# jinseikenai/glomeruli_segmentation

Hardware: AMD Instinct MI355X
Metric: patches/sec (1024x512 RGB) ESPNet p=2 q=8 5 classes, HBM-resident, two batches in flight (higher is better)
Workload: dtype f32; 1 GPU; ESPNet p=2 q=8 encoder+decoder, batch=32 synthetic 1024x512 uint8 BGR tiles per GPU, normalise+forward+argmax+counts, inputs resident in HBM, steps rotate through 4 distinct batches, 2 batch(es) in flight (engine lanes, one HIP stream each) for `value`; global_batch=32, weights=espnet_fold1 (tests/golden), parallelism=tile-range per rank x1

## Files before the change

glomeruli_segmentation_amd/_lib.py:

```python
import ctypes
import os

_PKG = os.path.dirname(os.path.abspath(__file__))
LIB_PATH = os.path.join(_PKG, "libglomseg.so")
if os.environ.get("GLOMSEG_LIB") and os.environ.get("GLOMSEG_EXPERIMENT") == "1":
    LIB_PATH = os.environ["GLOMSEG_LIB"]

GS_OK = 0
GS_IN_U8_BGR_NHWC = 0
GS_IN_F32_NCHW = 1
ABI_VERSION = 10
GS_BUILD_DIAG = 1
GS_FORM_NONE = -1
GS_MAX_ENSEMBLE_C = 8
MAX_CROPS_PER_CALL = 64

STATUS_NAMES = {0: "GS_OK", 1: "GS_ERR_INVALID", 2: "GS_ERR_HIP", 3: "GS_ERR_NOMEM", 4: "GS_ERR_UNSUPPORTED",
                5: "GS_ERR_NODEVICE", 6: "GS_ERR_DEVICE_FAULT"}


class GlomsegError(RuntimeError):
    def __init__(self, status, message):
        super().__init__("%s: %s" % (STATUS_NAMES.get(status, status), message))
        self.status = status


class LayerDesc(ctypes.Structure):
    _fields_ = [("name", ctypes.c_char * 96), ("offset", ctypes.c_int64), ("ndim", ctypes.c_int32),
                ("shape", ctypes.c_int32 * 4)]


class CropDesc(ctypes.Structure):
    _fields_ = [("in_off", ctypes.c_int64), ("out_off", ctypes.c_int64), ("h", ctypes.c_int32), ("w", ctypes.c_int32),
                ("x1", ctypes.c_int32), ("y1", ctypes.c_int32)]


class PasteTarget(ctypes.Structure):
    _fields_ = [("slide_map", ctypes.c_void_p), ("map_h", ctypes.c_int32), ("map_w", ctypes.c_int32), ("ds", ctypes.c_int32),
                ("sx_lut", ctypes.c_void_p), ("sy_lut", ctypes.c_void_p)]


class CropOverlay(ctypes.Structure):
    _fields_ = [("palette_rgb", ctypes.c_void_p), ("n_colours", ctypes.c_int32), ("wa", ctypes.c_float), ("wb", ctypes.c_float),
                ("out_bgr", ctypes.POINTER(ctypes.c_void_p))]


class CropScoring(ctypes.Structure):
    _fields_ = [("labels", ctypes.POINTER(ctypes.c_void_p)), ("conf", ctypes.c_void_p), ("seen", ctypes.c_void_p),
                ("gt_overlay_bgr", ctypes.POINTER(ctypes.c_void_p)), ("gt_clamp", ctypes.c_int32)]


class EvalBox(ctypes.Structure):
    _fields_ = [("x0", ctypes.c_int32), ("y0", ctypes.c_int32), ("x1", ctypes.c_int32), ("y1", ctypes.c_int32),
                ("raster_w", ctypes.c_int32), ("raster_h", ctypes.c_int32), ("offset", ctypes.c_int64)]


class EvalSet(ctypes.Structure):
    _fields_ = [("rasters", ctypes.c_void_p), ("raster_bytes", ctypes.c_int64), ("boxes", ctypes.c_void_p),
                ("n_boxes", ctypes.c_int32), ("win_ptr", ctypes.c_void_p), ("win_idx", ctypes.c_void_p), ("n_idx", ctypes.c_int32),
                ("small_map", ctypes.c_void_p)]


class DetectorLayerPlan(ctypes.Structure):
    _fields_ = [("images", ctypes.c_int64), ("in_h", ctypes.c_int32), ("in_w", ctypes.c_int32), ("out_h", ctypes.c_int32),
                ("out_w", ctypes.c_int32), ("form", ctypes.c_int32)]


class DetectorPlan(ctypes.Structure):
    _fields_ = [("hf", ctypes.c_int32), ("wf", ctypes.c_int32), ("workspace_bytes", ctypes.c_int64), ("n_layers", ctypes.c_int32),
                ("layers", DetectorLayerPlan * 16)]


class WeightPiece(ctypes.Structure):
    _fields_ = [("name", ctypes.c_char * 32), ("offset", ctypes.c_longlong), ("floats", ctypes.c_longlong)]


class KernelTime(ctypes.Structure):
    _fields_ = [("name", ctypes.c_char * 64), ("total_ms", ctypes.c_double), ("launches", ctypes.c_int64),
                ("flops_per_tile", ctypes.c_double)]


_P = ctypes.c_void_p
_FP = ctypes.POINTER(ctypes.c_float)
_I = ctypes.c_int

PROTOTYPES = {
    "gs_last_error": (ctypes.c_char_p, []),
    "gs_abi_version": (_I, []),
    "gs_build_flags": (_I, []),
    "gs_device_fault_check": (_I, []),
    "gs_espnet_create": (_I, [_P, ctypes.POINTER(LayerDesc), _I, _I, _I, _I, _I, ctypes.POINTER(_P)]),
    "gs_espnet_destroy": (None, [_P]),
    "gs_espnet_reserve": (_I, [_P, _I, _I, _I]),
    "gs_espnet_forward": (_I, [_P, _P, _I, _I, _I, _I, _FP, _FP, _P, _P, _P, _P]),
    "gs_espnet_set_lanes": (_I, [_P, _I]),
    "gs_espnet_lanes": (_I, [_P]),
    "gs_espnet_forward_lane": (_I, [_P, _I, _P, _I, _I, _I, _I, _FP, _FP, _P, _P, _P, _P]),
    "gs_espnet_segment_host": (_I, [_P, _P, _I, _I, _I, _FP, _FP, _I, _P, _P]),
    "gs_espnet_segment_crops": (_I, [_P, _I, _P, ctypes.POINTER(CropDesc), _I, _FP, _FP, _I, _I, _P, _P, _P,
                                ctypes.POINTER(PasteTarget), _P]),
    "gs_espnet_ensemble_segment_crops": (_I, [ctypes.POINTER(_P), _I, _P, ctypes.POINTER(CropDesc), _I, _FP, _FP, _I, _I, _P, _P, _P,
                                         ctypes.POINTER(PasteTarget), _P]),
    "gs_espnet_segment_crops_host": (_I, [ctypes.POINTER(_P), _I, ctypes.POINTER(_P), ctypes.POINTER(_I), ctypes.POINTER(_I), _I, _FP, _FP,
                                     _I, _I, _I, ctypes.POINTER(_P), _P, _P, ctypes.POINTER(PasteTarget), ctypes.POINTER(_I),
                                     ctypes.POINTER(_I), ctypes.POINTER(CropOverlay)]),
    "gs_crops_from_masks": (_I, [_P, ctypes.POINTER(CropDesc), _I, _I, _I, _I, _P, _P, ctypes.POINTER(PasteTarget), _P, _P, _I,
                            ctypes.c_float, ctypes.c_float, _I, _P, _P]),
    "gs_plan_crop_batches": (_I, [ctypes.POINTER(_I), ctypes.POINTER(_I), _I, _I, ctypes.POINTER(_I), _I, ctypes.POINTER(_I)]),
    "gs_host_block_is_pinned": (_I, [_P, ctypes.c_size_t]),
    "gs_espnet_ensemble_forward": (_I, [ctypes.POINTER(_P), _I, _P, _I, _I, _I, _FP, _FP, _P, _P, _P]),
    "gs_espnet_read_stage": (_I, [_P, ctypes.c_char_p, _I, _P, ctypes.c_size_t, ctypes.POINTER(_I * 3)]),
    "gs_espnet_block_forward": (_I, [_P, _I, _I, _I, _P, _I, _I, _P]),
    "gs_espnet_plan_forward": (_I, [_I, _I, _I, _I, _I, _I, _I, ctypes.POINTER(_I), _I, ctypes.POINTER(_I)]),
    "gs_espnet_form_info": (_I, [_I, _I, ctypes.POINTER(ctypes.c_char_p), ctypes.POINTER(_I)]),
    "gs_espnet_profile_enable": (_I, [_P, _I]),
    "gs_espnet_profile_read": (_I, [_P, ctypes.POINTER(KernelTime), _I, ctypes.POINTER(_I)]),
    "gs_crop_preprocess": (_I, [_P, _I, _I, _FP, _FP, _I, _I, _P, _P]),
    "gs_mask_resize_nearest": (_I, [_P, _I, _I, _I, _I, _P, _P]),
    "gs_find_contours": (_I, [_P, _I, _I, _I, _P, _I, _P, _I, ctypes.POINTER(_I), ctypes.POINTER(_I)]),
    "gs_arc_length_closed": (ctypes.c_double, [_P, _I]),
    "gs_approx_poly_closed": (_I, [_P, _I, ctypes.c_double, _P]),
    "gs_wsi_paste_max": (_I, [_P, _I, _I, _I, _P, _I, _I, _I, _I, _P]),
    "gs_wsi_paste_max_lut": (_I, [_P, _I, _I, _I, _P, _P, _P, _I, _I, _I, _I, _P]),
    "gs_overlay_classmap": (_I, [_P, _P, _I, _I, _P, _I, ctypes.c_float, ctypes.c_float, _P, _P]),
    "gs_confusion_u8": (_I, [_P, _P, ctypes.c_longlong, _I, _P, _P]),
    "gs_wsi_eval_windows": (_I, [_I, _I, _I, _I, ctypes.POINTER(EvalSet), ctypes.POINTER(EvalSet), _P, _P, _I, _I, _P, _P, _P]),
    "gs_conv2d_nhwc": (_I, [_P, _I, _I, _I, _I, _P, _I, _I, _I, _P, _I, _I, _I, _P, _P]),
    "gs_conv2d_nhwc_form": (_I, [_I] * 10 + [ctypes.POINTER(ctypes.c_char_p)]),
    "gs_roialign": (_I, [_P, _I, _I, _I, _I, _P, _P, _I, _I, _P, _P]),
    "gs_nms": (_I, [_P, _P, _I, ctypes.c_float, ctypes.c_float, _I, _P, _P, _P]),
    "gs_detector_create": (_I, [_P, ctypes.POINTER(LayerDesc), _I, ctypes.POINTER(_P)]),
    "gs_detector_destroy": (None, [_P]),
    "gs_detector_max_detections": (_I, []),
    "gs_detector_num_proposals": (_I, []),
    "gs_detector_layer_info": (_I, [_I, ctypes.POINTER(ctypes.c_char_p)] + [ctypes.POINTER(_I)] * 6),
    "gs_detector_plan": (_I, [_I, _I, _I, ctypes.POINTER(DetectorPlan)]),
    "gs_detector_set_thresholds": (_I, [_P, ctypes.c_float, ctypes.c_float, ctypes.c_float]),
    "gs_detector_forward": (_I, [_P, _P, _I, _I, _I, _P, _P, _P, _P, _P, _P, _P, _P, _P]),
    "gs_detector_detect_host": (_I, [_P, ctypes.POINTER(_P), _I, _I, _I, _I, _P, _P, _P, _P]),
}

SCORING_PROTOTYPES = {
    "gs_espnet_score_crops": (_I, [_P, _P, ctypes.POINTER(CropDesc), _I, _I, _I, _I, _P, _P, _P]),
    "gs_espnet_segment_crops_host_scored": (_I, PROTOTYPES["gs_espnet_segment_crops_host"][1] + [ctypes.POINTER(CropScoring)]),
}

PLAN_PROTOTYPES = {
    "gs_espnet_plan_flags": (_I, [_I, _I, _I, _I, _I, _I, _I, _I, ctypes.POINTER(_I)]),
    "gs_espnet_pack_weights": (_I, [_P, ctypes.POINTER(LayerDesc), _I, _I, _I, _I, _I, _P, ctypes.c_size_t, ctypes.POINTER(ctypes.c_size_t),
                                ctypes.POINTER(WeightPiece), _I, ctypes.POINTER(_I)]),
    "gs_espnet_workspace_plan": (_I, [_I] * 7 + [ctypes.POINTER(ctypes.c_size_t)]),
}
GS_PLAN_LAZY_B2, GS_PLAN_L3C_IN_REDUCE, GS_PLAN_CLS_IN_L3 = 1, 2, 4

INSTANCE_PROTOTYPES = {
    "gs_instances_plan": (_I, [_I, _I, _I, _I, ctypes.POINTER(ctypes.c_size_t)]),
    "gs_slide_instances": (_I, [_P, _I, _I, _I, _I, _P, ctypes.c_size_t, _I, _P, _P, _P, _P, _P]),
}

MATCH_PROTOTYPES = {
    "gs_instance_match_plan": (_I, [_I, _I, _I, ctypes.POINTER(ctypes.c_size_t)]),
    "gs_instance_overlaps": (_I, [_P, _P, _P, _P, _I, _I, _P, ctypes.c_size_t, _I, _P, _P, _P, _P]),
    "gs_instance_match": (_I, [_P, _P, _P, _I, _P, _I, _P, _I, _I, _I, _I, _P, _P, _P]),
}

BOUNDARY_PROTOTYPES = {
    "gs_boundary_dist_plan": (_I, [_I, _I, ctypes.POINTER(ctypes.c_size_t)]),
    "gs_instance_boundary_dist": (_I, [_P, _P, _P, _I, _P, _I, _I, _I, _P, ctypes.c_size_t, _P, _P, _P, _P]),
}

_lib = None


def load():
    global _lib
    if _lib is not None:
        return _lib
    if not os.path.exists(LIB_PATH):
        raise ImportError(
            "%s is missing: build it with `python -m glomeruli_segmentation_amd.build` "
            "(hipcc --offload-arch=gfx950).  There is no CPU fallback." % LIB_PATH)
    lib = ctypes.CDLL(LIB_PATH, mode=ctypes.RTLD_GLOBAL)
    for name, (res, args) in list(PROTOTYPES.items()) + list(SCORING_PROTOTYPES.items()) + list(PLAN_PROTOTYPES.items()) + \
            list(INSTANCE_PROTOTYPES.items()) + list(MATCH_PROTOTYPES.items()) + list(BOUNDARY_PROTOTYPES.items()):
        if name in PLAN_PROTOTYPES and not hasattr(lib, name):
            continue
        fn = getattr(lib, name)
        fn.restype = res
        fn.argtypes = args
    if lib.gs_abi_version() != ABI_VERSION:
        raise ImportError("libglomseg.so ABI %d != binding ABI %d: rebuild" % (lib.gs_abi_version(), ABI_VERSION))
    if (lib.gs_build_flags() & GS_BUILD_DIAG) and os.environ.get("GLOMSEG_ALLOW_DIAG") != "1":
        raise ImportError("%s is a -DGS_DIAG experiment build (its timing variants return wrong results by construction); "
                          "set GLOMSEG_ALLOW_DIAG=1 to load it for an A/B measurement" % LIB_PATH)
    _lib = lib
    return lib


def check(status):
    if status != GS_OK:
        raise GlomsegError(status, load().gs_last_error().decode("utf-8", "replace"))


def fptr3(values):
    arr = (ctypes.c_float * len(values))(*[float(v) for v in values])
    return arr
```

glomeruli_segmentation_amd/build.py:

```python
import os
import subprocess
import sys
import tempfile

PKG = os.path.dirname(os.path.abspath(__file__))
CSRC = os.path.join(PKG, "csrc")
LIB = os.path.join(PKG, "libglomseg.so")
SOURCES = ["espnet.hip", "dec_tail.hip", "crops.hip", "detect_ops.hip", "detector.hip", "wsi_eval.hip", "instances.hip", "instance_match.hip", "boundary_dist.hip", "contours.cpp"]
HEADERS = ["gs_internal.h", "conv_mfma.h", "dec_tail.h", "dec_tail_args.h", "espnet_kernels.h", "espnet_facts.h", "espnet_weights.h", "workspace_plan.h", "crop_sample.h", "crop_plan.h", "wave_block.h", "slide_map_plan.h", "instance_plan.h", "instance_match_plan.h", "boundary_dist_plan.h", "detect_math.h", "detect_plan.h", "host_copy.h", "host_jobs.h", "host_pipe.h",
           os.path.join("..", "..", "include", "glomseg.h"), os.path.join("..", "..", "include", "glomseg_scoring.h"),
           os.path.join("..", "..", "include", "glomseg_plan.h"), os.path.join("..", "..", "include", "glomseg_instances.h"),
           os.path.join("..", "..", "include", "glomseg_instance_match.h"),
           os.path.join("..", "..", "include", "glomseg_boundary_dist.h")]
FLAGS = ["-O3", "--offload-arch=gfx950", "-std=c++17", "-fPIC", "-Wall", "-Wno-unused-result",
         "-Wno-unused-value"]


def _sources():
    return [s for s in SOURCES if os.path.exists(os.path.join(CSRC, s))]


def _stale(lib):
    if not os.path.exists(lib):
        return True
    t = os.path.getmtime(lib)
    deps = [os.path.join(CSRC, s) for s in _sources() + HEADERS] + [os.path.abspath(__file__)]
    deps += [os.path.join(CSRC, f) for f in os.listdir(CSRC) if f.endswith(".h") or f.endswith(".inc")]
    return any(os.path.getmtime(d) > t for d in deps)


def build_lib(force=False, verbose=False, out=None, extra_flags=()):
    lib = os.path.abspath(out) if out else LIB
    if not (force or _stale(lib)):
        return lib
    hipcc = os.environ.get("HIPCC", "/opt/rocm/bin/hipcc")
    os.makedirs(os.path.dirname(lib), exist_ok=True)
    objdir = CSRC if out is None else tempfile.mkdtemp(prefix="glomseg_obj_")
    objs = []
    procs = []
    for s in _sources():
        o = os.path.join(objdir, s.replace(".hip", ".o").replace(".cpp", ".o"))
        objs.append(o)
        cmd = [hipcc] + FLAGS + list(extra_flags) + (["-x", "hip"] if s.endswith(".cpp") else []) + ["-c", os.path.join(CSRC, s), "-o", o]
        if verbose:
            print(" ".join(cmd))
        procs.append((cmd, subprocess.Popen(cmd)))
    for cmd, p in procs:
        if p.wait() != 0:
            raise RuntimeError("hipcc failed: " + " ".join(cmd))
    cmd = [hipcc, "--offload-arch=gfx950", "-shared", "-fPIC", "-o", lib] + objs + ["-Wl,-rpath,/opt/rocm/lib"]
    if verbose:
        print(" ".join(cmd))
    subprocess.check_call(cmd)
    return lib


if __name__ == "__main__":
    argv = sys.argv[1:]
    extra = []
    if "--" in argv:
        extra = argv[argv.index("--") + 1:]
        argv = argv[:argv.index("--")]
    out = argv[argv.index("--out") + 1] if "--out" in argv else None
    print(build_lib(force="--force" in argv or out is not None, verbose=True, out=out, extra_flags=extra))
```

glomeruli_segmentation_amd/csrc/conv_mfma.h:

```cpp
#pragma once
#include <map>
#include <mutex>
#include <type_traits>

#include "gs_internal.h"

namespace gs {

#ifdef GS_DIAG
constexpr bool kDiag = true;
#else
constexpr bool kDiag = false;
#endif

template <int N, typename F>
__device__ __forceinline__ void static_for(F &&f)
{
    if constexpr (N > 0) {
        static_for<N - 1>(f);
        f(std::integral_constant<int, N - 1>{});
    }
}

typedef float f32x16 __attribute__((ext_vector_type(16)));
typedef float f32x4 __attribute__((ext_vector_type(4)));

template <int MT>
struct Mfma;
template <>
struct Mfma<32> {
    static constexpr int KL = 2, NACC = 16;
    using acc_t = f32x16;
    static __device__ __forceinline__ acc_t run(float a, float b, acc_t c)
    {
        return __builtin_amdgcn_mfma_f32_32x32x2f32(a, b, c, 0, 0, 0);
    }
    static __device__ __forceinline__ int row(int r, int kq) { return (r & 3) + 8 * (r >> 2) + 4 * kq; }
};
template <>
struct Mfma<16> {
    static constexpr int KL = 4, NACC = 4;
    using acc_t = f32x4;
    static __device__ __forceinline__ acc_t run(float a, float b, acc_t c)
    {
        return __builtin_amdgcn_mfma_f32_16x16x4f32(a, b, c, 0, 0, 0);
    }
    static __device__ __forceinline__ int row(int r, int kq) { return kq * 4 + r; }
};

struct ConvArgs {
    const float *in;
    long long in_sn;
    int in_sc, in_pitch, in_off;
    unsigned in_img_bytes;
    const float *wpack;
    int wfloats;
    float *out;
    long long out_sn;
    int out_sc, out_pitch, out_off;
    unsigned out_img_bytes, res_img_bytes;
    const float *res;
    long long res_sn;
    int res_sc, res_pitch, res_off;
    float *out2;
    long long out2_sn;
    int out2_sc, out2_pitch, out2_off, out2_coff;
    unsigned out2_img_bytes;
    float *out3;
    long long out3_sn;
    int out3_sc, out3_pitch, out3_off, nout3;
    unsigned out3_img_bytes;
    int bnl_s0, bnl_s1;
    float *side;
    long long side_sn;
    int side_sc, side_pitch, side_off;
    unsigned side_img_bytes;
    const float *crec;
    float *cls;
    long long cls_sn;
    int cls_sc, cls_pitch;
    unsigned cls_img_bytes;
    int stagger;
    int prio_mode;
    unsigned long long *stamp;
    int N, H, W;
    int strips;
    int total_tasks;
    int wu;
};

typedef unsigned u32x3_t __attribute__((ext_vector_type(3)));
typedef unsigned u32x2_t __attribute__((ext_vector_type(2)));
typedef unsigned u32x4_t __attribute__((ext_vector_type(4)));

template <int N, int AUX = 0>
__device__ __forceinline__ void buf_load_vec(const __amdgpu_buffer_rsrc_t &rs, int voff, int soff, float *dst)
{
    if constexpr (N == 1) {
        dst[0] = __builtin_bit_cast(float, __builtin_amdgcn_raw_buffer_load_b32(rs, voff, soff, AUX));
    } else if constexpr (N == 2) {
        const u32x2_t v = __builtin_amdgcn_raw_buffer_load_b64(rs, voff, soff, AUX);
        const unsigned e0 = v[0], e1 = v[1];
        dst[0] = __builtin_bit_cast(float, e0);
        dst[1] = __builtin_bit_cast(float, e1);
    } else {
        static_assert(N == 4 || N == 8, "vector width");
#pragma unroll
        for (int h = 0; h < N / 4; ++h) {
            const u32x4_t v = __builtin_amdgcn_raw_buffer_load_b128(rs, voff + 16 * h, soff, AUX);
            const unsigned e0 = v[0], e1 = v[1], e2 = v[2], e3 = v[3];
            dst[4 * h + 0] = __builtin_bit_cast(float, e0);
            dst[4 * h + 1] = __builtin_bit_cast(float, e1);
            dst[4 * h + 2] = __builtin_bit_cast(float, e2);
            dst[4 * h + 3] = __builtin_bit_cast(float, e3);
        }
    }
}
template <int N, int AUX = 0>
__device__ __forceinline__ void buf_store_vec(const __amdgpu_buffer_rsrc_t &rs, int voff, const float *src)
{
    if constexpr (N == 1) {
        __builtin_amdgcn_raw_buffer_store_b32(__builtin_bit_cast(unsigned, src[0]), rs, voff, 0, AUX);
    } else if constexpr (N == 2) {
        u32x2_t v;
        v[0] = __builtin_bit_cast(unsigned, src[0]);
        v[1] = __builtin_bit_cast(unsigned, src[1]);
        __builtin_amdgcn_raw_buffer_store_b64(v, rs, voff, 0, AUX);
    } else {
#pragma unroll
        for (int h = 0; h < N / 4; ++h) {
            u32x4_t v;
#pragma unroll
            for (int j = 0; j < 4; ++j)
                v[j] = __builtin_bit_cast(unsigned, src[4 * h + j]);
            __builtin_amdgcn_raw_buffer_store_b128(v, rs, voff + 16 * h, 0, AUX);
        }
    }
}

__device__ __forceinline__ float prelu_pin(float alpha)
{
    return alpha <= 1.0f ? __builtin_inff() : -__builtin_inff();
}
__device__ __forceinline__ float prelu_med3(float v, float alpha, float pin)
{
    return __builtin_amdgcn_fmed3f(v, alpha * v, pin);
}

typedef float f32x2 __attribute__((ext_vector_type(2)));
__device__ __forceinline__ float cls_fma(float a, float b, float c) { return fmaf(a, b, c); }
__device__ __forceinline__ f32x2 cls_fma(float a, f32x2 b, f32x2 c) { return __builtin_elementwise_fma((f32x2)(a), b, c); }
__device__ __forceinline__ float cls_prelu(float v, float alpha, float pin) { return prelu_med3(v, alpha, pin); }
__device__ __forceinline__ f32x2 cls_prelu(f32x2 v, float alpha, float pin)
{
    const f32x2 av = v * alpha;
    f32x2 o;
    o[0] = __builtin_amdgcn_fmed3f(v[0], av[0], pin);
    o[1] = __builtin_amdgcn_fmed3f(v[1], av[1], pin);
    return o;
}

constexpr int F_BNACT = 1;
constexpr int F_RES = 2;
constexpr int F_NOSTORE = 4;
constexpr int F_DUAL = 8;
constexpr int F_S2PAIR = 512;
constexpr int F_VEC = 1024;
constexpr int F_RES_NT = 8192;
constexpr int F_ST_NT = 16384;
constexpr int F_ST2_NT = 32768;
constexpr int F_IN_NT = 65536;
constexpr int F_A_GLOBAL = 131072;
constexpr int F_FUSE1X1 = 262144;
constexpr int F_S2_FLIP = 1048576;
constexpr int F_SKIP_PAD = 4194304;
constexpr int F_BNLOAD = 8388608;
constexpr int F_SIDE_SHIFT = 27;
constexpr int F_SIDE1X1(int classes) { return classes << F_SIDE_SHIFT; }
constexpr int F_CLS1X1 = 256;
constexpr int CLS_N = 5, CLS_REC = 8;
constexpr int F_X_NOLOAD = 16;
constexpr int F_X_NOLDS = 32;
constexpr int F_X_NOEPI = 64;
constexpr int F_X_STAMP2 = 4096;
constexpr int STAMP2_SLOTS = 128;
constexpr int F_X_STAMP = 128;
constexpr int F_X_NOEPIMEM = 2097152;
constexpr int F_X_RESL2 = 33554432;
constexpr int F_X_STL2 = 67108864;
constexpr int F_X_ALL = F_X_NOLOAD | F_X_NOLDS | F_X_NOEPI | F_X_STAMP | F_X_STAMP2 | F_X_NOEPIMEM | F_X_RESL2 | F_X_STL2;

constexpr int conv_cls_lds_offset(int image_lds_floats) { return (image_lds_floats + 255) / 256 * 256; }

#ifndef CFG_STAGE_ROT
#define CFG_STAGE_ROT 17
#endif
#ifndef CFG_L3_RING
#define CFG_L3_RING 13
#endif
#ifndef CFG_L2_RING
#define CFG_L2_RING 27
#endif
constexpr int conv_ring_depth(int MT, int TAPS, int NDIL, int P, int G)
{
    return (MT == 32 && TAPS == 9 && NDIL == 5 && (P == 1 || P == 2) && G == 13) ? CFG_L3_RING
           : (MT == 16 && TAPS == 9 && NDIL == 5 && P == 4 && G == 9) ? CFG_L2_RING
                                                                    : G * (TAPS == 9 ? 3 : 1);
}

#define M_KL_OF(MT_) (Mfma<MT_>::KL)
template <int MT, int WAVES, int CINP, int TAPS, int STRIDE, int NDIL, int NOUT1, int NOUT, int P, int G, int FLAGS>
__global__ void __launch_bounds__(WAVES * 64, WAVES >= 8 ? WAVES / 8 : 2) conv_mfma_kernel(const ConvArgs a)
{
    constexpr bool BNACT = FLAGS & F_BNACT, RES = FLAGS & F_RES, STORE1 = !(FLAGS & F_NOSTORE), DUAL = FLAGS & F_DUAL;
    constexpr bool S2P = FLAGS & F_S2PAIR;
    constexpr bool VEC = FLAGS & F_VEC;
    constexpr bool AGL = FLAGS & F_A_GLOBAL, FUSE = FLAGS & F_FUSE1X1;
    constexpr bool S2FLIP = FLAGS & F_S2_FLIP;
    constexpr bool SKIP = FLAGS & F_SKIP_PAD;
    constexpr bool BNL = FLAGS & F_BNLOAD;
    constexpr int SCLS = (FLAGS >> F_SIDE_SHIFT) & 15;
    constexpr bool SIDE = SCLS > 0;
    constexpr bool CLSF = FLAGS & F_CLS1X1;
    static_assert(!CLSF || (MT == 32 && NDIL == 5 && TAPS == 9 && (FLAGS & F_BNACT) && !(FLAGS & (F_DUAL | F_NOSTORE | F_BNLOAD | F_X_ALL)) &&
                            !SIDE && ((NOUT1 + (NDIL - 1) * NOUT) * CLS_REC) % 256 == 0 && (NOUT1 + (NDIL - 1) * NOUT) * CLS_REC / 256 <= WAVES),
                  "F_CLS1X1 is for the level-3 branch launches: 32-row accumulators, five slots, the records in whole DMA pieces");
    static_assert(!SIDE || ((FLAGS & F_S2PAIR) && TAPS == 9 && STRIDE == 2 && MT == 32 && NDIL == 1 && SCLS <= SIDE_REC &&
                            (CINP / M_KL_OF(MT)) % G == 0 && G * M_KL_OF(MT) <= SIDE_ZROWS && !(FLAGS & (F_A_GLOBAL | F_VEC | F_X_ALL))),
                  "F_SIDE1X1 is for the stride-2 3x3 reduce on 32-pixel runs, a tap row in whole chunks");
    static_assert(!BNL || ((FLAGS & F_S2PAIR) && !(FLAGS & (F_BNACT | F_A_GLOBAL | F_VEC))), "F_BNLOAD is for the plain stride-2 reduce");
    static_assert(!SKIP || (TAPS == 9 && STRIDE == 1 && !(FLAGS & F_S2PAIR) && G * M_KL_OF(MT) == CINP),
                  "F_SKIP_PAD: unit-stride 3x3 with one tap row per chunk");
    static_assert(!S2FLIP || (STRIDE == 2 && TAPS == 9 && NDIL == 1), "F_S2_FLIP is for the stride-2 3x3 reduce");
    static_assert(kDiag || !(FLAGS & F_X_ALL), "timing / stamp variants exist in -DGS_DIAG builds only");
    constexpr int IAUX = (FLAGS & F_IN_NT) ? 2 : 0;
    constexpr int RAUX = (FLAGS & F_RES_NT) ? 2 : 0, SAUX = (FLAGS & F_ST_NT) ? 2 : 0, SAUX2 = (FLAGS & F_ST2_NT) ? 2 : 0;
    static_assert(!VEC || (STRIDE == 1 && (P == 2 || P == 4 || P == 8)), "F_VEC needs unit stride and P in {2,4,8}");
    static_assert(!S2P || (STRIDE == 2 && TAPS == 9 && NDIL == 1), "F_S2PAIR is for the stride-2 3x3 reduce");
    using M = Mfma<MT>;
    constexpr int KL = M::KL;
    constexpr int NSTEP = CINP / KL;
    constexpr int NROW = NOUT1 > NOUT ? NOUT1 : NOUT;
    constexpr int COUT = NOUT1 + (NDIL - 1) * NOUT;
    constexpr int TYN = TAPS == 1 ? 1 : 3;
    constexpr int TXN = TAPS == 9 ? 3 : 1;
    constexpr int XSTEP = P * MT;
    constexpr int RGN = TYN * NSTEP;
    constexpr int D = G * TXN;
    constexpr int R = conv_ring_depth(MT, TAPS, NDIL, P, G);
    constexpr int RA = R;
    static_assert(D % R == 0 && (R == D || !(FLAGS & (F_S2PAIR | F_BNLOAD))), "the ring divides the chunk");
    constexpr int CPD = RGN / G;
    constexpr int NCHUNK = NDIL * CPD;
    static_assert(CINP % KL == 0, "k-steps must tile");
    static_assert(TAPS == 1 || TAPS == 9, "1x1 or 3x3");
    static_assert(RGN % G == 0, "chunk must divide the row groups of one dilation");
    static_assert(NROW <= MT, "one MFMA row block");
    constexpr int KSTR = 4;

    extern __shared__ __attribute__((aligned(16))) float lds[];
    const int tid = threadIdx.x;
    unsigned long long tstamp0 = 0;
    if (FLAGS & (F_X_STAMP | F_X_STAMP2))
        tstamp0 = __builtin_amdgcn_s_memrealtime();
    constexpr int WFL = NDIL * TAPS * CINP * NROW;
    constexpr int LDS_SRC0 = AGL ? WFL : 0;
    static_assert(!AGL || WFL % 4 == 0, "LDS-DMA source must stay 16-byte aligned");
    static_assert(!FUSE || (TAPS == 9 && BNACT), "the fused 1x1 follows a branch kernel's epilogue");
    const float *bnp = lds + (WFL - LDS_SRC0);
    constexpr int BNFL = (BNACT ? 3 * COUT : 0) + (DUAL ? 3 * COUT : 0);
    const float *tab = bnp + BNFL;
    constexpr int BNL_C = CINP + M::KL;
    const float *bnl = lds + (conv_image(CINP, TAPS, NDIL, NOUT1, NOUT, BNACT, DUAL, FUSE ? M::NACC : 0).total - LDS_SRC0);
    const float *sidew = lds + side_table_offset(conv_image(CINP, TAPS, NDIL, NOUT1, NOUT, BNACT, DUAL, FUSE ? M::NACC : 0).total, CINP, M::KL);
    constexpr int CREC_OFF = conv_cls_lds_offset(conv_image(CINP, TAPS, NDIL, NOUT1, NOUT, BNACT, DUAL, FUSE ? M::NACC : 0).total - LDS_SRC0);
    const float *crecl = lds + CREC_OFF;
    const __amdgpu_buffer_rsrc_t rsrc_w =
        __builtin_amdgcn_make_buffer_rsrc(const_cast<float *>(a.wpack), 0, AGL ? WFL * 4 : 0, 0x00020000);

    const int lane = tid & 63;
    const int wid = __builtin_amdgcn_readfirstlane(tid >> 6);
    const int px = lane % MT, kq = lane / MT;
    const int xl = VEC ? px * P : px;
    const int voff = (kq * a.in_sc + xl * STRIDE) * 4;
    const int lbase = kq * NROW + (px < NROW ? px : NROW - 1);
    const int vout = (kq * KSTR * a.out_sc + xl) * 4;
    const int vres = RES ? (kq * KSTR * a.res_sc + xl) * 4 : 0;
    const int vout2 = DUAL ? (kq * KSTR * a.out2_sc + xl) * 4 : 0;
    const int vout3 = FUSE ? (kq * KSTR * a.out3_sc + xl) * 4 : 0;
    const int vcls = CLSF ? (kq * CLS_N * a.cls_sc + xl) * 4 : 0;
    const int prio_mode = kDiag ? a.prio_mode : 1;
    const bool second_of_simd = WAVES >= 8 ? wid >= WAVES / 2 : blockIdx.x >= gridDim.x / 2;

    const int NB = gridDim.x;
    const int wu = a.wu;
    int t0, t1, tstride;
    if ((NB & 7) == 0) {
        const int xcd = blockIdx.x & 7, per = NB >> 3;
        const int c0 = (int)((long long)a.total_tasks * xcd / 8), c1 = (int)((long long)a.total_tasks * (xcd + 1) / 8);
        t0 = c0 + (blockIdx.x >> 3) * wu + wid;
        t1 = c1;
        tstride = per * wu;
    } else {
        t0 = blockIdx.x * wu + wid;
        t1 = a.total_tasks;
        tstride = NB * wu;
    }
    if (wid >= wu)
        t0 = t1;
    const long long wg = (long long)blockIdx.x * WAVES + wid;
    const int tasks_per_img = a.H * a.strips;
    bool staged = false;

    float aq[RA], bq[S2P ? 1 : R][P];
    float bl[S2P ? G : 1][P][3];

    for (int task = t0; task < t1 || !staged; task += tstride) {
        const bool idle = task >= t1;
        const int tk = idle ? (a.total_tasks - 1) : task;
        const int n = tk / tasks_per_img;
        const int rem = tk - n * tasks_per_img;
        const int img_stride = tstride / tasks_per_img > 0 ? tstride / tasks_per_img : 1;
        const int yrot = SKIP ? a.H / 2 : 0;
        const int y0r = rem / a.strips;
        const int y = SKIP && ((n / img_stride) & 1) ? (y0r + yrot >= a.H ? y0r + yrot - a.H : y0r + yrot) : y0r;
        const int x0 = (rem - y0r * a.strips) * XSTEP;

        const __amdgpu_buffer_rsrc_t rsrc = __builtin_amdgcn_make_buffer_rsrc(
            const_cast<float *>(a.in + (long long)n * a.in_sn), 0, a.in_img_bytes, 0x00020000);
        const int sbase = (a.in_off + y * STRIDE * a.in_pitch + x0 * STRIDE) * 4;
        const int tn = task + tstride < t1 ? task + tstride : tk;
        const int n_n = tn / tasks_per_img;
        const int rem_n = tn - n_n * tasks_per_img;
        const int y0r_n = rem_n / a.strips;
        const int y_n = SKIP && ((n_n / img_stride) & 1) ? (y0r_n + yrot >= a.H ? y0r_n + yrot - a.H : y0r_n + yrot) : y0r_n;
        const __amdgpu_buffer_rsrc_t rsrc_n = __builtin_amdgcn_make_buffer_rsrc(
            const_cast<float *>(a.in + (long long)n_n * a.in_sn), 0, a.in_img_bytes, 0x00020000);
        const int sbase_n = (a.in_off + y_n * STRIDE * a.in_pitch + (rem_n - y0r_n * a.strips) * XSTEP * STRIDE) * 4;
        const bool flip = S2FLIP && (y & 1), flip_n = S2FLIP && (y_n & 1);
        const __amdgpu_buffer_rsrc_t rout =
            __builtin_amdgcn_make_buffer_rsrc(a.out + (long long)n * a.out_sn, 0, a.out_img_bytes, 0x00020000);
        const int sout = (a.out_off + y * a.out_pitch + x0) * 4;
        const __amdgpu_buffer_rsrc_t rres = __builtin_amdgcn_make_buffer_rsrc(
            const_cast<float *>(RES ? a.res + (long long)n * a.res_sn : a.in), 0, RES ? a.res_img_bytes : 0u, 0x00020000);
        const int sres = RES ? (a.res_off + y * a.res_pitch + x0) * 4 : 0;
        const __amdgpu_buffer_rsrc_t rout2 = __builtin_amdgcn_make_buffer_rsrc(
            DUAL ? a.out2 + (long long)n * a.out2_sn : a.out, 0, DUAL ? a.out2_img_bytes : 0u, 0x00020000);
        const int sout2 = DUAL ? (a.out2_off + y * a.out2_pitch + x0) * 4 : 0;
        const __amdgpu_buffer_rsrc_t rout3 = __builtin_amdgcn_make_buffer_rsrc(
            FUSE ? a.out3 + (long long)n * a.out3_sn : a.out, 0, FUSE ? a.out3_img_bytes : 0u, 0x00020000);
        const int sout3 = FUSE ? (a.out3_off + y * a.out3_pitch + x0) * 4 : 0;
        const __amdgpu_buffer_rsrc_t rcls = __builtin_amdgcn_make_buffer_rsrc(
            CLSF ? a.cls + (long long)n * a.cls_sn : a.out, 0, CLSF ? a.cls_img_bytes : 0u, 0x00020000);
        const int scls = CLSF ? (y * a.cls_pitch + x0) * 4 : 0;

        typename M::acc_t acc[P];
        typename M::acc_t acc2[FUSE ? P : 1];
        auto chunk_live = [&](int yy, int c) {
            const int di = c / CPD, ty = c - di * CPD;
            return ty == 1 || (ty == 0 ? yy >= (1 << di) : yy + (1 << di) < a.H);
        };
        const int c_first = SKIP && !chunk_live(y, 0) ? 1 : 0;
        const int c_first_n = SKIP && !chunk_live(y_n, 0) ? 1 : 0;

        constexpr int OOB = 0x7ffffff0;
        int vo[P], vr[P], vo2[P], vo3[P], vc[P];
#pragma unroll
        for (int p = 0; p < P; ++p) {
            const bool xok = x0 + (VEC ? xl : p * MT + px) < a.W;
            vo[p] = xok ? vout + (VEC ? 0 : p * MT * 4) : OOB;
            vr[p] = xok ? vres + (VEC ? 0 : p * MT * 4) : OOB;
            vo2[p] = xok ? vout2 + (VEC ? 0 : p * MT * 4) : OOB;
            vo3[p] = xok ? vout3 + (VEC ? 0 : p * MT * 4) : OOB;
            vc[p] = xok ? vcls + (VEC ? 0 : p * MT * 4) + scls : OOB;
        }
        constexpr int RR = RES ? M::NACC : 1;
        float resv[RR][P];
        auto load_res = [&](int di, int r) {
            if (!RES)
                return;
            if (FLAGS & F_X_NOEPIMEM) {
#pragma unroll
                for (int p = 0; p < P; ++p)
                    resv[r % RR][p] = __builtin_bit_cast(float, di + r + p);
                return;
            }
            const int nout = di == 0 ? NOUT1 : NOUT;
            const int cb = di == 0 ? 0 : NOUT1 + (di - 1) * NOUT;
            const int ch0 = M::row(r, 0);
            const bool live = ch0 + kq * KSTR < nout;
            const int sr = (cb + ch0) * a.res_sc * 4 + sres;
            if (VEC) {
                if (FLAGS & F_X_RESL2)
                    buf_load_vec<P, RAUX>(rres, live ? ((int)(wg & 255) * 8192 + ((vr[0] + sr) & 0x1ff0)) : OOB, 0, resv[r % RR]);
                else
                    buf_load_vec<P, RAUX>(rres, live ? vr[0] : OOB, sr, resv[r % RR]);
                return;
            }
#pragma unroll
            for (int p = 0; p < P; ++p)
                resv[r % RR][p] = __builtin_bit_cast(
                    float, __builtin_amdgcn_raw_buffer_load_b32(rres, live ? vr[p] : OOB, sr, RAUX));
        };
        auto prefetch_res = [&](int di) {
#pragma unroll
            for (int r = 0; r < RR; ++r)
                load_res(di, r);
        };

        auto decode_rg = [&](int cw, int g, int &ty0, int &sidx) {
            if constexpr (G % NSTEP == 0) {
                ty0 = cw * (G / NSTEP) + g / NSTEP;
                sidx = g % NSTEP;
            } else if constexpr (NSTEP % G == 0) {
                constexpr int CPR = NSTEP / G;
                ty0 = cw / CPR;
                sidx = (cw - ty0 * CPR) * G + g;
            } else {
                const int rg = cw * G + g;
                ty0 = rg / NSTEP;
                sidx = rg - ty0 * NSTEP;
            }
        };
        auto fetch_b = [&](const __amdgpu_buffer_rsrc_t &rs, int sb, int c, int g, int tx, bool fl) {
            const int di = c / CPD;
            int ty0, sidx;
            decode_rg(c - di * CPD, g, ty0, sidx);
            const int ty = S2FLIP && fl ? TYN - 1 - ty0 : ty0;
            const int toff = TAPS == 9 ? ((ty - 1) * a.in_pitch + (tx - 1)) << di : 0;
            const int soff = sb + (toff + sidx * KL * a.in_sc) * 4;
            if ((FLAGS & F_X_NOLOAD) && staged)
                return;
            if (VEC) {
                buf_load_vec<P, IAUX>(rs, voff, soff, bq[S2P ? 0 : (g * TXN + tx) % R]);
                return;
            }
#pragma unroll
            for (int p = 0; p < P; ++p)
                bq[(g * TXN + tx) % R][p] = __builtin_bit_cast(
                    float, __builtin_amdgcn_raw_buffer_load_b32(rs, voff + p * MT * STRIDE * 4, soff, IAUX));
        };
        auto fetch_pair = [&](const __amdgpu_buffer_rsrc_t &rs, int sb, int c, int g, bool fl) {
            if ((FLAGS & F_X_NOLOAD) && staged)
                return;
            int ty0, sidx;
            decode_rg(c, g, ty0, sidx);
            const int ty = S2FLIP && fl ? TYN - 1 - ty0 : ty0;
            const int soff = sb + ((ty - 1) * a.in_pitch - 1 + sidx * KL * a.in_sc) * 4;
#pragma unroll
            for (int p = 0; p < P; ++p) {
                const u32x3_t v = __builtin_amdgcn_raw_buffer_load_b96(rs, voff + p * MT * STRIDE * 4, soff, IAUX);
                const unsigned e0 = v[0], e1 = v[1], e2 = v[2];
                bl[g][p][0] = __builtin_bit_cast(float, e0);
                bl[g][p][1] = __builtin_bit_cast(float, e1);
                bl[g][p][2] = __builtin_bit_cast(float, e2);
            }
        };
        auto fetch_a = [&](int c, int g, int tx, bool fl) {
            const int di = c / CPD;
            int ty0, sidx;
            decode_rg(c - di * CPD, g, ty0, sidx);
            const int ty = S2FLIP && fl ? TYN - 1 - ty0 : ty0;
            const int tap = TAPS == 9 ? ty * 3 + tx : 0;
            if ((FLAGS & F_X_NOLDS) && staged)
                return;
            if (AGL)
                aq[(g * TXN + tx) % R] = __builtin_bit_cast(
                    float, __builtin_amdgcn_raw_buffer_load_b32(rsrc_w, lbase * 4, (((di * TAPS + tap) * CINP + sidx * KL) * NROW) * 4, 0));
            else
                aq[(g * TXN + tx) % R] = lds[((di * TAPS + tap) * CINP + sidx * KL) * NROW + lbase];
        };

        auto bnl_fetch = [&](int cc, int gg, int yy, bool ff, float &sc2, float &sh2, float &al2, bool &raw) {
            int ty0c, sidxc;
            decode_rg(cc, gg, ty0c, sidxc);
            const int tyc = S2FLIP && ff ? TYN - 1 - ty0c : ty0c;
            raw = sidxc >= a.bnl_s0 && sidxc < a.bnl_s1;
            const bool padrow = yy * STRIDE + tyc - 1 < 0 && raw;
            const int ch = (padrow ? NSTEP : sidxc) * KL + kq;
            sc2 = bnl[ch];
            sh2 = bnl[BNL_C + ch];
            al2 = bnl[2 * BNL_C + ch];
        };
        float tsc = 1.0f, tsh = 0.0f, tal = 1.0f, tpin = 0.0f;
        float nsc = 1.0f, nsh = 0.0f, nal = 1.0f;
        bool traw = false, nraw = false;
        float bt[BNL ? 2 : 1][P][3];
        static_assert(!BNL || G % 2 == 0, "F_BNLOAD: the two-group operand buffer alternates by row-group parity");
        auto bnl_apply = [&](float &dst, float v, float sc2, float sh2, float al2, float pin2, bool zero) {
            v = v * sc2 + sh2;
            v = prelu_med3(v, al2, pin2);
            dst = zero ? 0.0f : v;
        };

        float side[SIDE ? P : 1][SIDE ? SCLS : 1][2], sw[SIDE ? SCLS : 1];
        const __amdgpu_buffer_rsrc_t rside = __builtin_amdgcn_make_buffer_rsrc(
            SIDE ? a.side + (long long)n * a.side_sn : a.out, 0, SIDE ? a.side_img_bytes : 0u, 0x00020000);

        if (task == t0) {
#pragma unroll
            for (int g = 0; g < G; ++g) {
                if (S2P) {
                    fetch_pair(rsrc, sbase, 0, g, flip);
                    continue;
                }
#pragma unroll
                for (int tx = 0; tx < TXN; ++tx)
                    if (g * TXN + tx < R)
                        fetch_b(rsrc, sbase, c_first, g, tx, flip);
            }
        }
        if (!staged) {
            const int pieces = (a.wfloats - LDS_SRC0 + 255) / 256;
            if ((FLAGS & F_X_STAMP2) && lane == 0)
                a.stamp[wg * STAMP2_SLOTS + STAMP2_SLOTS - 2] = __builtin_amdgcn_s_memrealtime();
            const int rot = (int)((blockIdx.x * (unsigned)CFG_STAGE_ROT) % (unsigned)(pieces > 0 ? pieces : 1));
            for (int j0 = wid; j0 < pieces; j0 += WAVES) {
                const int j = j0 + rot < pieces ? j0 + rot : j0 + rot - pieces;
                __builtin_amdgcn_global_load_lds(
                    (const __attribute__((address_space(1))) void *)(a.wpack + LDS_SRC0 + j * 256 + lane * 4),
                    (__attribute__((address_space(3))) void *)(lds + j * 256), 16, 0, 0);
            }
            if (CLSF) {
                if (wid < COUT * CLS_REC / 256)
                    __builtin_amdgcn_global_load_lds(
                        (const __attribute__((address_space(1))) void *)(a.crec + wid * 256 + lane * 4),
                        (__attribute__((address_space(3))) void *)(lds + CREC_OFF + wid * 256), 16, 0, 0);
                if (tid < CLS_REC)
                    lds[CREC_OFF + COUT * CLS_REC + tid] = 0.0f;
// ... 421 lines not shown
```

glomeruli_segmentation_amd/csrc/espnet.hip:

```cpp
#include <chrono>
#include <cmath>
#include <cstdio>
#include <cstdlib>
#include <functional>
#include <map>
#include <memory>
#include <string>
#include <thread>
#include <vector>

#include "../../include/glomseg_plan.h"
#include "conv_mfma.h"
#include "dec_tail_args.h"
#include "enc_head.h"
#include "enc_head_ens.h"
#include "espnet_config.h"
#include "forward_plan.h"
#include "espnet_kernels.h"
#include "espnet_weights.h"
#include "host_copy.h"
#include "host_pipe.h"
#include "workspace_plan.h"

namespace gs {

static thread_local std::string g_err;
void set_error(const char *fmt, ...)
{
    char buf[1024];
    va_list ap;
    va_start(ap, fmt);
    vsnprintf(buf, sizeof buf, fmt, ap);
    va_end(ap);
    g_err = buf;
}

#ifdef GS_DIAG
static bool getenv_flag(const char *name)
{
    const char *e = std::getenv(name);
    return e && std::atoi(e) != 0;
}
static bool no_vec() { return getenv_flag("GS_NO_VEC"); }
#else
static constexpr bool no_vec() { return false; }
#endif

enum KernelId {
    K_STEM, K_POOL, K_L2_C1S, K_L2_DOWN, K_L2_C1, K_L2_ESP, K_CAT_B2, K_L3_C1S, K_L3_DOWN, K_L3_C1, K_L3_ESP,
    K_DEC1, K_DEC2, K_DEC3, K_DEC_CONV, K_DEC4, K_DEC_TAIL, K_ENC_HEAD, K_ENC_HEAD_ENS, K_COUNT
};
static const char *kKernelNames[K_COUNT] = {
    "stem_kernel", "pool_kernel", "conv_l2_reduce_s2", "conv_l2_down_branches", "conv_l2_reduce_1x1",
    "conv_l2_esp_branches", "cat_b2_kernel", "conv_l3_reduce_s2", "conv_l3_down_branches", "conv_l3_reduce_1x1",
    "conv_l3_esp_branches", "dec1_kernel", "dec2_kernel", "dec3_kernel", "conv_dec_cbr", "dec4_kernel", "dec_tail_kernel",
    "enc_head_kernel", "enc_head_ens_kernel"};

struct Model : Workspace {
    int classes = 0, p = 0, q = 0;
    int cp = 0;
    bool encoder_only = false;
    int device = 0, num_cus = 256;
#ifdef GS_DIAG
    int variant = 0;
#else
    static constexpr int variant = 0;
#endif
    float *dblob = nullptr;
    EspnetOffsets w;

    void *ws = nullptr;
    size_t ws_bytes = 0;
    int ws_n = 0, ws_h = 0, ws_w = 0;
    float *prob = nullptr;
    size_t prob_bytes = 0;
    std::map<std::string, std::pair<Act, int>> stages;
    void set_stage(const std::string &name, const Act &act, int C)
    {
        for (auto it = stages.begin(); it != stages.end();)
            it = it->second.first.base == act.base ? stages.erase(it) : std::next(it);
        stages[name] = {act, C};
    }
    int last_n = 0;
    bool b2_lazy = false;

    bool profile = false;
    struct Ev { hipEvent_t a, b; int k; };
    std::vector<Ev> events;
    double prof_ms[K_COUNT] = {0};
    long long prof_launches[K_COUNT] = {0};
    double prof_flops[K_COUNT] = {0};
};

static gs_status layout_workspace(Model *m, int n, int H, int W)
{
    if (m->ws && n <= m->ws_n && H == m->ws_h && W == m->ws_w)
        return GS_OK;
    if (m->ws) {
        GS_HIP(hipDeviceSynchronize());
        GS_HIP(hipFree(m->ws));
        m->ws = nullptr;
    }
    WorkspacePlan plan;
    const gs_status st = plan_workspace(n, H, W, m->cp, m->p, m->encoder_only, plan);
    if (st != GS_OK)
        return st;
    void *ws = nullptr;
    if (hipMalloc(&ws, plan.bytes) != hipSuccess) {
        set_error("workspace allocation of %zu bytes failed (n=%d, %dx%d)", plan.bytes, n, H, W);
        return GS_ERR_NOMEM;
    }
    GS_HIP(hipMemset(ws, 0, plan.bytes));
    GS_HIP(hipDeviceSynchronize());
    static_cast<Workspace &>(*m) = plan.acts;
    int i = 0;
    for (Act *a : acts_of(*m))
        a->base = reinterpret_cast<float *>(static_cast<char *>(ws) + plan.at[i++]);
    m->ws = ws;
    m->ws_bytes = plan.bytes;
    m->ws_n = n;
    m->ws_h = H;
    m->ws_w = W;
    return GS_OK;
}

struct Launcher {
    Model *m;
    hipStream_t s;
    gs_status st = GS_OK;
    int n;
    template <typename F>
    void run(int kid, double flops_per_tile, F &&f)
    {
        if (st != GS_OK)
            return;
        Model::Ev ev{nullptr, nullptr, kid};
        if (m->profile) {
            if (hipEventCreate(&ev.a) != hipSuccess || hipEventCreate(&ev.b) != hipSuccess ||
                hipEventRecord(ev.a, s) != hipSuccess) {
                set_error("profiling event setup failed");
                st = GS_ERR_HIP;
                return;
            }
        }
        st = f();
        if (st == GS_OK && hipGetLastError() != hipSuccess) {
            set_error("launch of %s failed", kKernelNames[kid]);
            st = GS_ERR_HIP;
        }
        if (m->profile && st == GS_OK) {
            hipEventRecord(ev.b, s);
            m->events.push_back(ev);
            m->prof_flops[kid] += flops_per_tile;
        }
    }
};

static ConvArgs conv_args(const Act &in, const float *wpack, const Act &out, const Act *res, int n)
{
    ConvArgs a{};
    a.in = in.base;
    a.in_sn = in.sn;
    a.in_sc = in.sc;
    a.in_pitch = in.pitch;
    a.in_off = in.off;
    a.in_img_bytes = (unsigned)(in.sn * sizeof(float));
    a.wpack = wpack;
    a.out = out.base;
    a.out_sn = out.sn;
    a.out_sc = out.sc;
    a.out_pitch = out.pitch;
    a.out_off = out.off;
    a.out_img_bytes = (unsigned)(out.sn * sizeof(float));
    if (res) {
        a.res = res->base;
        a.res_sn = res->sn;
        a.res_sc = res->sc;
        a.res_pitch = res->pitch;
        a.res_off = res->off;
        a.res_img_bytes = (unsigned)(res->sn * sizeof(float));
    }
    a.N = n;
    a.H = out.H;
    a.W = out.W;
    return a;
}

static inline unsigned blocks_for(long long items) { return (unsigned)((items + 255) / 256); }

#ifdef GS_DIAG
#include "espnet_diag.inc"
#define GS_DIAG_TRY(call)     \
    do {                      \
        gs_status dst_;       \
        if (call) return dst_; \
    } while (0)
#else
#define GS_DIAG_TRY(call) \
    do {                  \
    } while (0)
#define GS_DIAG_STAMPED(var, tag, ca, ...)
#endif

static gs_status not_planned(const char *launch_class)
{
    set_error("internal: the forward plan has no form for launch class %s", launch_class);
    return GS_ERR_INVALID;
}

template <int FLAGS, int... C>
static gs_status launch_vec(const ConvArgs &ca, int num_cus, hipStream_t s, bool vec)
{
    return vec ? launch_conv_mfma<C..., FLAGS | F_VEC>(ca, num_cus, s) : launch_conv_mfma<C..., FLAGS>(ca, num_cus, s);
}

static gs_status launch_l2_reduce(const Model *m, const ConvArgs &ca, hipStream_t s) { return launch_conv_mfma<CFG_L2_C1S, F_S2PAIR | POL_L2_C1S | S2FLIP_L2>(ca, m->num_cus, s); }
static gs_status launch_l2_c1(const Model *m, const ConvArgs &ca, hipStream_t s) { return launch_conv_mfma<CFG_L2_C1, POL_L2_C1>(ca, m->num_cus, s); }
static gs_status launch_l3_c1(const Model *m, const ConvArgs &ca, hipStream_t s) { return launch_conv_mfma<CFG_L3_C1, POL_L3_C1>(ca, m->num_cus, s); }

static gs_status launch_l2_down(const Model *m, form::l2_down f, const ConvArgs &ca, hipStream_t s)
{
    switch (f) {
    case form::l2_down::P2S_VEC: return launch_vec<F_BNACT | (POL_L2_DOWN & F_ST_NT) | FUSE_L2, CFG_L2_BR_P2S>(ca, m->num_cus, s, true);
    case form::l2_down::P4S_VEC_SKIP:
        GS_DIAG_STAMPED(162, "l2down", ca, F_BNACT | (POL_L2_DOWN & F_ST_NT) | FUSE_L2 | F_VEC, CFG_L2_BR_P4)
        return launch_conv_mfma<CFG_L2_BR_P4S, F_BNACT | (POL_L2_DOWN & F_ST_NT) | FUSE_L2 | F_VEC | F_SKIP_PAD>(ca, m->num_cus, s);
    case form::l2_down::P4_VEC:
        GS_DIAG_STAMPED(162, "l2down", ca, F_BNACT | (POL_L2_DOWN & F_ST_NT) | FUSE_L2 | F_VEC, CFG_L2_BR_P4)
        return launch_vec<F_BNACT | (POL_L2_DOWN & F_ST_NT) | FUSE_L2, CFG_L2_BR_P4>(ca, m->num_cus, s, true);
    case form::l2_down::P4: return launch_vec<F_BNACT | (POL_L2_DOWN & F_ST_NT) | FUSE_L2, CFG_L2_BR_P4>(ca, m->num_cus, s, false);
    case form::l2_down::UNFUSED_P4_VEC: return launch_vec<F_BNACT | (POL_L2_DOWN & F_ST_NT), CFG_L2_BR_P4>(ca, m->num_cus, s, true);
    case form::l2_down::UNFUSED_P4: return launch_vec<F_BNACT | (POL_L2_DOWN & F_ST_NT), CFG_L2_BR_P4>(ca, m->num_cus, s, false);
    case form::l2_down::none: break;
    }
    return not_planned("l2_down");
}

static gs_status launch_l2_esp_fused(const Model *m, form::l2_esp_fused f, const ConvArgs &ca, hipStream_t s)
{
    switch (f) {
    case form::l2_esp_fused::P2S_VEC: return launch_vec<F_BNACT | F_RES | POL_L2_ESP | FUSE_L2, CFG_L2_BR_P2S>(ca, m->num_cus, s, true);
    case form::l2_esp_fused::P4_VEC:
        GS_DIAG_STAMPED(161, "l2esp", ca, F_BNACT | F_RES | POL_L2_ESP | FUSE_L2 | F_VEC, CFG_L2_BR_P4)
        return launch_vec<F_BNACT | F_RES | POL_L2_ESP | FUSE_L2, CFG_L2_BR_P4>(ca, m->num_cus, s, true);
    case form::l2_esp_fused::P4: return launch_vec<F_BNACT | F_RES | POL_L2_ESP | FUSE_L2, CFG_L2_BR_P4>(ca, m->num_cus, s, false);
    case form::l2_esp_fused::UNFUSED_P4_VEC: return launch_vec<F_BNACT | F_RES | POL_L2_ESP, CFG_L2_BR_P4>(ca, m->num_cus, s, true);
    case form::l2_esp_fused::UNFUSED_P4: return launch_vec<F_BNACT | F_RES | POL_L2_ESP, CFG_L2_BR_P4>(ca, m->num_cus, s, false);
    case form::l2_esp_fused::none: break;
    }
    return not_planned("l2_esp_fused");
}

static gs_status launch_l2_esp_last(const Model *m, form::l2_esp_last f, const ConvArgs &ca, hipStream_t s)
{
    switch (f) {
    case form::l2_esp_last::P2S_VEC: return launch_vec<F_BNACT | F_RES | F_NOSTORE | F_DUAL | POL_L2_LAST, CFG_L2_BR_P2S>(ca, m->num_cus, s, true);
    case form::l2_esp_last::P4_VEC:
        GS_DIAG_STAMPED(163, "l2last", ca, F_BNACT | F_RES | F_NOSTORE | F_DUAL | POL_L2_LAST | F_VEC, CFG_L2_BR_P4)
        return launch_vec<F_BNACT | F_RES | F_NOSTORE | F_DUAL | POL_L2_LAST, CFG_L2_BR_P4>(ca, m->num_cus, s, true);
    case form::l2_esp_last::P4: return launch_vec<F_BNACT | F_RES | F_NOSTORE | F_DUAL | POL_L2_LAST, CFG_L2_BR_P4>(ca, m->num_cus, s, false);
    case form::l2_esp_last::none: break;
    }
    return not_planned("l2_esp_last");
}

static gs_status launch_l3_reduce(const Model *m, form::l3_reduce f, bool side5, const ConvArgs &ca, hipStream_t s)
{
    constexpr int SIDE5 = F_SIDE1X1(5);
    if (side5)
        switch (f) {
        case form::l3_reduce::BNL_P1: return launch_conv_mfma<CFG_L3_C1S_BNL_P1, F_S2PAIR | POL_L3_C1S | S2FLIP_L3 | F_BNLOAD | SIDE5>(ca, m->num_cus, s);
        case form::l3_reduce::BNL: return launch_conv_mfma<CFG_L3_C1S_BNL, F_S2PAIR | POL_L3_C1S | S2FLIP_L3 | F_BNLOAD | SIDE5>(ca, m->num_cus, s);
        case form::l3_reduce::C1S: return launch_conv_mfma<CFG_L3_C1S, F_S2PAIR | POL_L3_C1S | S2FLIP_L3 | SIDE5>(ca, m->num_cus, s);
        case form::l3_reduce::none: return not_planned("l3_reduce");
        }
    switch (f) {
    case form::l3_reduce::BNL_P1: return launch_conv_mfma<CFG_L3_C1S_BNL_P1, F_S2PAIR | POL_L3_C1S | S2FLIP_L3 | F_BNLOAD>(ca, m->num_cus, s);
    case form::l3_reduce::BNL:
        GS_DIAG_STAMPED(165, "l3c1s", ca, F_S2PAIR | POL_L3_C1S | S2FLIP_L3 | F_BNLOAD, CFG_L3_C1S_BNL)
        return launch_conv_mfma<CFG_L3_C1S_BNL, F_S2PAIR | POL_L3_C1S | S2FLIP_L3 | F_BNLOAD>(ca, m->num_cus, s);
    case form::l3_reduce::C1S: return launch_conv_mfma<CFG_L3_C1S, F_S2PAIR | POL_L3_C1S | S2FLIP_L3>(ca, m->num_cus, s);
    case form::l3_reduce::none: break;
    }
    return not_planned("l3_reduce");
}

static gs_status launch_l3_down(const Model *m, form::l3_down f, bool cls5, const ConvArgs &ca, hipStream_t s)
{
    if (cls5)
        switch (f) {
        case form::l3_down::P1R: return launch_conv_mfma<CFG_L3_BR_P1R, F_BNACT | POL_L3_DOWN | FUSE_L3 | SKIP_L3 | (CFG_SMALL_AGL ? F_A_GLOBAL : 0) | F_CLS1X1>(ca, m->num_cus, s);
        case form::l3_down::P2R_VEC: return launch_conv_mfma<CFG_L3_BR_P2R, F_BNACT | POL_L3_DOWN | FUSE_L3 | F_VEC | SKIP_L3 | F_CLS1X1>(ca, m->num_cus, s);
        case form::l3_down::P2F: return launch_conv_mfma<CFG_L3_BR_P2F, F_BNACT | POL_L3_DOWN | FUSE_L3 | F_CLS1X1>(ca, m->num_cus, s);
        default: return not_planned("l3_down with the classifier's side sums");
        }
    switch (f) {
    case form::l3_down::P1R: return launch_conv_mfma<CFG_L3_BR_P1R, F_BNACT | POL_L3_DOWN | FUSE_L3 | SKIP_L3 | (CFG_SMALL_AGL ? F_A_GLOBAL : 0)>(ca, m->num_cus, s);
    case form::l3_down::P2R_VEC:
        GS_DIAG_STAMPED(164, "l3down", ca, F_BNACT | POL_L3_DOWN | FUSE_L3 | F_VEC | SKIP_L3, CFG_L3_BR_P2R)
        return launch_conv_mfma<CFG_L3_BR_P2R, F_BNACT | POL_L3_DOWN | FUSE_L3 | F_VEC | SKIP_L3>(ca, m->num_cus, s);
    case form::l3_down::BR_VEC: return launch_conv_mfma<CFG_L3_BR, F_BNACT | POL_L3_DOWN | FUSE_L3 | F_VEC>(ca, m->num_cus, s);
    case form::l3_down::P2F: return launch_conv_mfma<CFG_L3_BR_P2F, F_BNACT | POL_L3_DOWN | FUSE_L3>(ca, m->num_cus, s);
    case form::l3_down::UNFUSED_BR_VEC: return launch_vec<F_BNACT | POL_L3_DOWN, CFG_L3_BR>(ca, m->num_cus, s, true);
    case form::l3_down::UNFUSED_BR: return launch_vec<F_BNACT | POL_L3_DOWN, CFG_L3_BR>(ca, m->num_cus, s, false);
    case form::l3_down::none: break;
    }
    return not_planned("l3_down");
}

static gs_status launch_l3_esp_fused(const Model *m, form::l3_esp_fused f, const ConvArgs &ca, int block, hipStream_t s)
{
    switch (f) {
    case form::l3_esp_fused::P1R: return launch_conv_mfma<CFG_L3_BR_P1R, F_BNACT | F_RES | POL_L3_ESP | FUSE_L3 | SKIP_L3 | (CFG_SMALL_AGL ? F_A_GLOBAL : 0)>(ca, m->num_cus, s);
    case form::l3_esp_fused::P2R_VEC:
        if (block == 1) {
            GS_DIAG_STAMPED(160, "l3esp", ca, F_BNACT | F_RES | F_VEC | POL_L3_ESP | FUSE_L3 | SKIP_L3, CFG_L3_BR_P2R)
        }
        return launch_conv_mfma<CFG_L3_BR_P2R, F_BNACT | F_RES | F_VEC | POL_L3_ESP | FUSE_L3 | SKIP_L3>(ca, m->num_cus, s);
    case form::l3_esp_fused::P2F: return launch_conv_mfma<CFG_L3_BR_P2F, F_BNACT | F_RES | FUSE_L3>(ca, m->num_cus, s);
    case form::l3_esp_fused::none: break;
    }
    return not_planned("l3_esp_fused");
}

static gs_status launch_l3_esp_last(const Model *m, form::l3_esp_last f, bool cls5, const ConvArgs &ca, hipStream_t s)
{
    if (cls5)
        switch (f) {
        case form::l3_esp_last::P1R: return launch_conv_mfma<CFG_L3_BR_P1R, F_BNACT | F_RES | POL_L3_ESP | SKIP_L3 | (CFG_SMALL_AGL ? F_A_GLOBAL : 0) | F_CLS1X1>(ca, m->num_cus, s);
        case form::l3_esp_last::P2R_VEC: return launch_conv_mfma<CFG_L3_BR_P2R, F_BNACT | F_RES | F_VEC | POL_L3_ESP | SKIP_L3 | F_CLS1X1>(ca, m->num_cus, s);
        case form::l3_esp_last::BR_VEC: return launch_conv_mfma<CFG_L3_BR, F_BNACT | F_RES | F_VEC | POL_L3_ESP | F_CLS1X1>(ca, m->num_cus, s);
        case form::l3_esp_last::P2: return launch_conv_mfma<CFG_L3_BR_P2, F_BNACT | F_RES | F_CLS1X1>(ca, m->num_cus, s);
        case form::l3_esp_last::none: return not_planned("l3_esp_last");
        }
    switch (f) {
    case form::l3_esp_last::P1R: return launch_conv_mfma<CFG_L3_BR_P1R, F_BNACT | F_RES | POL_L3_ESP | SKIP_L3 | (CFG_SMALL_AGL ? F_A_GLOBAL : 0)>(ca, m->num_cus, s);
    case form::l3_esp_last::P2R_VEC: return launch_conv_mfma<CFG_L3_BR_P2R, F_BNACT | F_RES | F_VEC | POL_L3_ESP | SKIP_L3>(ca, m->num_cus, s);
    case form::l3_esp_last::BR_VEC: return launch_conv_mfma<CFG_L3_BR, F_BNACT | F_RES | F_VEC | POL_L3_ESP>(ca, m->num_cus, s);
    case form::l3_esp_last::P2: return launch_conv_mfma<CFG_L3_BR_P2, F_BNACT | F_RES>(ca, m->num_cus, s);
    case form::l3_esp_last::none: break;
    }
    return not_planned("l3_esp_last");
}

template <int CLS>
static gs_status launch_dec3(const Model *m, form::dec3 f, const ConvArgs &ca, hipStream_t s)
{
    switch (f) {
    case form::dec3::MT16:
    case form::dec3::MT32: return launch_vec<F_BNACT, dec_mt(CLS), 8, 2 * CLS, 9, 1, 1, CLS, CLS, dec_pixels(CLS), 3>(ca, m->num_cus, s, false);
    case form::dec3::MT16_VEC:
    case form::dec3::MT32_VEC: return launch_vec<F_BNACT, dec_mt(CLS), 8, 2 * CLS, 9, 1, 1, CLS, CLS, dec_pixels(CLS), 3>(ca, m->num_cus, s, true);
    case form::dec3::KERNEL:
    case form::dec3::none: break;
    }
    return not_planned("dec3");
}

template <int CLS>
static gs_status launch_dec_conv(const Model *m, form::dec_conv f, const ConvArgs &ca, hipStream_t s)
{
    constexpr int CINP = (19 + CLS + 3) / 4 * 4;
    switch (f) {
    case form::dec_conv::MT16:
    case form::dec_conv::MT32: return launch_vec<F_BNACT | POL_DEC_CONV, dec_mt(CLS), 8, CINP, 9, 1, 1, CLS, CLS, dec_pixels(CLS), 3>(ca, m->num_cus, s, false);
    case form::dec_conv::MT16_VEC:
    case form::dec_conv::MT32_VEC: return launch_vec<F_BNACT | POL_DEC_CONV, dec_mt(CLS), 8, CINP, 9, 1, 1, CLS, CLS, dec_pixels(CLS), 3>(ca, m->num_cus, s, true);
    case form::dec_conv::TAIL:
    case form::dec_conv::none: break;
    }
    return not_planned("dec_conv");
}

struct Encoded { int last; bool lazy_b2; };
static Encoded encode(Model *m, Launcher &L, const ForwardPlan &plan, const ForwardReq &r)
{
    const float *wb = m->dblob;
    const hipStream_t s = r.s;
    const int n = r.n, H = r.H, W = r.W, H1 = H / 2, W1 = W / 2, H2 = H / 4, W2 = W / 4, H3 = H / 8, W3 = W / 8;
    const double px1 = (double)H1 * W1, px2 = (double)H2 * W2, px3 = (double)H3 * W3;
    m->stages.clear();
    m->last_n = n;
    L.run(K_STEM, px1 * (27 * 16 * 2), [&] {
        StemArgs a{};
        a.in = r.in;
        for (int i = 0; i < 3; ++i) {
            a.mean[i] = r.mean ? r.mean[i] : 0.0f;
            a.std[i] = r.stdv ? r.stdv[i] : 1.0f;
        }
        std::memcpy(a.w1, m->w.stem_params, sizeof(float) * 432);
        std::memcpy(a.bn1, m->w.stem_params + 432, sizeof(float) * 48);
        std::memcpy(a.b1, m->w.stem_params + 480, sizeof(float) * 57);
        a.a0 = view(m->a0);
        a.inp1 = view(m->inp1);
        a.N = n;
        a.H = H;
        a.W = W;
        if (r.hist && ens_finishes((int)r.role)) {
            a.hist_zero = r.hist;
            a.hist_count = n * m->classes;
        }
        hipLaunchKernelGGL(r.in_format == GS_IN_U8_BGR_NHWC ? stem_kernel<true> : stem_kernel<false>,
                           dim3(blocks_for((long long)n * H1 * ((W1 + STEM_PX - 1) / STEM_PX))), dim3(256), 0, s, a);
        return GS_OK;
    });
    L.run(K_POOL, 0, [&] {
        hipLaunchKernelGGL(pool_kernel, dim3(blocks_for((long long)n * 3 * H2 * W2)), dim3(256), 0, s, view(m->inp1),
                           view(m->inp2), n, 3, m->p > 0 ? wb + m->w.b2 : nullptr, view(m->a1), 128, 131);
        return GS_OK;
    });
    m->set_stage("b1", m->a0, 19);
    m->set_stage("sample2", m->inp2, 3);

    L.run(K_L2_C1S, px2 * (19 * 9 * 12 * 2), [&] {
        GS_DIAG_TRY(diag_reduce_s2(m, 2, conv_args(m->a0, wb + m->w.l2_0.c1, m->r2[0], nullptr, n), s, dst_));
        return launch_l2_reduce(m, conv_args(m->a0, wb + m->w.l2_0.c1, m->r2[0], nullptr, n), s);
    });
    auto with_dual = [&](ConvArgs a, int coff) {
        a.out2 = m->a1.base;
        a.out2_sn = m->a1.sn;
        a.out2_sc = m->a1.sc;
        a.out2_pitch = m->a1.pitch;
        a.out2_off = m->a1.off;
        a.out2_coff = coff;
        a.out2_img_bytes = (unsigned)(m->a1.sn * sizeof(float));
        return a;
    };
    auto with_fused = [&](ConvArgs a, const Act &r, int nout3) {
        a.out3 = r.base;
        a.out3_sn = r.sn;
        a.out3_sc = r.sc;
        a.out3_pitch = r.pitch;
        a.out3_off = r.off;
        a.out3_img_bytes = (unsigned)(r.sn * sizeof(float));
        a.nout3 = nout3;
        return a;
    };
    auto with_cls = [&](ConvArgs a, int producer) {
        a.crec = wb + m->w.b3 + (long long)producer * 128 * CLS_REC;
        a.cls_sc = H3 * W3;
        a.cls_pitch = W3;
        a.cls = m->tt.base + (long long)producer * 2 * CLS_N * a.cls_sc;
        a.cls_sn = m->tt.sn;
        a.cls_img_bytes = (unsigned)((size_t)2 * CLS_N * a.cls_sc * sizeof(float));
        return a;
    };
    const bool lazy_b2 = plan.lazy_b2;
    m->b2_lazy = lazy_b2;
    int rd2 = 0;
    L.run(K_L2_DOWN, px2 * (12 * 9 * 64 * 2) + (m->w.l2_0.fused_next ? px2 * (64 * 12 * 2) : 0), [&] {
        const ConvArgs ca = conv_args(m->r2[rd2], wb + m->w.l2_0.br, m->bb[0], nullptr, n);
        return launch_l2_down(m, plan.l2_down, m->w.l2_0.fused_next ? with_fused(ca, m->r2[rd2 ^ 1], 12) : ca, s);
    });
    bool have_r2 = m->w.l2_0.fused_next;
    rd2 ^= have_r2 ? 1 : 0;
    m->set_stage("level2_0", m->bb[0], 64);
    int cur2 = 0;
    for (int i = 0; i < m->p; ++i) {
        const int nxt = cur2 == 1 ? 2 : 1;
        const bool last = i == m->p - 1;
        const bool fuse_next = m->w.l2[i].fused_next;
        if (!have_r2)
            L.run(K_L2_C1, px2 * (64 * 12 * 2), [&] {
                return launch_l2_c1(m, conv_args(m->bb[cur2], wb + m->w.l2[i].c1, m->r2[rd2], nullptr, n), s);
            });
        L.run(K_L2_ESP, px2 * (12 * 9 * 64 * 2) + (fuse_next ? px2 * (64 * 12 * 2) : 0), [&] {
            const ConvArgs ca = conv_args(m->r2[rd2], wb + m->w.l2[i].br, m->bb[nxt], &m->bb[cur2], n);
            if (last)
                return launch_l2_esp_last(m, plan.l2_esp_last, with_dual(ca, 0), s);
            return launch_l2_esp_fused(m, plan.l2_esp_fused, fuse_next ? with_fused(ca, m->r2[rd2 ^ 1], 12) : ca, s);
        });
        have_r2 = fuse_next;
        rd2 ^= have_r2 ? 1 : 0;
        cur2 = nxt;
        if (!last)
            m->set_stage("level2." + std::to_string(i), m->bb[cur2], 64);
    }
    if (plan.cat_b2 == form::cat_b2::KERNEL) {
        L.run(K_CAT_B2, 0, [&] {
            hipLaunchKernelGGL(cat_b2_kernel, dim3(blocks_for((long long)n * 131 * H2 * W2)), dim3(256), 0, s, view(m->bb[cur2]),
                               view(m->bb[0]), view(m->inp2), wb + m->w.b2, view(m->a1), n);
            return GS_OK;
        });
    }
    m->set_stage("b2", m->a1, 131);

    int rd3 = 0;
    L.run(K_L3_C1S, px3 * (131 * 9 * 25 * 2) + (plan.l3c_in_reduce ? px2 * (131 * m->classes * 2) : 0), [&] {
        GS_DIAG_TRY(diag_reduce_s2(m, 3, conv_args(m->a1, wb + m->w.l3_0.c1, m->r3[0], nullptr, n), s, dst_));
        ConvArgs ca = conv_args(m->a1, wb + m->w.l3_0.c1, m->r3[0], nullptr, n);
        if (lazy_b2) {
            ca.bnl_s0 = 64 / 2;
            ca.bnl_s1 = 128 / 2;
        }
        if (plan.l3c_in_reduce) {
            ca.side = m->l3c.base;
            ca.side_sn = m->l3c.sn;
            ca.side_sc = m->l3c.sc;
            ca.side_pitch = m->l3c.pitch;
            ca.side_off = m->l3c.off;
            ca.side_img_bytes = (unsigned)(m->l3c.sn * sizeof(float));
        }
        return launch_l3_reduce(m, plan.l3_reduce, plan.l3c_in_reduce, ca, s);
    });
    if (plan.l3c_in_reduce)
        m->set_stage("level3_C", m->l3c, m->classes);
    const double cls_flops = plan.cls_in_l3 ? px3 * (128 * m->classes * 2) : 0;
    L.run(K_L3_DOWN, px3 * (25 * 9 * 128 * 2) + (m->w.l3_0.fused_next ? px3 * (128 * 25 * 2) : 0) + cls_flops, [&] {
        ConvArgs ca = conv_args(m->r3[rd3], wb + m->w.l3_0.br, m->cc[0], nullptr, n);
        if (plan.cls_in_l3) {
            if ((long long)CLS_PART_PLANES * H3 * W3 > m->tt.sn) {
                set_error("internal: the classifier's partial planes do not fit the workspace's tt");
                return GS_ERR_INVALID;
            }
            ca = with_cls(ca, 0);
        }
        return launch_l3_down(m, plan.l3_down, plan.cls_in_l3, m->w.l3_0.fused_next ? with_fused(ca, m->r3[rd3 ^ 1], 25) : ca, s);
    });
    bool have_r3 = m->w.l3_0.fused_next;
    m->set_stage("level3_reduce", m->r3[rd3], 25);
    rd3 ^= have_r3 ? 1 : 0;
    m->set_stage("level3_0", m->cc[0], 128);
    int cur3 = 0;
    for (int i = 0; i < m->q; ++i) {
        const int nxt = cur3 == 1 ? 2 : 1;
        const bool fuse_next = m->w.l3[i].fused_next;
        if (!have_r3)
            L.run(K_L3_C1, px3 * (128 * 25 * 2), [&] {
                return launch_l3_c1(m, conv_args(m->cc[cur3], wb + m->w.l3[i].c1, m->r3[rd3], nullptr, n), s);
            });
        L.run(K_L3_ESP, px3 * (25 * 9 * 128 * 2) + (fuse_next ? px3 * (128 * 25 * 2) : 0) + (i == m->q - 1 ? cls_flops : 0), [&] {
            const ConvArgs ca = conv_args(m->r3[rd3], wb + m->w.l3[i].br, m->cc[nxt], &m->cc[cur3], n);
            GS_DIAG_TRY(diag_l3_esp(m, ca, i, s, dst_));
            if (fuse_next)
                return launch_l3_esp_fused(m, plan.l3_esp_fused, with_fused(ca, m->r3[rd3 ^ 1], 25), i, s);
            const bool cls5 = plan.cls_in_l3 && i == m->q - 1;
            return launch_l3_esp_last(m, plan.l3_esp_last, cls5, cls5 ? with_cls(ca, 1) : ca, s);
        });
        have_r3 = fuse_next;
        rd3 ^= have_r3 ? 1 : 0;
        cur3 = nxt;
        m->set_stage("level3." + std::to_string(i), m->cc[cur3], 128);
    }
    return {cur3, lazy_b2};
}

template <int CLS>
static gs_status decode(Model *m, Launcher &L, const ForwardPlan &plan, const ForwardReq &r, const Encoded &enc)
{
    const float *wb = m->dblob;
    const hipStream_t s = r.s;
    const int n = r.n, H = r.H, W = r.W, H1 = H / 2, W1 = W / 2, H2 = H / 4, W2 = W / 4, H3 = H / 8, W3 = W / 8;
    const double px1 = (double)H1 * W1, px2 = (double)H2 * W2, px3 = (double)H3 * W3;
    const int ncls = m->classes;
    float *enc_logits = !m->encoder_only ? nullptr : r.logits ? r.logits : m->o2c.base;
    L.run(K_DEC1, (plan.cls_in_l3 ? 0 : px3 * (256 * ncls * 2)) + px3 * (ncls * ncls * 4 * 2), [&] {
        if constexpr (CLS == CLS_N) {
            if (plan.cls_in_l3) {
                Dec1SumsArgs a{};
                a.part = m->tt.base;
                a.psn = m->tt.sn;
                a.psc = H3 * W3;
                a.br = wb + m->w.br;
                a.wup = wb + m->w.wup3;
                a.out = view(m->o2c);
                a.N = n;
                a.H3 = H3;
                a.W3 = W3;
                a.classes = ncls;
                hipLaunchKernelGGL(dec1_sums_kernel<CLS>, dim3(blocks_for((long long)n * H3 * W3)), dim3(256), 0, s, a);
                return GS_OK;
            }
        }
        Dec1Args a{};
        a.c0 = view(m->cc[0]);
        a.clast = view(m->cc[enc.last]);
        a.b3w = wb + m->w.b3;
        a.br = m->encoder_only ? nullptr : wb + m->w.br;
        a.wup = m->encoder_only ? nullptr : wb + m->w.wup3;
        a.out = view(m->o2c);
        a.enc_logits = enc_logits;
        a.N = n;
        a.classes = ncls;
        constexpr int CB = CLS <= 5 ? 16 : CLS <= 8 ? 8 : 4;
        hipLaunchKernelGGL((dec1_kernel<CLS, CB>), dim3((unsigned)(((long long)n * H3 * W3 + 63) / 64)), dim3(256), 0, s, a);
        return GS_OK;
    });
    if (m->encoder_only) {
        if (r.mask)
            L.run(K_ENC_HEAD, (double)H * W * (ncls * 6), [&] {
                EncHeadArgs a{};
                a.logits = enc_logits;
                a.mask = r.mask;
                a.hist = r.hist;
                a.classes = ncls;
                a.H3 = H3;
                a.W3 = W3;
                launch_enc_head(a, n, s);
                return GS_OK;
            });
        return L.st;
    }
    m->set_stage("up_l3", m->o2c, ncls);

    L.run(K_DEC2, plan.l3c_in_reduce ? 0 : px2 * (131 * ncls * 2), [&] {
        Dec2Args a{};
        a.o2c = view(m->o2c);
        a.br = wb + m->w.cbr0;
        a.t = view(m->tt);
        a.N = n;
        a.classes = ncls;
        if constexpr (l3c_side_sums(CLS)) {
            if (plan.l3c_in_reduce) {
                a.a1 = view(m->l3c);
                hipLaunchKernelGGL(dec2_br_kernel<CLS>, dim3(blocks_for((long long)n * H2 * W2)), dim3(256), 0, s, a);
                return GS_OK;
            }
        }
        a.a1 = view(m->a1);
        a.raw = view(m->bb[0]);
        a.b2 = wb + m->w.b2;
        a.raw_c0 = 64;
        a.raw_cn = enc.lazy_b2 ? 64 : 0;
        a.w3c = wb + m->w.w3c;
        hipLaunchKernelGGL(dec2_kernel<CLS>, dim3((unsigned)(((long long)n * H2 * W2 + 63) / 64)), dim3(256), 0, s, a);
        return GS_OK;
    });
    if (ncls == CLS)
        m->set_stage("combine_t", m->tt, 2 * CLS);
    if constexpr (dec3_on_mfma(CLS)) {
        L.run(K_DEC3, px2 * (2 * ncls * 9 * ncls * 2), [&] {
            return launch_dec3<CLS>(m, plan.dec3, conv_args(m->tt, wb + m->w.wcc_mfma, m->t3, nullptr, n), s);
        });
        L.run(K_DEC3, px2 * (ncls * ncls * 4 * 2), [&] {
            Dec3Args a{};
            a.t = view(m->t3);
            a.wup = wb + m->w.wup2;
            a.bnu = wb + m->w.bnu2;
            a.e = view(m->ee);
            a.N = n;
            a.classes = ncls;
            hipLaunchKernelGGL(dec3b_kernel<CLS>, dim3(blocks_for((long long)n * H2 * W2)), dim3(256), 0, s, a);
            return GS_OK;
        });
    } else {
        L.run(K_DEC3, px2 * (2 * ncls * 9 * ncls * 2) + px2 * (ncls * ncls * 4 * 2), [&] {
            Dec3Args a{};
            a.t = view(m->tt);
            a.wc = wb + m->w.wcc;
            a.bnc = wb + m->w.bncc;
            a.wup = wb + m->w.wup2;
            a.bnu = wb + m->w.bnu2;
            a.e = view(m->ee);
            a.N = n;
            a.classes = ncls;
            hipLaunchKernelGGL(dec3_kernel<CLS>, dim3(blocks_for((long long)n * H2 * W2)), dim3(256), 0, s, a);
            return GS_OK;
        });
    }
    m->set_stage("up_l2", m->ee, ncls);
    if constexpr (dec_tail_fused(CLS)) {
        L.run(K_DEC_TAIL, px1 * ((19 + CLS) * 9 * CLS * 2) + px1 * (CLS * CLS * 4 * 2), [&] {
            DecTailArgs a{};
            a.in = m->a0c.base;
            a.in_sn = m->a0c.sn;
            a.in_sc = m->a0c.sc;
            a.in_pitch = m->a0c.pitch;
            a.in_off = m->a0c.off;
            a.in_img_bytes = (unsigned)(m->a0c.sn * sizeof(float));
            a.wpack = wb + m->w.wtail;
            a.logits = r.logits;
            a.mask = r.mask;
            a.hist = ens_finishes((int)r.role) ? r.hist : nullptr;
            a.prob = r.prob;
            a.ens_mode = (int)r.role;
            a.ens_w = r.ens_w;
            if (r.logits) {
                a.ff = m->ff.base;
                a.ff_sn = m->ff.sn;
                a.ff_sc = m->ff.sc;
                a.ff_pitch = m->ff.pitch;
                a.ff_off = m->ff.off;
            }
            a.N = n;
            a.H1 = H1;
            a.W1 = W1;
            return launch_dec_tail(a, m->num_cus, s);
        });
        if (r.logits)
            m->set_stage("conv", m->ff, CLS);
    } else {
        L.run(K_DEC_CONV, px1 * ((19 + ncls) * 9 * ncls * 2), [&] {
            return launch_dec_conv<CLS>(m, plan.dec_conv, conv_args(m->a0c, wb + m->w.wconv, m->ff, nullptr, n), s);
        });
        m->set_stage("conv", m->ff, ncls);
        L.run(K_DEC4, px1 * (ncls * ncls * 4 * 2), [&] {
            Dec4Args a{};
            a.f = view(m->ff);
            a.wcl = wb + m->w.wclassifier;
            a.logits = r.logits;
            a.mask = r.mask;
            a.hist = r.hist;
            a.prob = r.prob;
            a.ens_mode = (int)r.role;
            a.ens_w = r.ens_w;
            a.N = n;
            a.classes = ncls;
            const dim3 grid(blocks_for(((long long)H1 * W1 + dec4_px<CLS>() - 1) / dec4_px<CLS>()), n);
            hipLaunchKernelGGL((r.role != EnsRole::NONE ? dec4_kernel<CLS, true> : dec4_kernel<CLS, false>), grid, dim3(256), 0, s, a);
            return GS_OK;
        });
    }
    return L.st;
}

static gs_status forward_any(Model *m, const ForwardReq &r)
{
    Launcher L{m, r.s, GS_OK, r.n};
    const ForwardPlan plan = plan_forward(r.n, r.H, r.W, m->p, m->q, m->cp, m->num_cus, no_vec(), m->encoder_only);
    const Encoded e = encode(m, L, plan, r);
    switch (m->cp) {
    case 5: return decode<5>(m, L, plan, r, e);
    case 4: return decode<4>(m, L, plan, r, e);
    case 8: return decode<8>(m, L, plan, r, e);
    case 12: return decode<12>(m, L, plan, r, e);
    case 16: return decode<16>(m, L, plan, r, e);
    case 20: return decode<20>(m, L, plan, r, e);
    }
    set_error("internal: no decoder instantiation for %d padded classes", m->cp);
    return GS_ERR_UNSUPPORTED;
}

struct TileSlot : PipeSlot {
    Staging<uint8_t> in, out;
    Staging<unsigned long long> hist;
    void free_staging() { in.free(), out.free(), hist.free(); }
};

}

using namespace gs;

extern "C" {

const char *gs_last_error(void) { return g_err.c_str(); }
int gs_abi_version(void) { return 10; }
gs_status gs_device_fault_check(void)
{
    GS_HIP(hipDeviceSynchronize());
    int flags = 0;
    gs_status st = dec_tail_fault_flags(&flags);
    if (st != GS_OK) return st;
    if (flags) {
        set_error("device fault word %d: a decoder-tail wave gave up its strip-boundary exchange; the results of the calls since the last check are invalid", flags);
        return GS_ERR_DEVICE_FAULT;
    }
    return GS_OK;
}
int gs_build_flags(void)
{
#ifdef GS_DIAG
    return GS_BUILD_DIAG;
#else
    return 0;
#endif
}

struct gs_espnet {
    Model m;
    std::vector<std::unique_ptr<Model>> lanes;
    HostPipe<TileSlot, 4> tile_pipe;
    gs::CropPipe *crop_pipe = nullptr;
    Model &lane(int k) { return k == 0 ? m : *lanes[k - 1]; }
};

}

namespace gs {
CropPipe *&espnet_crop_pipe(gs_espnet *h) { return h->crop_pipe; }
int espnet_device(gs_espnet *h) { return h->m.device; }
int espnet_is_full_net(gs_espnet *h) { return h->m.encoder_only ? 0 : 1; }
int espnet_lanes(gs_espnet *h) { return 1 + (int)h->lanes.size(); }
int espnet_classes(gs_espnet *h) { return h->m.classes; }
static gs_status ensemble_scratch(gs_espnet *h, int lane, int n, int height, int width, float **prob)
{
    GS_REQUIRE(lane >= 0 && lane <= (int)h->lanes.size(), "lane %d does not exist (gs_espnet_set_lanes)", lane);
    Model &m0 = h->lane(lane);
    const gs_status st = grow(m0.prob, m0.prob_bytes, (size_t)n * m0.classes * height * width * sizeof(float), "ensemble scratch");
    *prob = m0.prob;
    return st;
}
gs_status espnet_forward(gs_espnet *h, int lane, const ForwardReq &r)
{
    GS_REQUIRE(h && r.in, "forward: null handle or input");
    GS_REQUIRE(lane >= 0 && lane <= (int)h->lanes.size(), "lane %d does not exist (gs_espnet_set_lanes)", lane);
    Model &m = h->lane(lane);
    GS_REQUIRE(!m.encoder_only || r.role == EnsRole::NONE, "an ESPNet-C handle cannot be an ensemble member");
    const gs_status st = layout_workspace(&m, r.n, r.H, r.W);
    return st != GS_OK ? st : forward_any(&m, r);
}

gs_status ensemble_kind(gs_espnet *const *models, int n_models, bool *enc_only)
{
    int n_enc = 0;
    for (int k = 0; k < n_models; ++k) {
        GS_REQUIRE(models[k], "ensemble member %d is null", k);
        n_enc += models[k]->m.encoder_only ? 1 : 0;
    }
    *enc_only = n_enc == n_models;
    for (int k = 0; k < n_models; ++k) {
        GS_REQUIRE(*enc_only || !models[k]->m.encoder_only, "ensemble member %d is not a full ESPNet", k);
        GS_REQUIRE(models[k]->m.classes == models[0]->m.classes, "ensemble member %d has %d classes, member 0 has %d", k,
                   models[k]->m.classes, models[0]->m.classes);
        for (int j = 0; *enc_only && j < k; ++j)
            GS_REQUIRE(models[j] != models[k], "ESPNet-C ensemble members %d and %d are the same handle", j, k);
    }
    if (*enc_only && n_models > GS_MAX_ENSEMBLE_C) {
        set_error("an ESPNet-C ensemble has at most %d members (got %d)", GS_MAX_ENSEMBLE_C, n_models);
        return GS_ERR_UNSUPPORTED;
    }
    return GS_OK;
}

static gs_status espnet_c_ensemble_head(gs_espnet *const *models, int n_models, int lane, const ForwardReq &r)
{
    EncHeadEnsArgs a{};
    for (int k = 0; k < n_models; ++k) {
        const Model &mk = models[k]->lane(lane);
        GS_REQUIRE(mk.encoder_only && mk.ws && r.n <= mk.ws_n && r.H == mk.ws_h && r.W == mk.ws_w,
                   "internal: member %d holds no 1/8-scale logits of this batch", k);
        a.logits[k] = mk.o2c.base;
    }
    a.mask = r.mask;
    a.hist = r.hist;
    a.classes = models[0]->m.classes;
    a.members = n_models;
    a.H3 = r.H / 8;
    a.W3 = r.W / 8;
    a.inv_members = 1.0f / (float)n_models;
    Model &m0 = models[0]->lane(lane);
    Launcher L{&m0, r.s, GS_OK, r.n};
    L.run(K_ENC_HEAD_ENS, (double)r.H * r.W * (a.classes * n_models * 20), [&] {
        launch_ens_head(a, r.n, r.s);
        return GS_OK;
    });
    return L.st;
}

gs_status run_ensemble(gs_espnet *const *models, int n_models, int lane, const ForwardReq &shared, const float *means,
                       const float *stds, const std::function<gs_status(int)> &prepare)
{
    const bool enc_only = models[0]->m.encoder_only;
    ForwardReq r = shared;
    r.ens_w = 1.0f / (float)n_models;
    gs_status st = GS_OK;
    if (!enc_only && (st = ensemble_scratch(models[0], lane, r.n, r.H, r.W, &r.prob)) != GS_OK) return st;
    for (int k = 0; k < n_models; ++k) {
        if (prepare && (st = prepare(k)) != GS_OK) return st;
        r.mean = means ? means + 3 * k : nullptr, r.stdv = stds ? stds + 3 * k : nullptr;
        if (enc_only)
            r.mask = nullptr, r.hist = k == 0 ? shared.hist : nullptr;
        else
            r.role = ens_role(k, n_models);
        st = espnet_forward(models[k], lane, r);
        if (st != GS_OK) return st;
    }
    return enc_only ? espnet_c_ensemble_head(models, n_models, lane, shared) : GS_OK;
}
}

extern "C" {

static gs_status check_model_args(const char *fn, const float *blob, const gs_layer_desc *table, int n_layers, int classes, int p, int q)
{
    GS_REQUIRE(blob && table && n_layers > 0, "%s: null argument", fn);
    GS_REQUIRE(p >= 0 && q >= 0, "%s: p and q must be non-negative", fn);
    if (classes < 2 || classes > 20) {
        set_error("%s: classes must be 2..20 (got %d)", fn, classes);
        return GS_ERR_UNSUPPORTED;
    }
    return GS_OK;
}

gs_status gs_espnet_create(const float *blob, const gs_layer_desc *table, int n_layers, int classes, int p, int q,
                           int encoder_only, gs_espnet **out)
{
    GS_REQUIRE(out, "gs_espnet_create: null argument");
    gs_status st = check_model_args("gs_espnet_create", blob, table, n_layers, classes, p, q);
    if (st != GS_OK) return st;
    int ndev = 0;
    if (hipGetDeviceCount(&ndev) != hipSuccess || ndev == 0) {
        set_error("gs_espnet_create: no HIP device visible");
        return GS_ERR_NODEVICE;
    }
    std::unique_ptr<gs_espnet> h(new gs_espnet());
    Model &m = h->m;
    m.classes = classes;
    m.cp = padded_classes(classes);
    m.p = p;
    m.q = q;
    m.encoder_only = encoder_only != 0;
    GS_HIP(hipGetDevice(&m.device));
    hipDeviceProp_t prop;
    GS_HIP(hipGetDeviceProperties(&prop, m.device));
    if (std::strncmp(prop.gcnArchName, "gfx950", 6) != 0) {
        set_error("gs_espnet_create: device %d is %s; this library is built for gfx950 only", m.device, prop.gcnArchName);
        return GS_ERR_NODEVICE;
    }
    m.num_cus = prop.multiProcessorCount;
#ifdef GS_DIAG
    if (const char *v = std::getenv("GS_VARIANT"))
        m.variant = std::atoi(v);
#endif
    EspnetWeights packed;
    st = pack_espnet_weights(blob, table, n_layers, classes, p, q, m.encoder_only, packed);
    if (st != GS_OK) return st;
    m.w = packed;
    GS_HIP(hipMalloc(reinterpret_cast<void **>(&m.dblob), packed.blob.size() * sizeof(float)));
    GS_HIP(hipMemcpy(m.dblob, packed.blob.data(), packed.blob.size() * sizeof(float), hipMemcpyHostToDevice));
    *out = h.release();
    return GS_OK;
}

gs_status gs_espnet_pack_weights(const float *blob, const gs_layer_desc *table, int n_layers, int classes, int p, int q,
                                 int encoder_only, float *out, size_t cap, size_t *n_floats, gs_weight_piece *pieces, int piece_cap,
                                 int *n_pieces)
{
    GS_REQUIRE(n_floats, "gs_espnet_pack_weights: null argument");
    gs_status st = check_model_args("gs_espnet_pack_weights", blob, table, n_layers, classes, p, q);
    if (st != GS_OK) return st;
    EspnetWeights packed;
    st = pack_espnet_weights(blob, table, n_layers, classes, p, q, encoder_only != 0, packed);
    if (st != GS_OK) return st;
    *n_floats = packed.blob.size();
    if (n_pieces) *n_pieces = (int)packed.pieces.size();
    if (out) {
        GS_REQUIRE(cap >= packed.blob.size(), "gs_espnet_pack_weights: %zu floats needed, room for %zu", packed.blob.size(), cap);
        std::memcpy(out, packed.blob.data(), packed.blob.size() * sizeof(float));
    }
    if (pieces) {
        GS_REQUIRE(piece_cap >= (int)packed.pieces.size(), "gs_espnet_pack_weights: %zu pieces, room for %d", packed.pieces.size(), piece_cap);
        std::memcpy(pieces, packed.pieces.data(), packed.pieces.size() * sizeof(gs_weight_piece));
    }
    return GS_OK;
}

static void free_lane(Model &l)
{
    for (auto &ev : l.events) {
        hipEventDestroy(ev.a);
        hipEventDestroy(ev.b);
    }
    if (l.ws) hipFree(l.ws);
    if (l.prob) hipFree(l.prob);
}

void gs_espnet_destroy(gs_espnet *h)
{
    if (!h)
        return;
    hipDeviceSynchronize();
    h->tile_pipe.destroy();
    crop_pipe_destroy(h->crop_pipe);
    for (int k = 0; k <= (int)h->lanes.size(); ++k)
        free_lane(h->lane(k));
    if (h->m.dblob) hipFree(h->m.dblob);
    delete h;
}

static gs_status check_shape(int n, int height, int width)
{
    GS_REQUIRE(n > 0, "batch size must be positive (got %d)", n);
    GS_REQUIRE(height >= 8 && width >= 8 && height % 8 == 0 && width % 8 == 0,
               "tile size must be a positive multiple of 8 in both dimensions (got %dx%d)", height, width);
    return GS_OK;
}

gs_status gs_espnet_reserve(gs_espnet *h, int n, int height, int width)
{
    GS_REQUIRE(h, "null handle");
    gs_status st = check_shape(n, height, width);
    if (st != GS_OK) return st;
    for (int k = 0; k <= (int)h->lanes.size(); ++k) {
        st = layout_workspace(&h->lane(k), n, height, width);
        if (st != GS_OK) return st;
    }
    return GS_OK;
}

gs_status gs_espnet_workspace_plan(int n, int height, int width, int p, int q, int classes, int encoder_only, size_t *bytes)
{
    GS_REQUIRE(bytes, "gs_espnet_workspace_plan: null argument");
    gs_status st = check_shape(n, height, width);
    if (st != GS_OK) return st;
    GS_REQUIRE(p >= 0 && q >= 0, "gs_espnet_workspace_plan: p and q must be non-negative");
    if (classes < 2 || classes > 20) {
        set_error("gs_espnet_workspace_plan: classes must be 2..20 (got %d)", classes);
        return GS_ERR_UNSUPPORTED;
    }
    WorkspacePlan plan;
    st = plan_workspace(n, height, width, padded_classes(classes), p, encoder_only != 0, plan);
    *bytes = plan.bytes;
    return st;
}

gs_status gs_espnet_set_lanes(gs_espnet *h, int n_lanes)
{
    GS_REQUIRE(h, "null handle");
    GS_REQUIRE(n_lanes >= 1 && n_lanes <= 4, "gs_espnet_set_lanes: 1 to 4 lanes (got %d)", n_lanes);
    GS_HIP(hipDeviceSynchronize());
    while ((int)h->lanes.size() > n_lanes - 1) {
        free_lane(*h->lanes.back());
        h->lanes.pop_back();
    }
    while ((int)h->lanes.size() < n_lanes - 1) {
        std::unique_ptr<Model> l(new Model(h->m));
        l->ws = nullptr;
        l->ws_bytes = 0;
        l->ws_n = l->ws_h = l->ws_w = 0;
        l->prob = nullptr;
        l->prob_bytes = 0;
        l->stages.clear();
        l->events.clear();
        l->profile = false;
        h->lanes.push_back(std::move(l));
    }
    return GS_OK;
}

int gs_espnet_lanes(gs_espnet *h) { return h ? 1 + (int)h->lanes.size() : 0; }

gs_status gs_espnet_forward(gs_espnet *h, const void *in, int in_format, int n, int height, int width,
                            const float mean[3], const float std[3], float *logits, uint8_t *mask,
                            unsigned long long *hist, void *hip_stream)
{
    return gs_espnet_forward_lane(h, 0, in, in_format, n, height, width, mean, std, logits, mask, hist, hip_stream);
}

gs_status gs_espnet_forward_lane(gs_espnet *h, int lane, const void *in, int in_format, int n, int height, int width,
                                 const float mean[3], const float std[3], float *logits, uint8_t *mask,
                                 unsigned long long *hist, void *hip_stream)
{
    GS_REQUIRE(h && in, "gs_espnet_forward: null handle or input");
    GS_REQUIRE(lane >= 0 && lane <= (int)h->lanes.size(), "lane %d does not exist (gs_espnet_set_lanes)", lane);
    gs_status st = check_shape(n, height, width);
    if (st != GS_OK) return st;
    GS_REQUIRE(in_format == GS_IN_U8_BGR_NHWC || in_format == GS_IN_F32_NCHW, "unknown input format %d", in_format);
    GS_REQUIRE(in_format != GS_IN_U8_BGR_NHWC || (mean && std), "uint8 input needs mean and std");
    GS_REQUIRE(logits || mask, "nothing to compute: logits and mask are both NULL");
    GS_REQUIRE(!hist || mask, "hist requires the mask output");
    if (in_format == GS_IN_U8_BGR_NHWC)
        for (int i = 0; i < 3; ++i)
            GS_REQUIRE(std[i] != 0.0f, "std[%d] is zero", i);
    ForwardReq r;
    r.in = in, r.in_format = in_format, r.n = n, r.H = height, r.W = width;
    r.mean = mean, r.stdv = std, r.logits = logits, r.mask = mask, r.hist = hist, r.s = static_cast<hipStream_t>(hip_stream);
    return espnet_forward(h, lane, r);
}

gs_status gs_espnet_read_stage(gs_espnet *h, const char *stage, int image, float *dst, size_t cap, int dims[3])
{
    GS_REQUIRE(h && stage && dims, "gs_espnet_read_stage: null argument");
    Model &m = h->m;
    auto it = m.stages.find(stage);
    GS_REQUIRE(it != m.stages.end(), "stage '%s' was not produced by the last forward", stage);
    GS_REQUIRE(image >= 0 && image < m.last_n, "image index %d out of range", image);
    const Act &a = it->second.first;
    const int C = it->second.second;
    dims[0] = C;
    dims[1] = a.H;
    dims[2] = a.W;
    const size_t count = (size_t)C * a.H * a.W;
    if (!dst)
        return GS_OK;
    GS_REQUIRE(cap >= count, "destination too small for stage '%s'", stage);
    float *tmp = nullptr;
    GS_HIP(hipMalloc(reinterpret_cast<void **>(&tmp), count * sizeof(float)));
    hipLaunchKernelGGL(unpad_kernel, dim3(blocks_for((long long)count)), dim3(256), 0, 0, view(a), image, C, tmp);
    if (m.b2_lazy && std::string(stage) == "b2")
        hipLaunchKernelGGL(b2_apply_kernel, dim3(blocks_for((long long)64 * a.H * a.W)), dim3(256), 0, 0, tmp, m.dblob + m.w.b2, a.H * a.W, 64, 64);
    hipError_t e = hipMemcpy(dst, tmp, count * sizeof(float), hipMemcpyDeviceToHost);
    hipFree(tmp);
    GS_HIP(e);
    return GS_OK;
}

gs_status gs_espnet_block_forward(gs_espnet *h, int kind, int level, int index, const float *in, int height, int width,
                                  float *out)
{
    GS_REQUIRE(h && in && out, "gs_espnet_block_forward: null argument");
    GS_REQUIRE((kind == 0 || kind == 1) && (level == 2 || level == 3), "kind must be 0/1 and level 2/3");
    GS_REQUIRE(height >= 1 && width >= 1, "empty input");
    Model &m = h->m;
    GS_REQUIRE(kind == 1 || (index >= 0 && index < (level == 2 ? m.p : m.q)), "no ESP block %d at level %d", index, level);
    GS_REQUIRE(kind == 0 || (height % 2 == 0 && width % 2 == 0), "the down-sampler needs an even input size");
    const int up = kind == 0 ? (level == 2 ? 4 : 8) : (level == 2 ? 2 : 4);
    gs_status st = layout_workspace(&m, 1, height * up, width * up);
    if (st != GS_OK) return st;
    const float *wb = m.dblob;
    const Act &src = kind == 0 ? (level == 2 ? m.bb[0] : m.cc[0]) : (level == 2 ? m.a0 : m.a1);
    const Act &dst = level == 2 ? (kind == 0 ? m.bb[1] : m.bb[0]) : (kind == 0 ? m.cc[1] : m.cc[0]);
    const Act &red = level == 2 ? m.r2[0] : m.r3[0];
    const int cin = kind == 0 ? (level == 2 ? 64 : 128) : (level == 2 ? 19 : 131);
    const int cout = level == 2 ? 64 : 128;
    GS_REQUIRE(src.H == height && src.W == width, "internal: workspace level size mismatch");
    const size_t nin = (size_t)cin * height * width, nout = (size_t)cout * dst.H * dst.W;
    float *tmp = nullptr;
    GS_HIP(hipMalloc(reinterpret_cast<void **>(&tmp), (nin > nout ? nin : nout) * sizeof(float)));
    gs_status rc = GS_OK;
    hipStream_t s = nullptr;
    auto body = [&]() -> gs_status {
        GS_HIP(hipMemcpy(tmp, in, nin * sizeof(float), hipMemcpyHostToDevice));
        hipLaunchKernelGGL(pad_kernel, dim3(blocks_for((long long)nin)), dim3(256), 0, s, view(src), 0, cin, tmp);
        const PackedConv &pc = kind == 1 ? (level == 2 ? m.w.l2_0 : m.w.l3_0) : (level == 2 ? m.w.l2[index] : m.w.l3[index]);
        const ConvArgs rca = conv_args(src, wb + pc.c1, red, nullptr, 1);
        const ConvArgs bca = conv_args(red, wb + pc.br, dst, kind == 1 ? nullptr : &src, 1);
        gs_status r;
        if (level == 2) {
            r = kind == 1 ? launch_l2_reduce(&m, rca, s) : launch_l2_c1(&m, rca, s);
            if (r != GS_OK) return r;
            r = kind == 1 ? launch_l2_down(&m, unfused_l2_down(dst.W, no_vec()), bca, s)
                          : launch_l2_esp_fused(&m, unfused_l2_esp(dst.W, no_vec()), bca, s);
        } else {
            r = kind == 1 ? launch_l3_reduce(&m, form::l3_reduce::C1S, false, rca, s) : launch_l3_c1(&m, rca, s);
            if (r != GS_OK) return r;
            r = kind == 1 ? launch_l3_down(&m, unfused_l3_down(dst.W, no_vec()), false, bca, s)
                          : launch_l3_esp_last(&m, whole_row_l3_esp(dst.W, no_vec()), false, bca, s);
        }
        if (r != GS_OK) return r;
        hipLaunchKernelGGL(unpad_kernel, dim3(blocks_for((long long)nout)), dim3(256), 0, s, view(dst), 0, cout, tmp);
        GS_HIP(hipGetLastError());
        GS_HIP(hipMemcpy(out, tmp, nout * sizeof(float), hipMemcpyDeviceToHost));
        return GS_OK;
    };
    rc = body();
    hipFree(tmp);
    m.stages.clear();
    return rc;
}

gs_status gs_espnet_plan_forward(int n, int height, int width, int p, int q, int classes, int num_cus, int *out_forms, int cap,
                                 int *n_out)
{
    GS_REQUIRE(n_out, "gs_espnet_plan_forward: null argument");
    gs_status st = check_shape(n, height, width);
    if (st != GS_OK) return st;
    GS_REQUIRE(p >= 0 && q >= 0 && num_cus > 0, "gs_espnet_plan_forward: p and q must be non-negative, num_cus positive");
    if (classes < 2 || classes > 20) {
        set_error("gs_espnet_plan_forward: classes must be 2..20 (got %d)", classes);
        return GS_ERR_UNSUPPORTED;
    }
    *n_out = kLaunchClassCount;
    if (!out_forms)
        return GS_OK;
    GS_REQUIRE(cap >= kLaunchClassCount, "gs_espnet_plan_forward: %d entries needed, room for %d", kLaunchClassCount, cap);
    plan_forward(n, height, width, p, q, padded_classes(classes), num_cus, no_vec()).codes(out_forms);
    return GS_OK;
}

gs_status gs_espnet_plan_flags(int n, int height, int width, int p, int q, int classes, int encoder_only, int num_cus, int *flags)
{
    GS_REQUIRE(flags, "gs_espnet_plan_flags: null argument");
    int count = 0;
    gs_status st = gs_espnet_plan_forward(n, height, width, p, q, classes, num_cus, nullptr, 0, &count);
    if (st != GS_OK) return st;
    const ForwardPlan pl = plan_forward(n, height, width, p, q, padded_classes(classes), num_cus, no_vec(), encoder_only != 0);
    *flags = (pl.lazy_b2 ? GS_PLAN_LAZY_B2 : 0) | (pl.l3c_in_reduce ? GS_PLAN_L3C_IN_REDUCE : 0) | (pl.cls_in_l3 ? GS_PLAN_CLS_IN_L3 : 0);
    return GS_OK;
}

gs_status gs_espnet_form_info(int launch_class, int form, const char **name, int *pixels_per_lane)
{
    GS_REQUIRE(launch_class >= 0 && launch_class < kLaunchClassCount, "no launch class %d", launch_class);
    const LaunchClassInfo &c = kLaunchClasses[launch_class];
    GS_REQUIRE(form >= GS_FORM_NONE && form < c.n_forms, "launch class %s has no form %d", c.name, form);
    if (name) *name = form == GS_FORM_NONE ? c.name : c.forms[form].name;
    if (pixels_per_lane) *pixels_per_lane = form == GS_FORM_NONE ? 0 : c.forms[form].pixels_per_lane;
    return GS_OK;
}

gs_status gs_espnet_profile_enable(gs_espnet *h, int on)
{
    GS_REQUIRE(h, "null handle");
    h->m.profile = on != 0;
    return GS_OK;
}

gs_status gs_espnet_profile_read(gs_espnet *h, gs_kernel_time *out, int cap, int *n_out)
{
    GS_REQUIRE(h && n_out, "null argument");
    Model &m = h->m;
    for (auto &ev : m.events) {
        GS_HIP(hipEventSynchronize(ev.b));
        float ms = 0.0f;
        GS_HIP(hipEventElapsedTime(&ms, ev.a, ev.b));
        m.prof_ms[ev.k] += ms;
        m.prof_launches[ev.k] += 1;
        hipEventDestroy(ev.a);
        hipEventDestroy(ev.b);
    }
    m.events.clear();
    int k = 0;
    for (int i = 0; i < K_COUNT && out && k < cap; ++i) {
        if (!m.prof_launches[i])
            continue;
        std::snprintf(out[k].name, sizeof out[k].name, "%s", kKernelNames[i]);
        out[k].total_ms = m.prof_ms[i];
        out[k].launches = m.prof_launches[i];
        out[k].flops_per_tile = m.prof_flops[i] / (double)m.prof_launches[i];
        ++k;
    }
    *n_out = k;
    for (int i = 0; i < K_COUNT; ++i) {
        m.prof_ms[i] = 0;
        m.prof_launches[i] = 0;
        m.prof_flops[i] = 0;
    }
    return GS_OK;
}

gs_status gs_espnet_ensemble_forward(gs_espnet *const *models, int n_models, const void *in_u8, int n, int height,
                                     int width, const float *means, const float *stds, uint8_t *mask,
                                     unsigned long long *hist, void *hip_stream)
{
    GS_REQUIRE(models && n_models > 0 && in_u8 && means && stds && mask, "gs_espnet_ensemble_forward: null argument");
    gs_status st = check_shape(n, height, width);
    if (st != GS_OK) return st;
    bool enc_only = false;
    st = ensemble_kind(models, n_models, &enc_only);
    if (st != GS_OK) return st;
    for (int k = 0; k < n_models; ++k)
        for (int i = 0; i < 3; ++i)
            GS_REQUIRE(stds[3 * k + i] != 0.0f, "ensemble member %d: std[%d] is zero", k, i);
    ForwardReq r;
    r.in = in_u8, r.in_format = GS_IN_U8_BGR_NHWC, r.n = n, r.H = height, r.W = width;
    r.mask = mask, r.hist = hist, r.s = static_cast<hipStream_t>(hip_stream);
    return run_ensemble(models, n_models, 0, r, means, stds);
}

gs_status gs_espnet_segment_host(gs_espnet *h, const uint8_t *tiles, int n_tiles, int height, int width,
                                 const float mean[3], const float std[3], int batch, uint8_t *masks,
                                 unsigned long long *hist)
{
    GS_REQUIRE(h && tiles && masks && mean && std, "gs_espnet_segment_host: null argument");
    GS_REQUIRE(n_tiles > 0 && batch > 0, "n_tiles and batch must be positive");
    gs_status st = check_shape(batch, height, width);
    if (st != GS_OK) return st;
    if (batch > n_tiles) batch = n_tiles;
    const size_t in_b = (size_t)height * width * 3, out_b = (size_t)height * width;
    const size_t ncl = (size_t)h->m.classes;
    const int nl = h->lanes.empty() ? 1 : 2;
    const bool in_pinned = host_is_pinned(tiles), out_pinned = host_is_pinned(masks) && (!hist || host_is_pinned(hist));
    auto &pipe = h->tile_pipe;
    HipLatch fail;
    if (!pipe.ensure(2, true, fail, [&](TileSlot &s) {
            s.in.grow(in_b * batch, fail);
            s.out.grow(out_b * batch, fail);
            s.hist.grow(sizeof(unsigned long long) * GS_MAX_CLASSES * batch, fail);
        }))
        return fail.rc;
#ifdef GS_DIAG
    const bool ptrace = std::getenv("GS_PIPE_TRACE") != nullptr;
    const auto pt0 = std::chrono::steady_clock::now();
    auto stamp = [&](int bi, const char *what) {
        if (ptrace && bi < 12)
            std::fprintf(stderr, "pipe %2d %-10s %9.1f us\n", bi, what,
                         std::chrono::duration<double, std::micro>(std::chrono::steady_clock::now() - pt0).count());
    };
    const int pskip = std::getenv("GS_PIPE_SKIP") ? std::atoi(std::getenv("GS_PIPE_SKIP")) : 0;
#else
    auto stamp = [](int, const char *) {};
    constexpr int pskip = 0;
#endif
    const gs_status rc = pipe.run(
        (n_tiles + batch - 1) / batch, nl == 1, fail,
        [&](int bi, TileSlot &s, hipStream_t h2d) {
            s.first = bi * batch;
            s.count = n_tiles - s.first < batch ? n_tiles - s.first : batch;
            const uint8_t *src = tiles + (size_t)s.first * in_b;
            if (!in_pinned) {
                parallel_memcpy(s.in.h, src, in_b * s.count);
                src = s.in.h;
            }
            if (!(pskip & 1) || bi < pipe.NSLOT)
                fail(hipMemcpyAsync(s.in.d, src, in_b * s.count, hipMemcpyHostToDevice, h2d), "H2D copy");
        },
        [&](int bi, TileSlot &s, hipStream_t compute) {
            return gs_espnet_forward_lane(h, bi % nl, s.in.d, GS_IN_U8_BGR_NHWC, s.count, height, width, mean, std, nullptr, s.out.d,
                                          s.hist.d, compute);
        },
        [&](int, TileSlot &s, hipStream_t compute) {
            uint8_t *hdst = out_pinned ? masks + (size_t)s.first * out_b : s.out.h;
            unsigned long long *hhdst = (out_pinned && hist) ? hist + (size_t)s.first * ncl : s.hist.h;
            const size_t hb = sizeof(unsigned long long) * ncl * s.count;
            if (!(pskip & 2))
                fail(hipMemcpy2DAsync(hdst, out_b, s.out.d, out_b, out_b, s.count, hipMemcpyDeviceToHost, compute), "D2H copy");
            if (hist || !out_pinned)
                fail(hipMemcpy2DAsync(hhdst, hb, s.hist.d, hb, hb, 1, hipMemcpyDeviceToHost, compute), "D2H copy");
        },
        [&](TileSlot &s) {
            if (out_pinned)
                return;
            parallel_memcpy(masks + (size_t)s.first * out_b, s.out.h, out_b * s.count);
            if (hist) std::memcpy(hist + (size_t)s.first * ncl, s.hist.h, sizeof(unsigned long long) * ncl * s.count);
        },
        stamp);
    return rc != GS_OK ? rc : gs_device_fault_check();
}

}
```

glomeruli_segmentation_amd/csrc/espnet_kernels.h:

```cpp
#pragma once
#include <type_traits>
#include "gs_internal.h"

namespace gs {

struct ActV {
    float *base;
    long long sn;
    int sc, pitch, off;
    int H, W;
};
static inline ActV view(const Act &a) { return ActV{a.base, a.sn, a.sc, a.pitch, a.off, a.H, a.W}; }

__device__ __forceinline__ float *at(const ActV &t, int n, int c, int y, int x)
{
    return t.base + (long long)n * t.sn + (long long)c * t.sc + t.off + y * t.pitch + x;
}
__device__ __forceinline__ float ldz(const ActV &t, int n, int c, int y, int x)
{
    const bool ok = (unsigned)y < (unsigned)t.H && (unsigned)x < (unsigned)t.W;
    const int yc = min(max(y, 0), t.H - 1), xc = min(max(x, 0), t.W - 1);
    const float v = *at(t, n, c, yc, xc);
    return ok ? v : 0.0f;
}
#ifndef NT_STEM_ST
#define NT_STEM_ST 1
#endif
#ifndef NT_DEC1_LD
#define NT_DEC1_LD 1
#endif
#ifndef NT_DEC2_LD
#define NT_DEC2_LD 1
#endif
#ifndef NT_DEC4_ST
#define NT_DEC4_ST 1
#endif
typedef float f32x2_t __attribute__((ext_vector_type(2)));
template <bool NT>
__device__ __forceinline__ float ld_stream(const float *p)
{
    return NT ? __builtin_nontemporal_load(p) : *p;
}
template <bool NT, typename T>
__device__ __forceinline__ void st_stream(T *p, T v)
{
    if (NT)
        __builtin_nontemporal_store(v, p);
    else
        *p = v;
}

__device__ __forceinline__ float prelu(float v, float alpha)
{
    return __builtin_amdgcn_fmed3f(v, alpha * v, alpha <= 1.0f ? __builtin_inff() : -__builtin_inff());
}
__device__ __forceinline__ float bn_prelu(float v, const float *bnp, int C, int c)
{
    return prelu(v * bnp[c] + bnp[C + c], bnp[2 * C + c]);
}
__device__ __forceinline__ float bn_prelu_sel(float v, const float *bnp, int C, int c)
{
    v = v * bnp[c] + bnp[C + c];
    return v > 0.0f ? v : bnp[2 * C + c] * v;
}

struct StemArgs {
    const void *in;
    float mean[3], std[3];
    float w1[432];
    float bn1[48];
    float b1[57];
    ActV a0;
    ActV inp1;
    unsigned long long *hist_zero;
    int hist_count;
    int N, H, W;
};

template <bool U8>
__device__ __forceinline__ float stem_fetch(const StemArgs &a, const float (*lut)[256], int n, int c, int y, int x)
{
    const bool ok = (unsigned)y < (unsigned)a.H && (unsigned)x < (unsigned)a.W;
    const int yc = min(max(y, 0), a.H - 1), xc = min(max(x, 0), a.W - 1);
    float v;
    if (U8)
        v = lut[c][static_cast<const unsigned char *>(a.in)[(((long long)n * a.H + yc) * a.W + xc) * 3 + c]];
    else
        v = static_cast<const float *>(a.in)[(((long long)n * 3 + c) * a.H + yc) * a.W + xc];
    return ok ? v : 0.0f;
}

constexpr int STEM_PX = 2;
#ifndef STEM_DWORD
#define STEM_DWORD 1
#endif
#ifndef STEM_LUT_COPIES
#define STEM_LUT_COPIES 1
#endif
template <bool U8>
__global__ void __launch_bounds__(256) stem_kernel(const StemArgs a)
{
    constexpr int NC = (U8 && STEM_DWORD) ? STEM_LUT_COPIES : 1;
    __shared__ float lut[3][256 * NC];
    if (U8) {
#pragma unroll
        for (int c = 0; c < 3; ++c) {
            float v = (float)threadIdx.x;
            v = v - a.mean[c];
            v = v / a.std[c];
            v = v / 255.0f;
#pragma unroll
            for (int k = 0; k < NC; ++k)
                lut[c][threadIdx.x * NC + k] = v;
        }
        __syncthreads();
    }
    if (a.hist_zero && blockIdx.x == 0)
        for (int i = threadIdx.x; i < a.hist_count; i += 256)
            a.hist_zero[i] = 0ull;
    const int H1 = a.H / 2, W1 = a.W / 2;
    const int W1p = (W1 + STEM_PX - 1) / STEM_PX;
    const long long idx = (long long)blockIdx.x * 256 + threadIdx.x;
    if (idx >= (long long)a.N * H1 * W1p)
        return;
    const int x = (int)(idx % W1p) * STEM_PX;
    const int y = (int)((idx / W1p) % H1);
    const int n = (int)(idx / ((long long)W1p * H1));
    const bool two = x + 1 < W1;

    float v[3][3][2 * STEM_PX + 1];
    if (U8 && STEM_DWORD) {
        const unsigned char *img = static_cast<const unsigned char *>(a.in) + (long long)n * a.H * a.W * 3;
        const int cp = (threadIdx.x & (NC - 1));
        unsigned d[3][4];
#pragma unroll
        for (int ky = 0; ky < 3; ++ky) {
            const int yy = min(max(2 * y - 1 + ky, 0), a.H - 1);
            const unsigned *row = reinterpret_cast<const unsigned *>(img + (long long)yy * a.W * 3) + (x > 0 ? (6 * x - 4) / 4 : 0);
            d[ky][0] = row[0];
            d[ky][1] = row[1];
            d[ky][2] = row[2];
            d[ky][3] = row[3];
            if (x == 0) {
                d[ky][3] = d[ky][2];
                d[ky][2] = d[ky][1];
                d[ky][1] = d[ky][0];
                d[ky][0] = 0u;
            }
        }
        const bool top = y == 0, left = x == 0;
#pragma unroll
        for (int ky = 0; ky < 3; ++ky)
#pragma unroll
            for (int kx = 0; kx < 2 * STEM_PX + 1; ++kx)
#pragma unroll
                for (int c = 0; c < 3; ++c) {
                    const int pos = 1 + kx * 3 + c;
                    const unsigned b = (d[ky][pos >> 2] >> (8 * (pos & 3))) & 0xffu;
                    float t = lut[c][b * NC + cp];
                    if ((ky == 0 && top) || (kx == 0 && left))
                        t = 0.0f;
                    v[c][ky][kx] = t;
                }
    } else if (!U8 && STEM_DWORD) {
        const float *img = static_cast<const float *>(a.in) + (long long)n * 3 * a.H * a.W;
        const bool top = y == 0, left = x == 0;
#pragma unroll
        for (int c = 0; c < 3; ++c)
#pragma unroll
            for (int ky = 0; ky < 3; ++ky) {
                const int yy = max(2 * y - 1 + ky, 0);
                const float *row = img + ((long long)c * a.H + yy) * a.W + (left ? 0 : 2 * x - 1);
                float r[5];
#pragma unroll
                for (int kx = 0; kx < 5; ++kx)
                    r[kx] = row[kx];
#pragma unroll
                for (int kx = 0; kx < 5; ++kx) {
                    float t = left ? (kx > 0 ? r[kx - 1] : 0.0f) : r[kx];
                    if (ky == 0 && top)
                        t = 0.0f;
                    v[c][ky][kx] = t;
                }
            }
    } else {
#pragma unroll
        for (int c = 0; c < 3; ++c)
#pragma unroll
            for (int ky = 0; ky < 3; ++ky)
#pragma unroll
                for (int kx = 0; kx < 2 * STEM_PX + 1; ++kx)
                    v[c][ky][kx] = stem_fetch<U8>(a, reinterpret_cast<const float(*)[256]>(&lut[0][0]), n, c, 2 * y - 1 + ky, 2 * x - 1 + kx);
    }

    float outv[19][STEM_PX], poolv[3][STEM_PX];
#pragma unroll
    for (int o = 0; o < 16; ++o) {
        float s[STEM_PX];
#pragma unroll
        for (int q = 0; q < STEM_PX; ++q)
            s[q] = 0.0f;
#pragma unroll
        for (int c = 0; c < 3; ++c)
#pragma unroll
            for (int ky = 0; ky < 3; ++ky)
#pragma unroll
                for (int kx = 0; kx < 3; ++kx) {
                    const float wgt = a.w1[((o * 3 + c) * 3 + ky) * 3 + kx];
#pragma unroll
                    for (int q = 0; q < STEM_PX; ++q)
                        s[q] = fmaf(wgt, v[c][ky][2 * q + kx], s[q]);
                }
#pragma unroll
        for (int q = 0; q < STEM_PX; ++q)
            outv[o][q] = bn_prelu_sel(bn_prelu_sel(s[q], a.bn1, 16, o), a.b1, 19, o);
    }
#pragma unroll
    for (int c = 0; c < 3; ++c)
#pragma unroll
        for (int q = 0; q < STEM_PX; ++q) {
            float s = 0.0f;
#pragma unroll
            for (int ky = 0; ky < 3; ++ky)
#pragma unroll
                for (int kx = 0; kx < 3; ++kx)
                    s += v[c][ky][2 * q + kx];
            s = s / 9.0f;
            poolv[c][q] = s;
            outv[16 + c][q] = bn_prelu_sel(s, a.b1, 19, 16 + c);
        }
#pragma unroll
    for (int o = 0; o < 19; ++o) {
        if (two)
            st_stream<NT_STEM_ST>(reinterpret_cast<f32x2_t *>(at(a.a0, n, o, y, x)), f32x2_t{outv[o][0], outv[o][1]});
        else
            st_stream<NT_STEM_ST>(at(a.a0, n, o, y, x), outv[o][0]);
    }
#pragma unroll
    for (int c = 0; c < 3; ++c) {
        if (two)
            st_stream<NT_STEM_ST>(reinterpret_cast<f32x2_t *>(at(a.inp1, n, c, y, x)), f32x2_t{poolv[c][0], poolv[c][1]});
        else
            st_stream<NT_STEM_ST>(at(a.inp1, n, c, y, x), poolv[c][0]);
    }
}

__global__ void __launch_bounds__(256)
pool_kernel(const ActV in, const ActV out, int N, int C, const float *bnp2, const ActV out2, int coff2, int C2)
{
    const long long idx = (long long)blockIdx.x * 256 + threadIdx.x;
    if (idx >= (long long)N * C * out.H * out.W)
        return;
    const int x = (int)(idx % out.W);
    const int y = (int)((idx / out.W) % out.H);
    const int c = (int)((idx / ((long long)out.W * out.H)) % C);
    const int n = (int)(idx / ((long long)out.W * out.H * C));
    float s = 0.0f;
#pragma unroll
    for (int ky = 0; ky < 3; ++ky)
#pragma unroll
        for (int kx = 0; kx < 3; ++kx)
            s += ldz(in, n, c, 2 * y - 1 + ky, 2 * x - 1 + kx);
    s = s / 9.0f;
    *at(out, n, c, y, x) = s;
    if (bnp2)
        *at(out2, n, coff2 + c, y, x) = bn_prelu(s, bnp2, C2, coff2 + c);
}

__global__ void __launch_bounds__(256)
cat_b2_kernel(const ActV o1, const ActV o10, const ActV inp2, const float *bnp, const ActV out, int N)
{
    const long long idx = (long long)blockIdx.x * 256 + threadIdx.x;
    if (idx >= (long long)N * 131 * out.H * out.W)
        return;
    const int x = (int)(idx % out.W);
    const int y = (int)((idx / out.W) % out.H);
    const int c = (int)((idx / ((long long)out.W * out.H)) % 131);
    const int n = (int)(idx / ((long long)out.W * out.H * 131));
    const float v = c < 64 ? *at(o1, n, c, y, x) : c < 128 ? *at(o10, n, c - 64, y, x) : *at(inp2, n, c - 128, y, x);
    *at(out, n, c, y, x) = bn_prelu(v, bnp, 131, c);
}

template <int CLS>
__device__ __forceinline__ int real_classes(int classes)
{
    return CLS == 5 ? 5 : classes;
}
template <int CLS>
__device__ __forceinline__ void zero_padding_lanes(float *s, int ncls)
{
    if constexpr (CLS != 5) {
#pragma unroll
        for (int k = 0; k < CLS; ++k)
            s[k] = k < ncls ? s[k] : 0.0f;
    }
}
template <int CLS>
constexpr int dec1_record() { return (3 + CLS + 3) / 4 * 4; }
template <int CLS>
constexpr int dec2_record() { return (CLS + 3) / 4 * 4; }

struct Dec1Args {
    ActV c0, clast;
    const float *b3w;
    const float *br;
    const float *wup;
    ActV out;
    float *enc_logits;
    int N;
    int classes;
};

template <int CLS, int CB>
__global__ void __launch_bounds__(256) dec1_kernel(const Dec1Args a)
{
    const int H3 = a.c0.H, W3 = a.c0.W;
    __shared__ float part[3][CLS][64];
    const int lane = threadIdx.x & 63, w = __builtin_amdgcn_readfirstlane(threadIdx.x >> 6);
    const long long total = (long long)a.N * H3 * W3;
    long long idx = (long long)blockIdx.x * 64 + lane;
    const bool active = idx < total;
    if (!active)
        idx = total - 1;
    const int x = (int)(idx % W3);
    const int y = (int)((idx / W3) % H3);
    const int n = (int)(idx / ((long long)W3 * H3));
    float s[CLS];
#pragma unroll
    for (int k = 0; k < CLS; ++k)
        s[k] = 0.0f;
    const long long pix = (long long)n * a.c0.sn + a.c0.off + y * a.c0.pitch + x;
    const float *plane0 = (w < 2 ? a.c0.base : a.clast.base) + pix + (long long)((w & 1) * 64) * a.c0.sc;
    auto fetch = [&](int c0, float *dst) {
#pragma unroll
        for (int j = 0; j < CB; ++j)
            dst[j] = ld_stream<NT_DEC1_LD>(plane0 + (long long)(c0 + j) * a.c0.sc);
    };
    float cur[CB], nxt[CB];
    fetch(0, cur);
    for (int c0 = 0; c0 < 64; c0 += CB) {
        if (c0 + CB < 64)
            fetch(c0 + CB, nxt);
        __builtin_amdgcn_sched_barrier(0);
#pragma unroll
        for (int j = 0; j < CB; ++j) {
            const float *pc = a.b3w + (w * 64 + c0 + j) * dec1_record<CLS>();
            const float t = cur[j] * pc[0] + pc[1];
            const float v = prelu(t, pc[2]);
#pragma unroll
            for (int k = 0; k < CLS; ++k)
                s[k] = fmaf(pc[3 + k], v, s[k]);
        }
#pragma unroll
        for (int j = 0; j < CB; ++j)
            cur[j] = nxt[j];
    }
    if (w > 0) {
#pragma unroll
        for (int k = 0; k < CLS; ++k)
            part[w - 1][k][lane] = s[k];
    }
    __syncthreads();
    if (w > 0 || !active)
        return;
#pragma unroll
    for (int k = 0; k < CLS; ++k)
        s[k] = (s[k] + part[0][k][lane]) + (part[1][k][lane] + part[2][k][lane]);
    const int ncls = real_classes<CLS>(a.classes);
    if (a.enc_logits) {
#pragma unroll
        for (int k = 0; k < CLS; ++k)
            if (k < ncls)
                a.enc_logits[(((long long)n * ncls + k) * H3 + y) * W3 + x] = s[k];
        return;
    }
#pragma unroll
    for (int k = 0; k < CLS; ++k)
        s[k] = s[k] * a.br[k] + a.br[CLS + k];
    zero_padding_lanes<CLS>(s, ncls);
    if constexpr (CLS != 5) {
        for (int o = 0; o < ncls; ++o) {
            float t[4] = {0.0f, 0.0f, 0.0f, 0.0f};
#pragma unroll
            for (int i = 0; i < CLS; ++i)
#pragma unroll
                for (int k = 0; k < 4; ++k)
                    t[k] = fmaf(s[i], a.wup[(i * CLS + o) * 4 + k], t[k]);
            *reinterpret_cast<float2 *>(at(a.out, n, o, 2 * y, 2 * x)) = make_float2(t[0], t[1]);
            *reinterpret_cast<float2 *>(at(a.out, n, o, 2 * y + 1, 2 * x)) = make_float2(t[2], t[3]);
        }
        return;
    }
    float up[CLS][2][2];
#pragma unroll
    for (int o = 0; o < CLS; ++o)
#pragma unroll
        for (int dy = 0; dy < 2; ++dy)
#pragma unroll
            for (int dx = 0; dx < 2; ++dx) {
                float t = 0.0f;
#pragma unroll
                for (int i = 0; i < CLS; ++i)
                    t = fmaf(s[i], a.wup[((i * CLS + o) * 2 + dy) * 2 + dx], t);
                up[o][dy][dx] = t;
            }
#pragma unroll
    for (int o = 0; o < CLS; ++o)
#pragma unroll
        for (int dy = 0; dy < 2; ++dy)
            *reinterpret_cast<float2 *>(at(a.out, n, o, 2 * y + dy, 2 * x)) = make_float2(up[o][dy][0], up[o][dy][1]);
}

struct Dec1SumsArgs {
    const float *part;
    long long psn;
    int psc;
    const float *br;
    const float *wup;
    ActV out;
    int N, H3, W3;
    int classes;
};

template <int CLS>
__global__ void __launch_bounds__(256) dec1_sums_kernel(const Dec1SumsArgs a)
{
    const long long idx = (long long)blockIdx.x * 256 + threadIdx.x;
    if (idx >= (long long)a.N * a.H3 * a.W3)
        return;
    const int x = (int)(idx % a.W3);
    const int y = (int)((idx / a.W3) % a.H3);
    const int n = (int)(idx / ((long long)a.W3 * a.H3));
    const float *pp = a.part + (long long)n * a.psn + y * a.W3 + x;
    float g[4][CLS];
#pragma unroll
    for (int j = 0; j < 4; ++j)
#pragma unroll
        for (int k = 0; k < CLS; ++k)
            g[j][k] = pp[(long long)(j * CLS + k) * a.psc];
    float s[CLS];
#pragma unroll
    for (int k = 0; k < CLS; ++k) {
        s[k] = (g[0][k] + g[1][k]) + (g[2][k] + g[3][k]);
        s[k] = s[k] * a.br[k] + a.br[CLS + k];
    }
    zero_padding_lanes<CLS>(s, real_classes<CLS>(a.classes));
    float up[CLS][2][2];
#pragma unroll
    for (int o = 0; o < CLS; ++o)
#pragma unroll
        for (int dy = 0; dy < 2; ++dy)
#pragma unroll
            for (int dx = 0; dx < 2; ++dx) {
                float t = 0.0f;
#pragma unroll
                for (int i = 0; i < CLS; ++i)
                    t = fmaf(s[i], a.wup[((i * CLS + o) * 2 + dy) * 2 + dx], t);
                up[o][dy][dx] = t;
            }
#pragma unroll
    for (int o = 0; o < CLS; ++o)
#pragma unroll
        for (int dy = 0; dy < 2; ++dy)
            *reinterpret_cast<float2 *>(at(a.out, n, o, 2 * y + dy, 2 * x)) = make_float2(up[o][dy][0], up[o][dy][1]);
}

struct Dec2Args {
    ActV a1;
    ActV raw;
    const float *b2;
    int raw_c0, raw_cn;
    ActV o2c;
    const float *w3c;
    const float *br;
    ActV t;
    int N;
    int classes;
};

template <int CLS>
__global__ void __launch_bounds__(256) dec2_kernel(const Dec2Args a)
{
    const int H2 = a.a1.H, W2 = a.a1.W;
    __shared__ float part[3][CLS][64];
    const int lane = threadIdx.x & 63, w = __builtin_amdgcn_readfirstlane(threadIdx.x >> 6);
    const long long total = (long long)a.N * H2 * W2;
    long long idx = (long long)blockIdx.x * 64 + lane;
    const bool active = idx < total;
    if (!active)
        idx = total - 1;
    const int x = (int)(idx % W2);
    const int y = (int)((idx / W2) % H2);
    const int n = (int)(idx / ((long long)W2 * H2));
    float s[CLS];
#pragma unroll
    for (int k = 0; k < CLS; ++k)
        s[k] = 0.0f;
    const int cb = 32 * w;
    if (cb >= a.raw_c0 && cb < a.raw_c0 + a.raw_cn) {
#pragma unroll 16
        for (int c = cb; c < cb + 32; ++c) {
            const float v = bn_prelu(ld_stream<NT_DEC2_LD>(at(a.raw, n, c - a.raw_c0, y, x)), a.b2, 131, c);
            const float *pc = a.w3c + c * dec2_record<CLS>();
#pragma unroll
            for (int k = 0; k < CLS; ++k)
                s[k] = fmaf(pc[k], v, s[k]);
        }
    } else {
#pragma unroll 16
        for (int c = cb; c < cb + 32; ++c) {
            const float v = ld_stream<NT_DEC2_LD>(at(a.a1, n, c, y, x));
            const float *pc = a.w3c + c * dec2_record<CLS>();
#pragma unroll
            for (int k = 0; k < CLS; ++k)
                s[k] = fmaf(pc[k], v, s[k]);
        }
    }
    if (w == 3) {
#pragma unroll
        for (int c = 128; c < 131; ++c) {
            const float v = ld_stream<NT_DEC2_LD>(at(a.a1, n, c, y, x));
            const float *pc = a.w3c + c * dec2_record<CLS>();
#pragma unroll
            for (int k = 0; k < CLS; ++k)
                s[k] = fmaf(pc[k], v, s[k]);
        }
    }
    if (w > 0) {
#pragma unroll
        for (int k = 0; k < CLS; ++k)
            part[w - 1][k][lane] = s[k];
    }
    __syncthreads();
    if (w > 0 || !active)
        return;
#pragma unroll
    for (int k = 0; k < CLS; ++k)
        s[k] = (s[k] + part[0][k][lane]) + (part[1][k][lane] + part[2][k][lane]);
    float tv[2 * CLS];
#pragma unroll
    for (int k = 0; k < CLS; ++k) {
        tv[k] = bn_prelu(s[k], a.br, 2 * CLS, k);
        tv[CLS + k] = bn_prelu(*at(a.o2c, n, k, y, x), a.br, 2 * CLS, CLS + k);
    }
    const int ncls = real_classes<CLS>(a.classes);
#pragma unroll
    for (int k = 0; k < 2 * CLS; ++k)
        if (k % CLS < ncls)
            *at(a.t, n, k, y, x) = tv[k];
}

template <int CLS>
__global__ void __launch_bounds__(256) dec2_br_kernel(const Dec2Args a)
{
    const int H2 = a.t.H, W2 = a.t.W;
    const long long idx = (long long)blockIdx.x * 256 + threadIdx.x;
    if (idx >= (long long)a.N * H2 * W2)
        return;
    const int x = (int)(idx % W2);
    const int y = (int)((idx / W2) % H2);
    const int n = (int)(idx / ((long long)W2 * H2));
    const int ncls = real_classes<CLS>(a.classes);
#pragma unroll
    for (int k = 0; k < CLS; ++k)
        if (k < ncls) {
            *at(a.t, n, k, y, x) = bn_prelu(*at(a.a1, n, k, y, x), a.br, 2 * CLS, k);
            *at(a.t, n, CLS + k, y, x) = bn_prelu(*at(a.o2c, n, k, y, x), a.br, 2 * CLS, CLS + k);
        }
}

struct Dec3Args {
    ActV t;
    const float *wc;
    const float *bnc;
    const float *wup;
    const float *bnu;
    ActV e;
    int N;
    int classes;
};

template <int CLS>
__global__ void __launch_bounds__(256) dec3_kernel(const Dec3Args a)
{
    const int H2 = a.t.H, W2 = a.t.W;
    const long long idx = (long long)blockIdx.x * 256 + threadIdx.x;
    if (idx >= (long long)a.N * H2 * W2)
        return;
    const int x = (int)(idx % W2);
    const int y = (int)((idx / W2) % H2);
    const int n = (int)(idx / ((long long)W2 * H2));
    float s[CLS];
#pragma unroll
    for (int k = 0; k < CLS; ++k)
        s[k] = 0.0f;
    const int ncls = real_classes<CLS>(a.classes);
    for (int c = 0; c < 2 * CLS; ++c) {
        if (CLS != 5 && c % CLS >= ncls)
            continue;
#pragma unroll
        for (int ky = 0; ky < 3; ++ky)
#pragma unroll
            for (int kx = 0; kx < 3; ++kx) {
                const float v = ldz(a.t, n, c, y - 1 + ky, x - 1 + kx);
#pragma unroll
                for (int k = 0; k < CLS; ++k)
                    s[k] = fmaf(CLS == 5 ? a.wc[((k * 2 * CLS + c) * 3 + ky) * 3 + kx] : a.wc[((c * 3 + ky) * 3 + kx) * CLS + k], v, s[k]);
            }
    }
#pragma unroll
    for (int k = 0; k < CLS; ++k)
        s[k] = bn_prelu(s[k], a.bnc, CLS, k);
    zero_padding_lanes<CLS>(s, ncls);
    float up[CLS][2][2];
#pragma unroll
    for (int o = 0; o < CLS; ++o)
#pragma unroll
        for (int dy = 0; dy < 2; ++dy)
#pragma unroll
            for (int dx = 0; dx < 2; ++dx) {
                float t = 0.0f;
#pragma unroll
                for (int i = 0; i < CLS; ++i)
                    t = fmaf(s[i], a.wup[((i * CLS + o) * 2 + dy) * 2 + dx], t);
                up[o][dy][dx] = bn_prelu(t, a.bnu, CLS, o);
            }
#pragma unroll
    for (int o = 0; o < CLS; ++o)
#pragma unroll
        for (int dy = 0; dy < 2; ++dy)
            if (o < ncls)
                *reinterpret_cast<float2 *>(at(a.e, n, o, 2 * y + dy, 2 * x)) = make_float2(up[o][dy][0], up[o][dy][1]);
}

template <int CLS>
__global__ void __launch_bounds__(256) dec3b_kernel(const Dec3Args a)
{
    const int H2 = a.t.H, W2 = a.t.W;
    const long long idx = (long long)blockIdx.x * 256 + threadIdx.x;
    if (idx >= (long long)a.N * H2 * W2)
        return;
    const int x = (int)(idx % W2);
    const int y = (int)((idx / W2) % H2);
    const int n = (int)(idx / ((long long)W2 * H2));
    const int ncls = real_classes<CLS>(a.classes);
    float s[CLS];
#pragma unroll
    for (int k = 0; k < CLS; ++k)
        s[k] = *at(a.t, n, k, y, x);
    zero_padding_lanes<CLS>(s, ncls);
    for (int o = 0; o < ncls; ++o) {
        float t[4] = {0.0f, 0.0f, 0.0f, 0.0f};
#pragma unroll
        for (int i = 0; i < CLS; ++i)
#pragma unroll
            for (int k = 0; k < 4; ++k)
                t[k] = fmaf(s[i], a.wup[(i * CLS + o) * 4 + k], t[k]);
#pragma unroll
        for (int k = 0; k < 4; ++k)
            t[k] = bn_prelu(t[k], a.bnu, CLS, o);
        *reinterpret_cast<float2 *>(at(a.e, n, o, 2 * y, 2 * x)) = make_float2(t[0], t[1]);
        *reinterpret_cast<float2 *>(at(a.e, n, o, 2 * y + 1, 2 * x)) = make_float2(t[2], t[3]);
    }
}

struct Dec4Args {
    ActV f;
    const float *wcl;
    float *logits;
    unsigned char *mask;
    unsigned long long *hist;
    float *prob;
    int ens_mode;
    float ens_w;
    int N;
    int classes;
};

template <int CLS>
constexpr int dec4_px() { return CLS <= 8 ? 4 : CLS <= 12 ? 2 : 1; }
template <int CLS, bool ENS>
__global__ void __launch_bounds__(256) dec4_kernel(const Dec4Args a)
{
    __shared__ unsigned int lhist[CLS];
    const int H1 = a.f.H, W1 = a.f.W;
    const int H = 2 * H1, W = 2 * W1;
    const int n = blockIdx.y;
    const int ncls = real_classes<CLS>(a.classes);
    constexpr int DEC4_PX = dec4_px<CLS>();
    __shared__ float wl[CLS * CLS * 4];
    for (int i = threadIdx.x; i < CLS * CLS * 4; i += 256)
        wl[i] = a.wcl[i];
    if (threadIdx.x < CLS)
        lhist[threadIdx.x] = 0;
    __syncthreads();
    int cls_of[DEC4_PX][4];
    float s[DEC4_PX][CLS];
    bool live[DEC4_PX];
    int xs[DEC4_PX], ys[DEC4_PX];
#pragma unroll
    for (int q = 0; q < DEC4_PX; ++q) {
        const int idx = (blockIdx.x * DEC4_PX + q) * 256 + threadIdx.x;
        live[q] = idx < H1 * W1;
        const int ic = live[q] ? idx : 0;
        xs[q] = ic % W1;
        ys[q] = ic / W1;
#pragma unroll
        for (int k = 0; k < CLS; ++k)
            s[q][k] = *at(a.f, n, k, ys[q], xs[q]);
        zero_padding_lanes<CLS>(s[q], ncls);
    }
#pragma unroll
    for (int q = 0; q < DEC4_PX; ++q) {
        const int x = xs[q], y = ys[q];
#pragma unroll
        for (int dy = 0; dy < 2; ++dy) {
            unsigned char m[2];
#pragma unroll
            for (int dx = 0; dx < 2; ++dx) {
                float best = 0.0f;
                int bi = 0;
                float lg[CLS];
#pragma unroll
                for (int o = 0; o < CLS; ++o) {
                    float t = 0.0f;
#pragma unroll
                    for (int i = 0; i < CLS; ++i)
                        t = fmaf(s[q][i], wl[((i * CLS + o) * 2 + dy) * 2 + dx], t);
                    lg[o] = t;
                    if (!ENS && o < ncls && (o == 0 || t > best)) {
                        best = t;
                        bi = o;
                    }
                }
                const long long pix = ((long long)(2 * y + dy)) * W + 2 * x + dx;
                if (ENS) {
                    float mx = -3.4e38f;
#pragma unroll
                    for (int o = 0; o < CLS; ++o)
                        if (o < ncls)
                            mx = fmaxf(mx, lg[o]);
                    float sum = 0.0f;
#pragma unroll
                    for (int o = 0; o < CLS; ++o)
                        if (o < ncls) {
                            lg[o] = expf(lg[o] - mx);
                            sum += lg[o];
                        }
                    bool first = true;
#pragma unroll
                    for (int o = 0; o < CLS; ++o)
                        if (o < ncls && live[q]) {
                            float pr = lg[o] / sum * a.ens_w;
                            float *pp = a.prob + ((long long)n * ncls + o) * H * W + pix;
                            if (a.ens_mode == 2 || a.ens_mode == 3)
                                pr = *pp + pr;
                            if (a.ens_mode == 1 || a.ens_mode == 2)
                                *pp = pr;
                            else if (first || pr > best) {
                                best = pr;
                                bi = o;
                            }
                            first = false;
                        }
                } else if (a.logits && live[q]) {
#pragma unroll
                    for (int o = 0; o < CLS; ++o)
                        if (o < ncls)
                            a.logits[((long long)n * ncls + o) * H * W + pix] = lg[o];
                }
                m[dx] = (unsigned char)bi;
                cls_of[q][dy * 2 + dx] = live[q] ? bi : -1;
            }
            if (a.mask && live[q] && (!ENS || a.ens_mode >= 3))
                st_stream<NT_DEC4_ST>(reinterpret_cast<unsigned short *>(a.mask + ((long long)n * H + 2 * y + dy) * W + 2 * x),
                                      (unsigned short)(m[0] | (m[1] << 8)));
        }
    }
    if (a.hist && (!ENS || a.ens_mode >= 3)) {
#pragma unroll
        for (int k = 0; k < CLS; ++k) {
            unsigned cnt = 0;
#pragma unroll
            for (int q = 0; q < DEC4_PX; ++q)
#pragma unroll
                for (int j = 0; j < 4; ++j)
                    cnt += (unsigned)__popcll(__ballot(cls_of[q][j] == k));
            if ((threadIdx.x & 63) == 0 && cnt)
                atomicAdd(&lhist[k], cnt);
        }
        __syncthreads();
        if (threadIdx.x < ncls && lhist[threadIdx.x])
            atomicAdd(&a.hist[(long long)n * ncls + threadIdx.x], (unsigned long long)lhist[threadIdx.x]);
    }
}

__global__ void __launch_bounds__(256) b2_apply_kernel(float *chw, const float *b2, int hw, int c0, int cn)
{
    const long long idx = (long long)blockIdx.x * 256 + threadIdx.x;
    if (idx >= (long long)cn * hw)
        return;
    const int c = c0 + (int)(idx / hw);
    float *p = chw + (long long)c0 * hw + idx;
    *p = bn_prelu(*p, b2, 131, c);
}

__global__ void __launch_bounds__(256) unpad_kernel(const ActV t, int n, int C, float *dst)
{
    const long long idx = (long long)blockIdx.x * 256 + threadIdx.x;
    if (idx >= (long long)C * t.H * t.W)
        return;
    const int x = (int)(idx % t.W);
    const int y = (int)((idx / t.W) % t.H);
    const int c = (int)(idx / ((long long)t.W * t.H));
    dst[idx] = *at(t, n, c, y, x);
}

__global__ void __launch_bounds__(256) pad_kernel(const ActV t, int n, int C, const float *src)
{
    const long long idx = (long long)blockIdx.x * 256 + threadIdx.x;
    if (idx >= (long long)C * t.H * t.W)
        return;
    const int x = (int)(idx % t.W);
    const int y = (int)((idx / t.W) % t.H);
    const int c = (int)(idx / ((long long)t.W * t.H));
    *at(t, n, c, y, x) = src[idx];
}

}
```

glomeruli_segmentation_amd/csrc/forward_plan.h:

```cpp
#pragma once
#include "espnet_config.h"

namespace gs {

constexpr int cfg_pixels(int, int, int, int, int, int, int, int, int p, int) { return p; }

constexpr int dec_mt(int cp) { return cp <= 16 ? 16 : 32; }
constexpr int dec_pixels(int cp) { return cp <= 16 ? 8 : 4; }

#define GS_FORMS_L2_DOWN(X)                              \
    X(P2S_VEC, "CFG_L2_BR_P2S+F_VEC", cfg_pixels(CFG_L2_BR_P2S))                                  \
    X(P4S_VEC_SKIP, "CFG_L2_BR_P4S+F_VEC+F_SKIP_PAD", cfg_pixels(CFG_L2_BR_P4S))                  \
    X(P4_VEC, "CFG_L2_BR_P4+F_VEC", cfg_pixels(CFG_L2_BR_P4))                                     \
    X(P4, "CFG_L2_BR_P4", 0)                                                                      \
    X(UNFUSED_P4_VEC, "unfused CFG_L2_BR_P4+F_VEC", cfg_pixels(CFG_L2_BR_P4))                     \
    X(UNFUSED_P4, "unfused CFG_L2_BR_P4", 0)
#define GS_FORMS_L2_ESP_FUSED(X)                        \
    X(P2S_VEC, "CFG_L2_BR_P2S+F_VEC", cfg_pixels(CFG_L2_BR_P2S))                                  \
    X(P4_VEC, "CFG_L2_BR_P4+F_VEC", cfg_pixels(CFG_L2_BR_P4))                                     \
    X(P4, "CFG_L2_BR_P4", 0)                                                                      \
    X(UNFUSED_P4_VEC, "unfused CFG_L2_BR_P4+F_VEC", cfg_pixels(CFG_L2_BR_P4))                     \
    X(UNFUSED_P4, "unfused CFG_L2_BR_P4", 0)
#define GS_FORMS_L2_ESP_LAST(X)             \
    X(P2S_VEC, "CFG_L2_BR_P2S+F_VEC", cfg_pixels(CFG_L2_BR_P2S))                                  \
    X(P4_VEC, "CFG_L2_BR_P4+F_VEC", cfg_pixels(CFG_L2_BR_P4))                                     \
    X(P4, "CFG_L2_BR_P4", 0)
#define GS_FORMS_CAT_B2(X)                            \
    X(KERNEL, "cat_b2_kernel", 0)
#define GS_FORMS_L3_REDUCE(X)                                    \
    X(BNL_P1, "CFG_L3_C1S_BNL_P1", 0)                                                             \
    X(BNL, "CFG_L3_C1S_BNL", 0)                                                                   \
    X(C1S, "CFG_L3_C1S", 0)
#define GS_FORMS_L3_DOWN(X)                              \
    X(P1R, "CFG_L3_BR_P1R", 0)                                                                    \
    X(P2R_VEC, "CFG_L3_BR_P2R+F_VEC", cfg_pixels(CFG_L3_BR_P2R))                                  \
    X(BR_VEC, "CFG_L3_BR+F_VEC", cfg_pixels(CFG_L3_BR))                                           \
    X(P2F, "CFG_L3_BR_P2F", 0)                                                                    \
    X(UNFUSED_BR_VEC, "unfused CFG_L3_BR+F_VEC", cfg_pixels(CFG_L3_BR))                           \
    X(UNFUSED_BR, "unfused CFG_L3_BR", 0)
#define GS_FORMS_L3_ESP_FUSED(X)    \
    X(P1R, "CFG_L3_BR_P1R", 0)                                                                    \
    X(P2R_VEC, "CFG_L3_BR_P2R+F_VEC", cfg_pixels(CFG_L3_BR_P2R))                                  \
    X(P2F, "CFG_L3_BR_P2F", 0)
#define GS_FORMS_L3_ESP_LAST(X)                      \
    X(P1R, "CFG_L3_BR_P1R", 0)                                                                    \
    X(P2R_VEC, "CFG_L3_BR_P2R+F_VEC", cfg_pixels(CFG_L3_BR_P2R))                                  \
    X(BR_VEC, "CFG_L3_BR+F_VEC", cfg_pixels(CFG_L3_BR))                                           \
    X(P2, "CFG_L3_BR_P2", 0)
#define GS_FORMS_DEC3(X)                                     \
    X(KERNEL, "dec3_kernel", 0)                                                                   \
    X(MT16, "MFMA MT16", 0)                                                                       \
    X(MT16_VEC, "MFMA MT16+F_VEC", dec_pixels(16))                                                \
    X(MT32, "MFMA MT32", 0)                                                                       \
    X(MT32_VEC, "MFMA MT32+F_VEC", dec_pixels(20))
#define GS_FORMS_DEC_CONV(X)                           \
    X(TAIL, "dec_tail_kernel", 0)                                                                 \
    X(MT16, "MFMA MT16", 0)                                                                       \
    X(MT16_VEC, "MFMA MT16+F_VEC", dec_pixels(16))                                                \
    X(MT32, "MFMA MT32", 0)                                                                       \
    X(MT32_VEC, "MFMA MT32+F_VEC", dec_pixels(20))
#define GS_LAUNCH_CLASSES(C)               \
    C(l2_down, GS_FORMS_L2_DOWN)           \
    C(l2_esp_fused, GS_FORMS_L2_ESP_FUSED) \
    C(l2_esp_last, GS_FORMS_L2_ESP_LAST)   \
    C(cat_b2, GS_FORMS_CAT_B2)             \
    C(l3_reduce, GS_FORMS_L3_REDUCE)       \
    C(l3_down, GS_FORMS_L3_DOWN)           \
    C(l3_esp_fused, GS_FORMS_L3_ESP_FUSED) \
    C(l3_esp_last, GS_FORMS_L3_ESP_LAST)   \
    C(dec3, GS_FORMS_DEC3)                 \
    C(dec_conv, GS_FORMS_DEC_CONV)

struct FormInfo {
    const char *name;
    int pixels_per_lane;
};
struct LaunchClassInfo {
    const char *name;
    const FormInfo *forms;
    int n_forms;
};

#define GS_FORM_ID(id, name, ppl) id,
#define GS_FORM_INFO(id, name, ppl) {name, ppl},
#define GS_CLASS_ENUM(cls, FORMS) enum class cls : int { none = -1, FORMS(GS_FORM_ID) };
#define GS_CLASS_FORMS(cls, FORMS)                                          \
    constexpr FormInfo kForms_##cls[] = {FORMS(GS_FORM_INFO)};              \
    constexpr int pixels_per_lane(form::cls f) { return kForms_##cls[(int)f].pixels_per_lane; }
#define GS_CLASS_INFO(cls, FORMS) {#cls, kForms_##cls, (int)(sizeof kForms_##cls / sizeof kForms_##cls[0])},
#define GS_PLAN_MEMBER(cls, FORMS) form::cls cls = form::cls::none;
#define GS_PLAN_CODE(cls, FORMS) *out++ = (int)cls;
namespace form {
GS_LAUNCH_CLASSES(GS_CLASS_ENUM)
}
GS_LAUNCH_CLASSES(GS_CLASS_FORMS)
constexpr LaunchClassInfo kLaunchClasses[] = {GS_LAUNCH_CLASSES(GS_CLASS_INFO)};
constexpr int kLaunchClassCount = (int)(sizeof kLaunchClasses / sizeof kLaunchClasses[0]);

struct ForwardPlan {
    GS_LAUNCH_CLASSES(GS_PLAN_MEMBER)
    bool lazy_b2 = false;
    bool l3c_in_reduce = false;
    bool cls_in_l3 = false;
    void codes(int *out) const { GS_LAUNCH_CLASSES(GS_PLAN_CODE) }
};
#undef GS_FORM_ID
#undef GS_FORM_INFO
#undef GS_CLASS_ENUM
#undef GS_CLASS_FORMS
#undef GS_CLASS_INFO
#undef GS_PLAN_MEMBER
#undef GS_PLAN_CODE

template <typename F>
constexpr bool vec_fits(F v, int w, bool no_vec)
{
    return !no_vec && w % pixels_per_lane(v) == 0;
}

constexpr form::l2_down unfused_l2_down(int W2, bool no_vec)
{
    return vec_fits(form::l2_down::UNFUSED_P4_VEC, W2, no_vec) ? form::l2_down::UNFUSED_P4_VEC : form::l2_down::UNFUSED_P4;
}
constexpr form::l2_esp_fused unfused_l2_esp(int W2, bool no_vec)
{
    return vec_fits(form::l2_esp_fused::UNFUSED_P4_VEC, W2, no_vec) ? form::l2_esp_fused::UNFUSED_P4_VEC : form::l2_esp_fused::UNFUSED_P4;
}
constexpr form::l3_down unfused_l3_down(int W3, bool no_vec)
{
    return vec_fits(form::l3_down::UNFUSED_BR_VEC, W3, no_vec) ? form::l3_down::UNFUSED_BR_VEC : form::l3_down::UNFUSED_BR;
}
constexpr form::l3_esp_last whole_row_l3_esp(int W3, bool no_vec)
{
    return vec_fits(form::l3_esp_last::BR_VEC, W3, no_vec) ? form::l3_esp_last::BR_VEC : form::l3_esp_last::P2;
}

inline ForwardPlan plan_forward(int n, int H, int W, int p, int q, int cp, int num_cus, bool no_vec, bool encoder_only = false)
{
    namespace f = form;
    const int W1 = W / 2, H2 = H / 4, W2 = W / 4, H3 = H / 8, W3 = W / 8;
    const long long cus = num_cus;
    ForwardPlan pl;
    pl.lazy_b2 = b2_is_lazy(p);
    pl.l3c_in_reduce = !encoder_only && l3c_side_sums(cp);
    pl.cls_in_l3 = !encoder_only && cls_side_sums(cp, q);

    const bool small2 = CFG_SMALL2_WAVES > 0 && (long long)n * H2 * cdiv(W2, 64) * 2 <= cus * CFG_SMALL2_WAVES &&
                        vec_fits(f::l2_down::P2S_VEC, W2, no_vec);
    if (!l2_c1_fused(0, p))
        pl.l2_down = unfused_l2_down(W2, no_vec);
    else if (small2)
        pl.l2_down = f::l2_down::P2S_VEC;
    else if (CFG_L2_DOWN_SKIP && vec_fits(f::l2_down::P4S_VEC_SKIP, W2, no_vec))
        pl.l2_down = f::l2_down::P4S_VEC_SKIP;
    else
        pl.l2_down = vec_fits(f::l2_down::P4_VEC, W2, no_vec) ? f::l2_down::P4_VEC : f::l2_down::P4;
    if (p > 1) {
        if (!l2_c1_fused(1, p))
            pl.l2_esp_fused = unfused_l2_esp(W2, no_vec);
        else if (small2)
            pl.l2_esp_fused = f::l2_esp_fused::P2S_VEC;
        else
            pl.l2_esp_fused = vec_fits(f::l2_esp_fused::P4_VEC, W2, no_vec) ? f::l2_esp_fused::P4_VEC : f::l2_esp_fused::P4;
    }
    if (p > 0)
        pl.l2_esp_last = small2                                            ? f::l2_esp_last::P2S_VEC
                         : vec_fits(f::l2_esp_last::P4_VEC, W2, no_vec) ? f::l2_esp_last::P4_VEC
                                                                          : f::l2_esp_last::P4;
    if (!pl.lazy_b2)
        pl.cat_b2 = f::cat_b2::KERNEL;

    if (!pl.lazy_b2)
        pl.l3_reduce = f::l3_reduce::C1S;
    else
        pl.l3_reduce = (long long)n * H3 * cdiv(W3, 128) * 4 <= cus * 8 ? f::l3_reduce::BNL_P1 : f::l3_reduce::BNL;
    const bool small3 = (long long)n * H3 * cdiv(W3, 64) * 2 <= cus * CFG_SMALL3_WAVES && !no_vec;
    if (!l3_c1_fused(0, q))
        pl.l3_down = unfused_l3_down(W3, no_vec);
    else if (small3)
        pl.l3_down = f::l3_down::P1R;
    else if (CFG_L3_DOWN_P2 && vec_fits(f::l3_down::P2R_VEC, W3, no_vec))
        pl.l3_down = f::l3_down::P2R_VEC;
    else
        pl.l3_down = !pl.cls_in_l3 && vec_fits(f::l3_down::BR_VEC, W3, no_vec) ? f::l3_down::BR_VEC : f::l3_down::P2F;
    if (q > 1 && l3_c1_fused(1, q))
        pl.l3_esp_fused = small3                                              ? f::l3_esp_fused::P1R
                          : vec_fits(f::l3_esp_fused::P2R_VEC, W3, no_vec) ? f::l3_esp_fused::P2R_VEC
                                                                             : f::l3_esp_fused::P2F;
    if (q > 0) {
        if (small3)
            pl.l3_esp_last = f::l3_esp_last::P1R;
        else if (CFG_L3_LAST_P2 && vec_fits(f::l3_esp_last::P2R_VEC, W3, no_vec))
            pl.l3_esp_last = f::l3_esp_last::P2R_VEC;
        else
            pl.l3_esp_last = whole_row_l3_esp(W3, no_vec);
    }

    if (!dec3_on_mfma(cp))
        pl.dec3 = f::dec3::KERNEL;
    else if (dec_mt(cp) == 16)
        pl.dec3 = vec_fits(f::dec3::MT16_VEC, W2, no_vec) ? f::dec3::MT16_VEC : f::dec3::MT16;
    else
        pl.dec3 = vec_fits(f::dec3::MT32_VEC, W2, no_vec) ? f::dec3::MT32_VEC : f::dec3::MT32;
    if (dec_tail_fused(cp))
        pl.dec_conv = f::dec_conv::TAIL;
    else if (dec_mt(cp) == 16)
        pl.dec_conv = vec_fits(f::dec_conv::MT16_VEC, W1, no_vec) ? f::dec_conv::MT16_VEC : f::dec_conv::MT16;
    else
        pl.dec_conv = vec_fits(f::dec_conv::MT32_VEC, W1, no_vec) ? f::dec_conv::MT32_VEC : f::dec_conv::MT32;
    return pl;
}

}
```

glomeruli_segmentation_amd/engine.py:

```python
import ctypes
import functools

import numpy as np
import torch

from . import _lib


def _to_numpy(v):
    if isinstance(v, torch.Tensor):
        return v.detach().cpu().numpy()
    return np.asarray(v)


def pack_state_dict(state_dict):
    items = []
    total = 0
    for name, v in state_dict.items():
        a = _to_numpy(v)
        if a.dtype.kind != "f":
            continue
        a = np.ascontiguousarray(a, dtype=np.float32)
        if a.ndim > 4:
            raise ValueError("tensor %s has %d dims" % (name, a.ndim))
        items.append((name, a, total))
        total += a.size
    blob = np.empty(total, dtype=np.float32)
    table = (_lib.LayerDesc * len(items))()
    for i, (name, a, off) in enumerate(items):
        blob[off:off + a.size] = a.ravel()
        enc = name.encode()
        if len(enc) >= 96:
            raise ValueError("tensor name too long: " + name)
        table[i].name = enc
        table[i].offset = off
        table[i].ndim = a.ndim
        for d in range(a.ndim):
            table[i].shape[d] = a.shape[d]
    return blob, table


def _check_out(t, name, shape, dtype, device):
    if t is None:
        return
    if not isinstance(t, torch.Tensor) or tuple(t.shape) != tuple(shape) or t.dtype != dtype or not t.is_contiguous() or \
            t.device.type != torch.device(device).type or (t.is_cuda and t.device != torch.device(device)):
        raise ValueError("%s must be a contiguous %s tensor of shape %s on %s" % (name, dtype, tuple(shape), device))


def _stream_ptr(device):
    return ctypes.c_void_p(torch.cuda.current_stream(device).cuda_stream)


class EspnetEngine:

    def __init__(self, state_dict, classes=5, p=2, q=8, encoder_only=False, device=None, lanes=1):
        if not torch.cuda.is_available():
            raise RuntimeError("EspnetEngine needs a HIP device (torch.cuda.is_available() is False); "
                               "there is no CPU path in this build")
        self.lib = _lib.load()
        self.device = torch.device("cuda", torch.cuda.current_device() if device is None else
                                   torch.device(device).index or 0)
        self.classes, self.p, self.q, self.encoder_only = classes, p, q, encoder_only
        blob, table = pack_state_dict(state_dict)
        h = ctypes.c_void_p()
        with torch.cuda.device(self.device):
            _lib.check(self.lib.gs_espnet_create(blob.ctypes.data_as(ctypes.c_void_p), table, len(table), classes, p,
                                                 q, 1 if encoder_only else 0, ctypes.byref(h)))
        self.handle = h
        self.lanes = 1
        self._lane_streams = {}
        if lanes != 1:
            self.set_lanes(lanes)

    def set_lanes(self, n):
        with torch.cuda.device(self.device):
            _lib.check(self.lib.gs_espnet_set_lanes(self.handle, int(n)))
        self.lanes = int(n)

    def lane_stream(self, lane):
        if not 0 <= lane < self.lanes:
            raise ValueError("lane %d of %d" % (lane, self.lanes))
        if lane not in self._lane_streams:
            self._lane_streams[lane] = torch.cuda.Stream(device=self.device)
        return self._lane_streams[lane]

    def wait_lanes(self):
        cur = torch.cuda.current_stream(self.device)
        for st in self._lane_streams.values():
            cur.wait_stream(st)

    def quiesce(self):
        for st in self._lane_streams.values():
            st.synchronize()
        torch.cuda.current_stream(self.device).synchronize()

    def check_device_faults(self):
        with torch.cuda.device(self.device):
            _lib.check(self.lib.gs_device_fault_check())

    def close(self):
        if getattr(self, "handle", None):
            with torch.cuda.device(self.device):
                self.lib.gs_espnet_destroy(self.handle)
            self.handle = None

    def __del__(self):
        try:
            self.close()
        except Exception:
            pass

    def reserve(self, n, height, width):
        with torch.cuda.device(self.device):
            _lib.check(self.lib.gs_espnet_reserve(self.handle, n, height, width))

    def forward_logits(self, x):
        if x.dtype != torch.float32 or x.dim() != 4 or x.shape[1] != 3 or not x.is_cuda:
            raise ValueError("expected a float32 [N,3,H,W] tensor on the GPU")
        x = x.contiguous()
        n, _, h, w = x.shape
        oh, ow = (h // 8, w // 8) if self.encoder_only else (h, w)
        out = torch.empty((n, self.classes, oh, ow), dtype=torch.float32, device=x.device)
        with torch.cuda.device(x.device):
            _lib.check(self.lib.gs_espnet_forward(self.handle, x.data_ptr(), _lib.GS_IN_F32_NCHW, n, h, w, None, None,
                                                  out.data_ptr(), None, None, _stream_ptr(x.device)))
        return out

    def segment(self, tiles_u8, mean, std, want_logits=False, want_hist=True, out_mask=None, out_hist=None, lane=None,
                want_enc_logits=False):
        if tiles_u8.dtype != torch.uint8 or tiles_u8.dim() != 4 or tiles_u8.shape[3] != 3 or not tiles_u8.is_cuda:
            raise ValueError("expected a uint8 [N,H,W,3] tensor on the GPU")
        if want_enc_logits and not self.encoder_only:
            raise ValueError("want_enc_logits: the 1/8-scale logits are an output of ESPNet-C engines only")
        if want_logits and self.encoder_only:
            raise ValueError("want_logits: an ESPNet-C engine has no full-resolution logits (want_enc_logits=True gives the 1/8-scale ones)")
        want_logits = bool(want_logits or want_enc_logits)
        tiles_u8 = tiles_u8.contiguous()
        n, h, w, _ = tiles_u8.shape
        dev = tiles_u8.device
        _check_out(out_mask, "out_mask", (n, h, w), torch.uint8, dev)
        _check_out(out_hist, "out_hist", (n, self.classes), torch.int64, dev)
        mask = out_mask if out_mask is not None else torch.empty((n, h, w), dtype=torch.uint8, device=dev)
        hist = None
        if want_hist:
            hist = out_hist if out_hist is not None else torch.empty((n, self.classes), dtype=torch.int64, device=dev)
        lh, lw = (h // 8, w // 8) if self.encoder_only else (h, w)
        logits = torch.empty((n, self.classes, lh, lw), dtype=torch.float32, device=dev) if want_logits else None
        with torch.cuda.device(dev):
            if lane is None:
                if 0 in self._lane_streams:
                    torch.cuda.current_stream(dev).wait_stream(self._lane_streams[0])
                k, sp = 0, _stream_ptr(dev)
            else:
                st = self.lane_stream(lane)
                st.wait_stream(torch.cuda.current_stream(dev))
                for t in (tiles_u8, mask, hist, logits):
                    if t is not None:
                        t.record_stream(st)
                k, sp = lane, ctypes.c_void_p(st.cuda_stream)
            _lib.check(self.lib.gs_espnet_forward_lane(
                self.handle, k, tiles_u8.data_ptr(), _lib.GS_IN_U8_BGR_NHWC, n, h, w, _lib.fptr3(mean), _lib.fptr3(std),
                logits.data_ptr() if want_logits else None, mask.data_ptr(),
                hist.data_ptr() if want_hist else None, sp))
        return mask, hist, logits

    def segment_host(self, tiles, mean, std, batch=32, want_hist=True, out_masks=None, out_hist=None):
        self.quiesce()
        if isinstance(tiles, torch.Tensor):
            if tiles.is_cuda or tiles.dtype != torch.uint8 or not tiles.is_contiguous():
                raise ValueError("expected a contiguous uint8 CPU tensor")
            t, h, w, _ = tiles.shape
            in_ptr = ctypes.c_void_p(tiles.data_ptr())
            pin = tiles.is_pinned()
            _check_out(out_masks, "out_masks", (t, h, w), torch.uint8, torch.device("cpu"))
            _check_out(out_hist, "out_hist", (t, self.classes), torch.int64, torch.device("cpu"))
            masks_t = out_masks if out_masks is not None else torch.empty((t, h, w), dtype=torch.uint8, pin_memory=pin)
            hist_t = None
            if want_hist:
                hist_t = out_hist if out_hist is not None else torch.zeros((t, self.classes), dtype=torch.int64, pin_memory=pin)
            with torch.cuda.device(self.device):
                _lib.check(self.lib.gs_espnet_segment_host(
                    self.handle, in_ptr, t, h, w, _lib.fptr3(mean), _lib.fptr3(std), batch, ctypes.c_void_p(masks_t.data_ptr()),
                    ctypes.c_void_p(hist_t.data_ptr()) if want_hist else None))
            return masks_t.numpy(), (hist_t.numpy() if want_hist else None)
        tiles = np.ascontiguousarray(tiles, dtype=np.uint8)
        t, h, w, _ = tiles.shape
        masks = np.empty((t, h, w), dtype=np.uint8)
        hist = np.zeros((t, self.classes), dtype=np.uint64) if want_hist else None
        with torch.cuda.device(self.device):
            _lib.check(self.lib.gs_espnet_segment_host(
                self.handle, tiles.ctypes.data_as(ctypes.c_void_p), t, h, w, _lib.fptr3(mean), _lib.fptr3(std), batch,
                masks.ctypes.data_as(ctypes.c_void_p), hist.ctypes.data_as(ctypes.c_void_p) if want_hist else None))
        return masks, (hist.astype(np.int64) if want_hist else None)

    scores_crops = True

    def segment_crops(self, crops, mean, std, net_h=512, net_w=1024, batch=32, **kw):
        return segment_crops_host([self], [(mean, std)], crops, net_h, net_w, batch, **kw)

    def segment_crops_resident(self, packed_in, descs, mean, std, net_h=512, net_w=1024, want_net_maps=True, want_hist=True,
                               packed_out=None, paste=None, lane=None):
        n = len(descs)
        dev = packed_in.device
        tab = (_lib.CropDesc * n)(*descs)
        net = torch.empty((n, net_h, net_w), dtype=torch.uint8, device=dev) if want_net_maps else None
        hist = torch.empty((n, self.classes), dtype=torch.int64, device=dev) if want_hist else None
        with torch.cuda.device(dev):
            if lane is None:
                if 0 in self._lane_streams:
                    torch.cuda.current_stream(dev).wait_stream(self._lane_streams[0])
                k, sp = 0, _stream_ptr(dev)
            else:
                st = self.lane_stream(lane)
                st.wait_stream(torch.cuda.current_stream(dev))
                for t in (packed_in, packed_out, net, hist):
                    if t is not None:
                        t.record_stream(st)
                k, sp = lane, ctypes.c_void_p(st.cuda_stream)
            _lib.check(self.lib.gs_espnet_segment_crops(
                self.handle, k, packed_in.data_ptr(), tab, n, _lib.fptr3(mean), _lib.fptr3(std), net_h, net_w,
                net.data_ptr() if net is not None else None, packed_out.data_ptr() if packed_out is not None else None,
                hist.data_ptr() if hist is not None else None, ctypes.byref(paste) if paste is not None else None, sp))
        return net, hist

    def read_stage(self, name, image=0):
        dims = (ctypes.c_int * 3)()
        _lib.check(self.lib.gs_espnet_read_stage(self.handle, name.encode(), image, None, 0, ctypes.byref(dims)))
        out = np.empty(tuple(dims), dtype=np.float32)
        with torch.cuda.device(self.device):
            _lib.check(self.lib.gs_espnet_read_stage(self.handle, name.encode(), image,
                                                     out.ctypes.data_as(ctypes.c_void_p), out.size, ctypes.byref(dims)))
        return out

    def block_forward(self, kind, level, index, x):
        x = np.ascontiguousarray(x, dtype=np.float32)
        c, h, w = x.shape
        cout = 64 if level == 2 else 128
        out = np.empty((cout, h, w) if kind == 0 else (cout, h // 2, w // 2), dtype=np.float32)
        with torch.cuda.device(self.device):
            _lib.check(self.lib.gs_espnet_block_forward(self.handle, kind, level, index, x.ctypes.data_as(ctypes.c_void_p),
                                                        h, w, out.ctypes.data_as(ctypes.c_void_p)))
        return out

    def profile(self, on):
        _lib.check(self.lib.gs_espnet_profile_enable(self.handle, 1 if on else 0))

    def profile_read(self):
        arr = (_lib.KernelTime * 32)()
        n = ctypes.c_int()
        with torch.cuda.device(self.device):
            _lib.check(self.lib.gs_espnet_profile_read(self.handle, arr, 32, ctypes.byref(n)))
        return [{"name": arr[i].name.decode(), "total_ms": arr[i].total_ms, "launches": arr[i].launches,
                 "flops_per_tile": arr[i].flops_per_tile} for i in range(n.value)]


@functools.lru_cache(maxsize=None)
def forward_forms():
    lib = _lib.load()
    table = []
    name, ppl = ctypes.c_char_p(), ctypes.c_int()
    while lib.gs_espnet_form_info(len(table), _lib.GS_FORM_NONE, ctypes.byref(name), ctypes.byref(ppl)) == _lib.GS_OK:
        k, cls, forms = len(table), name.value.decode(), []
        while lib.gs_espnet_form_info(k, len(forms), ctypes.byref(name), ctypes.byref(ppl)) == _lib.GS_OK:
            forms.append((name.value.decode(), ppl.value))
        table.append((cls, tuple(forms)))
    return tuple(table)


def plan_forward(n, height, width, p, q, classes, num_cus):
    lib = _lib.load()
    table = forward_forms()
    codes, count = (ctypes.c_int * len(table))(), ctypes.c_int()
    _lib.check(lib.gs_espnet_plan_forward(n, height, width, p, q, classes, num_cus, codes, len(table), ctypes.byref(count)))
    return {cls: forms[codes[k]][0] for k, (cls, forms) in enumerate(table) if codes[k] != _lib.GS_FORM_NONE}


def plan_flags(n, height, width, p, q, classes, num_cus, encoder_only=False):
    flags = ctypes.c_int()
    _lib.check(_lib.load().gs_espnet_plan_flags(n, height, width, p, q, classes, int(bool(encoder_only)), num_cus, ctypes.byref(flags)))
    return {"lazy_b2": bool(flags.value & _lib.GS_PLAN_LAZY_B2), "l3c_in_reduce": bool(flags.value & _lib.GS_PLAN_L3C_IN_REDUCE)}


def plan_cls_in_l3(n, height, width, p, q, classes, num_cus, encoder_only=False):
    flags = ctypes.c_int()
    _lib.check(_lib.load().gs_espnet_plan_flags(n, height, width, p, q, classes, int(bool(encoder_only)), num_cus, ctypes.byref(flags)))
    return bool(flags.value & _lib.GS_PLAN_CLS_IN_L3)


def pack_weights(state_dict, classes=5, p=2, q=8, encoder_only=False):
    lib = _lib.load()
    src, table = pack_state_dict(state_dict)
    head = (src.ctypes.data_as(ctypes.c_void_p), table, len(table), classes, p, q, int(bool(encoder_only)))
    n, n_pieces = ctypes.c_size_t(), ctypes.c_int()
    _lib.check(lib.gs_espnet_pack_weights(*head, None, 0, ctypes.byref(n), None, 0, ctypes.byref(n_pieces)))
    blob, pieces = np.empty(n.value, dtype=np.float32), (_lib.WeightPiece * n_pieces.value)()
    _lib.check(lib.gs_espnet_pack_weights(*head, blob.ctypes.data_as(ctypes.c_void_p), blob.size, ctypes.byref(n), pieces, len(pieces),
                                          ctypes.byref(n_pieces)))
    return blob, {pc.name.decode(): (pc.offset, pc.floats) for pc in pieces}


def workspace_bytes(n, height, width, p, q, classes, encoder_only=False):
    b = ctypes.c_size_t()
    _lib.check(_lib.load().gs_espnet_workspace_plan(n, height, width, p, q, classes, int(bool(encoder_only)), ctypes.byref(b)))
    return b.value


def crop_preprocess(crop_u8, mean, std, out_h, out_w, out=None):
    lib = _lib.load()
    crop_u8 = crop_u8.contiguous()
    h, w, _ = crop_u8.shape
    if out is None:
        out = torch.empty((3, out_h, out_w), dtype=torch.float32, device=crop_u8.device)
    with torch.cuda.device(crop_u8.device):
        _lib.check(lib.gs_crop_preprocess(crop_u8.data_ptr(), h, w, _lib.fptr3(mean), _lib.fptr3(std), out_h, out_w,
                                          out.data_ptr(), _stream_ptr(crop_u8.device)))
    return out


def mask_resize_nearest(mask, out_h, out_w):
    lib = _lib.load()
    mask = mask.contiguous()
    h, w = mask.shape
    out = torch.empty((out_h, out_w), dtype=torch.uint8, device=mask.device)
    with torch.cuda.device(mask.device):
        _lib.check(lib.gs_mask_resize_nearest(mask.data_ptr(), h, w, out_h, out_w, out.data_ptr(), _stream_ptr(mask.device)))
    return out


def paste_target(slide_map, ds=8, luts=None):
    if slide_map.dtype != torch.uint8 or slide_map.dim() != 2 or not slide_map.is_cuda or not slide_map.is_contiguous():
        raise ValueError("slide_map must be a contiguous uint8 [map_h,map_w] tensor on the GPU")
    t = _lib.PasteTarget()
    t.slide_map = slide_map.data_ptr()
    t.map_h, t.map_w, t.ds = int(slide_map.shape[0]), int(slide_map.shape[1]), int(ds)
    t.sx_lut = luts[0].data_ptr() if luts is not None else None
    t.sy_lut = luts[1].data_ptr() if luts is not None else None
    return t


def seen_values(seen_words):
    bits = np.unpackbits(np.ascontiguousarray(seen_words, dtype="<u8").view(np.uint8), bitorder="little")
    return np.nonzero(bits)[0].astype(np.uint8)


def score_crops_resident(net_masks, packed_labels, descs, classes, want_seen=True):
    lib = _lib.load()
    n, net_h, net_w = (int(v) for v in net_masks.shape)
    if n != len(descs):
        raise ValueError("%d masks for %d descriptors" % (n, len(descs)))
    if net_masks.dtype != torch.uint8 or packed_labels.dtype != torch.uint8 or not net_masks.is_contiguous() or not packed_labels.is_contiguous():
        raise ValueError("expected contiguous uint8 GPU tensors")
    need = max(int(d.out_off) + int(d.h) * int(d.w) for d in descs)
    if packed_labels.numel() < need:
        raise ValueError("packed_labels holds %d bytes, the descriptors reach %d" % (packed_labels.numel(), need))
    dev = net_masks.device
    tab = (_lib.CropDesc * n)(*descs)
    conf = torch.empty((n, classes, classes), dtype=torch.int64, device=dev)
    seen = torch.empty((n, 4), dtype=torch.int64, device=dev) if want_seen else None
    with torch.cuda.device(dev):
        _lib.check(lib.gs_espnet_score_crops(net_masks.data_ptr(), packed_labels.data_ptr(), tab, n, net_h, net_w, classes,
                                             conf.data_ptr(), seen.data_ptr() if seen is not None else None, _stream_ptr(dev)))
    return conf, seen


def segment_crops_host(engines, mean_stds, crops, net_h=512, net_w=1024, batch=32, want_masks=True, want_net_maps=False,
                       want_hist=True, paste=None, origins=None, overlay=None, labels=None, want_gt_overlay=False):
    lib = _lib.load()
    n = len(crops)
    if labels is not None and len(labels) != n:
        raise ValueError("%d labels for %d crops" % (len(labels), n))
    if want_gt_overlay and (labels is None or overlay is None):
        raise ValueError("want_gt_overlay needs labels and overlay")
    if n == 0:
        return {"masks": [] if want_masks else None, "net_maps": None, "counts": None, "overlays": [] if overlay is not None else None,
                "conf": None, "seen": [] if labels is not None else None, "gt_overlays": [] if want_gt_overlay else None}
    keep = []
    ptrs = (ctypes.c_void_p * n)()
    hs, ws = (ctypes.c_int * n)(), (ctypes.c_int * n)()
    for i, c in enumerate(crops):
        if isinstance(c, torch.Tensor):
            if c.is_cuda or c.dtype != torch.uint8 or c.dim() != 3 or c.shape[2] != 3 or not c.is_contiguous():
                raise ValueError("crop %d: expected a contiguous uint8 [h,w,3] CPU tensor" % i)
            ptrs[i] = c.data_ptr()
        else:
            c = np.ascontiguousarray(c, dtype=np.uint8)
            if c.ndim != 3 or c.shape[2] != 3:
                raise ValueError("crop %d: expected uint8 [h,w,3]" % i)
            ptrs[i] = c.ctypes.data
        keep.append(c)
        hs[i], ws[i] = int(c.shape[0]), int(c.shape[1])
    eng0 = engines[0]
    handles = (ctypes.c_void_p * len(engines))(*[e.handle for e in engines])
    means = (ctypes.c_float * (3 * len(engines)))(*[float(v) for ms in mean_stds for v in ms[0]])
    stds = (ctypes.c_float * (3 * len(engines)))(*[float(v) for ms in mean_stds for v in ms[1]])
    out_ptrs, out_buf, offs = None, None, None
    if want_masks:
        sizes = [int(hs[i]) * int(ws[i]) for i in range(n)]
        offs = np.zeros(n + 1, dtype=np.int64)
        np.cumsum([(s + 255) // 256 * 256 for s in sizes], out=offs[1:])
        out_buf = torch.empty(int(offs[-1]), dtype=torch.uint8, pin_memory=True)
        base = out_buf.data_ptr()
        out_ptrs = (ctypes.c_void_p * n)(*[base + int(offs[i]) for i in range(n)])
    net = torch.empty((n, net_h, net_w), dtype=torch.uint8, pin_memory=True) if want_net_maps else None
    hist = torch.zeros((n, eng0.classes), dtype=torch.int64, pin_memory=True) if want_hist else None
    x1 = y1 = None
    if paste is not None:
        if origins is None or len(origins) != n:
            raise ValueError("paste needs one (x1, y1) level-0 origin per crop")
        x1 = (ctypes.c_int * n)(*[int(o[0]) for o in origins])
        y1 = (ctypes.c_int * n)(*[int(o[1]) for o in origins])
    ov, ov_buf, ov_offs, pal = None, None, None, None
    if overlay is not None:
        palette, wa, wb = overlay
        pal = np.ascontiguousarray(palette, dtype=np.uint8).reshape(-1, 3)
        ov_offs = np.zeros(n + 1, dtype=np.int64)
        np.cumsum([(int(hs[i]) * int(ws[i]) * 3 + 255) // 256 * 256 for i in range(n)], out=ov_offs[1:])
        ov_buf = torch.empty(int(ov_offs[-1]), dtype=torch.uint8, pin_memory=True)
        ov = _lib.CropOverlay()
        ov.palette_rgb = pal.ctypes.data
        ov.n_colours = int(pal.shape[0])
        ov.wa, ov.wb = float(wa), float(wb)
        ov_ptrs = (ctypes.c_void_p * n)(*[ov_buf.data_ptr() + int(ov_offs[i]) for i in range(n)])
        ov.out_bgr = ctypes.cast(ov_ptrs, ctypes.POINTER(ctypes.c_void_p))
        keep.append(ov_ptrs)
    sc, conf, seen, gt_buf = None, None, None, None
    if labels is not None:
        lab_ptrs = (ctypes.c_void_p * n)()
        for i, lb in enumerate(labels):
            if not isinstance(lb, np.ndarray) or lb.dtype != np.uint8 or lb.shape != (int(hs[i]), int(ws[i])):
                raise ValueError("label %d: expected a uint8 [%d,%d] array" % (i, int(hs[i]), int(ws[i])))
            lb = np.ascontiguousarray(lb)
            keep.append(lb)
            lab_ptrs[i] = lb.ctypes.data
        conf = np.zeros((n, eng0.classes, eng0.classes), dtype=np.uint64)
        seen = np.zeros((n, 4), dtype=np.uint64)
        sc = _lib.CropScoring()
        sc.labels = ctypes.cast(lab_ptrs, ctypes.POINTER(ctypes.c_void_p))
        sc.conf, sc.seen = conf.ctypes.data, seen.ctypes.data
        sc.gt_clamp = 1
        keep.append(lab_ptrs)
        if want_gt_overlay:
            gt_buf = torch.empty(int(ov_offs[-1]), dtype=torch.uint8, pin_memory=True)
            gt_ptrs = (ctypes.c_void_p * n)(*[gt_buf.data_ptr() + int(ov_offs[i]) for i in range(n)])
            sc.gt_overlay_bgr = ctypes.cast(gt_ptrs, ctypes.POINTER(ctypes.c_void_p))
            keep.append(gt_ptrs)
    for e in engines:
        e.quiesce()
    args = (handles, len(engines), ptrs, hs, ws, n, means, stds, net_h, net_w, batch, out_ptrs,
            ctypes.c_void_p(net.data_ptr()) if net is not None else None,
            ctypes.c_void_p(hist.data_ptr()) if hist is not None else None,
            ctypes.byref(paste) if paste is not None else None, x1, y1, ctypes.byref(ov) if ov is not None else None)
    with torch.cuda.device(eng0.device):
        if sc is None:
            _lib.check(lib.gs_espnet_segment_crops_host(*args))
        else:
            _lib.check(lib.gs_espnet_segment_crops_host_scored(*args, ctypes.byref(sc)))
    masks = None
    if want_masks:
        flat = out_buf.numpy()
        masks = [flat[int(offs[i]):int(offs[i]) + int(hs[i]) * int(ws[i])].reshape(int(hs[i]), int(ws[i])) for i in range(n)]
    overlays = None
    if ov is not None:
        flat = ov_buf.numpy()
        overlays = [flat[int(ov_offs[i]):int(ov_offs[i]) + int(hs[i]) * int(ws[i]) * 3].reshape(int(hs[i]), int(ws[i]), 3) for i in range(n)]
    gt_overlays = None
    if gt_buf is not None:
        flat = gt_buf.numpy()
        gt_overlays = [flat[int(ov_offs[i]):int(ov_offs[i]) + int(hs[i]) * int(ws[i]) * 3].reshape(int(hs[i]), int(ws[i]), 3) for i in range(n)]
    return {"masks": masks, "net_maps": net.numpy() if net is not None else None,
            "counts": hist.numpy() if hist is not None else None, "overlays": overlays,
            "conf": conf.astype(np.int64) if conf is not None else None,
            "seen": [seen_values(seen[i]) for i in range(n)] if seen is not None else None, "gt_overlays": gt_overlays}


def ensemble_segment(engines, tiles_u8, mean_stds):
    lib = _lib.load()
    tiles_u8 = tiles_u8.contiguous()
    n, h, w, _ = tiles_u8.shape
    dev = tiles_u8.device
    handles = (ctypes.c_void_p * len(engines))(*[e.handle for e in engines])
    means = (ctypes.c_float * (3 * len(engines)))(*[float(v) for ms in mean_stds for v in ms[0]])
    stds = (ctypes.c_float * (3 * len(engines)))(*[float(v) for ms in mean_stds for v in ms[1]])
    mask = torch.empty((n, h, w), dtype=torch.uint8, device=dev)
    hist = torch.empty((n, engines[0].classes), dtype=torch.int64, device=dev)
    with torch.cuda.device(dev):
        _lib.check(lib.gs_espnet_ensemble_forward(handles, len(engines), tiles_u8.data_ptr(), n, h, w, means, stds,
                                                  mask.data_ptr(), hist.data_ptr(), _stream_ptr(dev)))
    return mask, hist
```

Before: 11800 patches/s.

## Add lean mask-only forward: skip last level-3 store, fuse dec2 into dec3

When logits are not requested, the last level-3 branch launch keeps only its class side-sums and drops the full activation store. The dec2 concat/BN kernel is skipped, and a new dec3_cat_kernel reads the l3c and o2c planes directly, applying BN/PReLU on load, doing the 3x3 conv and the 2x upsample on 2x2 pixel blocks with vector stores. The pool kernel also now handles two output pixels per thread with float4 row loads. The intent is to cut memory traffic and launches in the decoder tail. The cost is more code paths and stages that can no longer be read in lean mode.

```diff
diff --git a/glomeruli_segmentation_amd/_lib.py b/glomeruli_segmentation_amd/_lib.py
--- a/glomeruli_segmentation_amd/_lib.py
+++ b/glomeruli_segmentation_amd/_lib.py
@@ -153,6 +153,10 @@
 }
 GS_PLAN_LAZY_B2, GS_PLAN_L3C_IN_REDUCE, GS_PLAN_CLS_IN_L3 = 1, 2, 4
 
+LEAN_PROTOTYPES = {
+    "gs_espnet_plan_lean": (_I, [_I] * 9 + [ctypes.POINTER(_I)]),
+}
+
 INSTANCE_PROTOTYPES = {
     "gs_instances_plan": (_I, [_I, _I, _I, _I, ctypes.POINTER(ctypes.c_size_t)]),
     "gs_slide_instances": (_I, [_P, _I, _I, _I, _I, _P, ctypes.c_size_t, _I, _P, _P, _P, _P, _P]),
@@ -182,8 +186,9 @@
             "(hipcc --offload-arch=gfx950).  There is no CPU fallback." % LIB_PATH)
     lib = ctypes.CDLL(LIB_PATH, mode=ctypes.RTLD_GLOBAL)
     for name, (res, args) in list(PROTOTYPES.items()) + list(SCORING_PROTOTYPES.items()) + list(PLAN_PROTOTYPES.items()) + \
-            list(INSTANCE_PROTOTYPES.items()) + list(MATCH_PROTOTYPES.items()) + list(BOUNDARY_PROTOTYPES.items()):
-        if name in PLAN_PROTOTYPES and not hasattr(lib, name):
+            list(INSTANCE_PROTOTYPES.items()) + list(MATCH_PROTOTYPES.items()) + list(BOUNDARY_PROTOTYPES.items()) + \
+            list(LEAN_PROTOTYPES.items()):
+        if (name in PLAN_PROTOTYPES or name in LEAN_PROTOTYPES) and not hasattr(lib, name):
             continue
         fn = getattr(lib, name)
         fn.restype = res
diff --git a/glomeruli_segmentation_amd/build.py b/glomeruli_segmentation_amd/build.py
--- a/glomeruli_segmentation_amd/build.py
+++ b/glomeruli_segmentation_amd/build.py
@@ -9,7 +9,7 @@
 SOURCES = ["espnet.hip", "dec_tail.hip", "crops.hip", "detect_ops.hip", "detector.hip", "wsi_eval.hip", "instances.hip", "instance_match.hip", "boundary_dist.hip", "contours.cpp"]
 HEADERS = ["gs_internal.h", "conv_mfma.h", "dec_tail.h", "dec_tail_args.h", "espnet_kernels.h", "espnet_facts.h", "espnet_weights.h", "workspace_plan.h", "crop_sample.h", "crop_plan.h", "wave_block.h", "slide_map_plan.h", "instance_plan.h", "instance_match_plan.h", "boundary_dist_plan.h", "detect_math.h", "detect_plan.h", "host_copy.h", "host_jobs.h", "host_pipe.h",
            os.path.join("..", "..", "include", "glomseg.h"), os.path.join("..", "..", "include", "glomseg_scoring.h"),
-           os.path.join("..", "..", "include", "glomseg_plan.h"), os.path.join("..", "..", "include", "glomseg_instances.h"),
+           os.path.join("..", "..", "include", "glomseg_plan.h"), os.path.join("..", "..", "include", "glomseg_lean.h"), os.path.join("..", "..", "include", "glomseg_instances.h"),
            os.path.join("..", "..", "include", "glomseg_instance_match.h"),
            os.path.join("..", "..", "include", "glomseg_boundary_dist.h")]
 FLAGS = ["-O3", "--offload-arch=gfx950", "-std=c++17", "-fPIC", "-Wall", "-Wno-unused-result",
diff --git a/glomeruli_segmentation_amd/csrc/conv_mfma.h b/glomeruli_segmentation_amd/csrc/conv_mfma.h
--- a/glomeruli_segmentation_amd/csrc/conv_mfma.h
+++ b/glomeruli_segmentation_amd/csrc/conv_mfma.h
@@ -178,6 +178,7 @@
 constexpr int F_SIDE_SHIFT = 27;
 constexpr int F_SIDE1X1(int classes) { return classes << F_SIDE_SHIFT; }
 constexpr int F_CLS1X1 = 256;
+constexpr int F_CLS_ONLY = 2048;
 constexpr int CLS_N = 5, CLS_REC = 8;
 constexpr int F_X_NOLOAD = 16;
 constexpr int F_X_NOLDS = 32;
@@ -212,7 +213,7 @@
 template <int MT, int WAVES, int CINP, int TAPS, int STRIDE, int NDIL, int NOUT1, int NOUT, int P, int G, int FLAGS>
 __global__ void __launch_bounds__(WAVES * 64, WAVES >= 8 ? WAVES / 8 : 2) conv_mfma_kernel(const ConvArgs a)
 {
-    constexpr bool BNACT = FLAGS & F_BNACT, RES = FLAGS & F_RES, STORE1 = !(FLAGS & F_NOSTORE), DUAL = FLAGS & F_DUAL;
+    constexpr bool BNACT = FLAGS & F_BNACT, RES = FLAGS & F_RES, STORE1 = !(FLAGS & (F_NOSTORE | F_CLS_ONLY)), DUAL = FLAGS & F_DUAL;
     constexpr bool S2P = FLAGS & F_S2PAIR;
     constexpr bool VEC = FLAGS & F_VEC;
     constexpr bool AGL = FLAGS & F_A_GLOBAL, FUSE = FLAGS & F_FUSE1X1;
@@ -225,6 +226,8 @@
     static_assert(!CLSF || (MT == 32 && NDIL == 5 && TAPS == 9 && (FLAGS & F_BNACT) && !(FLAGS & (F_DUAL | F_NOSTORE | F_BNLOAD | F_X_ALL)) &&
                             !SIDE && ((NOUT1 + (NDIL - 1) * NOUT) * CLS_REC) % 256 == 0 && (NOUT1 + (NDIL - 1) * NOUT) * CLS_REC / 256 <= WAVES),
                   "F_CLS1X1 is for the level-3 branch launches: 32-row accumulators, five slots, the records in whole DMA pieces");
+    static_assert(!(FLAGS & F_CLS_ONLY) || (CLSF && !(FLAGS & (F_FUSE1X1 | F_DUAL))),
+                  "F_CLS_ONLY drops the store of a launch whose class sums are its only output: F_CLS1X1 without a fused 1x1 or a second store");
     static_assert(!SIDE || ((FLAGS & F_S2PAIR) && TAPS == 9 && STRIDE == 2 && MT == 32 && NDIL == 1 && SCLS <= SIDE_REC &&
                             (CINP / M_KL_OF(MT)) % G == 0 && G * M_KL_OF(MT) <= SIDE_ZROWS && !(FLAGS & (F_A_GLOBAL | F_VEC | F_X_ALL))),
                   "F_SIDE1X1 is for the stride-2 3x3 reduce on 32-pixel runs, a tap row in whole chunks");
diff --git a/glomeruli_segmentation_amd/csrc/espnet.hip b/glomeruli_segmentation_amd/csrc/espnet.hip
--- a/glomeruli_segmentation_amd/csrc/espnet.hip
+++ b/glomeruli_segmentation_amd/csrc/espnet.hip
@@ -10,6 +10,7 @@
 #include <vector>
 
 #include "../../include/glomseg_plan.h"
+#include "../../include/glomseg_lean.h"
 #include "conv_mfma.h"
 #include "dec_tail_args.h"
 #include "enc_head.h"
@@ -83,6 +84,7 @@
     }
     int last_n = 0;
     bool b2_lazy = false;
+    bool lean = false;
 
     bool profile = false;
     struct Ev { hipEvent_t a, b; int k; };
@@ -323,8 +325,16 @@
     return not_planned("l3_esp_fused");
 }
 
-static gs_status launch_l3_esp_last(const Model *m, form::l3_esp_last f, bool cls5, const ConvArgs &ca, hipStream_t s)
-{
+static gs_status launch_l3_esp_last(const Model *m, form::l3_esp_last f, bool cls5, bool cls_only, const ConvArgs &ca, hipStream_t s)
+{
+    if (cls5 && cls_only)
+        switch (f) {
+        case form::l3_esp_last::P1R: return launch_conv_mfma<CFG_L3_BR_P1R, F_BNACT | F_RES | POL_L3_ESP | SKIP_L3 | (CFG_SMALL_AGL ? F_A_GLOBAL : 0) | F_CLS1X1 | F_CLS_ONLY>(ca, m->num_cus, s);
+        case form::l3_esp_last::P2R_VEC: return launch_conv_mfma<CFG_L3_BR_P2R, F_BNACT | F_RES | F_VEC | POL_L3_ESP | SKIP_L3 | F_CLS1X1 | F_CLS_ONLY>(ca, m->num_cus, s);
+        case form::l3_esp_last::BR_VEC: return launch_conv_mfma<CFG_L3_BR, F_BNACT | F_RES | F_VEC | POL_L3_ESP | F_CLS1X1 | F_CLS_ONLY>(ca, m->num_cus, s);
+        case form::l3_esp_last::P2: return launch_conv_mfma<CFG_L3_BR_P2, F_BNACT | F_RES | F_CLS1X1 | F_CLS_ONLY>(ca, m->num_cus, s);
+        case form::l3_esp_last::none: return not_planned("l3_esp_last");
+        }
     if (cls5)
         switch (f) {
         case form::l3_esp_last::P1R: return launch_conv_mfma<CFG_L3_BR_P1R, F_BNACT | F_RES | POL_L3_ESP | SKIP_L3 | (CFG_SMALL_AGL ? F_A_GLOBAL : 0) | F_CLS1X1>(ca, m->num_cus, s);
@@ -381,6 +391,7 @@
     const double px1 = (double)H1 * W1, px2 = (double)H2 * W2, px3 = (double)H3 * W3;
     m->stages.clear();
     m->last_n = n;
+    m->lean = plan.lean;
     L.run(K_STEM, px1 * (27 * 16 * 2), [&] {
         StemArgs a{};
         a.in = r.in;
@@ -405,7 +416,7 @@
         return GS_OK;
     });
     L.run(K_POOL, 0, [&] {
-        hipLaunchKernelGGL(pool_kernel, dim3(blocks_for((long long)n * 3 * H2 * W2)), dim3(256), 0, s, view(m->inp1),
+        hipLaunchKernelGGL(pool_kernel, dim3(blocks_for((long long)n * 3 * H2 * (W2 / POOL_PX))), dim3(256), 0, s, view(m->inp1),
                            view(m->inp2), n, 3, m->p > 0 ? wb + m->w.b2 : nullptr, view(m->a1), 128, 131);
         return GS_OK;
     });
@@ -535,12 +546,14 @@
             if (fuse_next)
                 return launch_l3_esp_fused(m, plan.l3_esp_fused, with_fused(ca, m->r3[rd3 ^ 1], 25), i, s);
             const bool cls5 = plan.cls_in_l3 && i == m->q - 1;
-            return launch_l3_esp_last(m, plan.l3_esp_last, cls5, cls5 ? with_cls(ca, 1) : ca, s);
+            return launch_l3_esp_last(m, plan.l3_esp_last, cls5, plan.lean, cls5 ? with_cls(ca, 1) : ca, s);
         });
         have_r3 = fuse_next;
         rd3 ^= have_r3 ? 1 : 0;
         cur3 = nxt;
         m->set_stage("level3." + std::to_string(i), m->cc[cur3], 128);
+        if (plan.lean && i == m->q - 1)
+            m->stages.erase("level3." + std::to_string(i));
     }
     return {cur3, lazy_b2};
 }
@@ -603,31 +616,38 @@
     }
     m->set_stage("up_l3", m->o2c, ncls);
 
-    L.run(K_DEC2, plan.l3c_in_reduce ? 0 : px2 * (131 * ncls * 2), [&] {
-        Dec2Args a{};
-        a.o2c = view(m->o2c);
-        a.br = wb + m->w.cbr0;
-        a.t = view(m->tt);
-        a.N = n;
-        a.classes = ncls;
-        if constexpr (l3c_side_sums(CLS)) {
-            if (plan.l3c_in_reduce) {
+    if constexpr (l3c_side_sums(CLS)) {
+        if (!plan.l3c_in_reduce) {
+            set_error("internal: a %d-class decoder without level3_C from the stride-2 reduce", CLS);
+            return GS_ERR_INVALID;
+        }
+    }
+    const bool cat_on_load = l3c_side_sums(CLS);
+    if (!plan.lean) {
+        L.run(K_DEC2, cat_on_load ? 0 : px2 * (131 * ncls * 2), [&] {
+            Dec2Args a{};
+            a.o2c = view(m->o2c);
+            a.br = wb + m->w.cbr0;
+            a.t = view(m->tt);
+            a.N = n;
+            a.classes = ncls;
+            if constexpr (l3c_side_sums(CLS)) {
                 a.a1 = view(m->l3c);
                 hipLaunchKernelGGL(dec2_br_kernel<CLS>, dim3(blocks_for((long long)n * H2 * W2)), dim3(256), 0, s, a);
-                return GS_OK;
+            } else {
+                a.a1 = view(m->a1);
+                a.raw = view(m->bb[0]);
+                a.b2 = wb + m->w.b2;
+                a.raw_c0 = 64;
+                a.raw_cn = enc.lazy_b2 ? 64 : 0;
+                a.w3c = wb + m->w.w3c;
+                hipLaunchKernelGGL(dec2_kernel<CLS>, dim3((unsigned)(((long long)n * H2 * W2 + 63) / 64)), dim3(256), 0, s, a);
             }
-        }
-        a.a1 = view(m->a1);
-        a.raw = view(m->bb[0]);
-        a.b2 = wb + m->w.b2;
-        a.raw_c0 = 64;
-        a.raw_cn = enc.lazy_b2 ? 64 : 0;
-        a.w3c = wb + m->w.w3c;
-        hipLaunchKernelGGL(dec2_kernel<CLS>, dim3((unsigned)(((long long)n * H2 * W2 + 63) / 64)), dim3(256), 0, s, a);
-        return GS_OK;
-    });
-    if (ncls == CLS)
-        m->set_stage("combine_t", m->tt, 2 * CLS);
+            return GS_OK;
+        });
+        if (ncls == CLS)
+            m->set_stage("combine_t", m->tt, 2 * CLS);
+    }
     if constexpr (dec3_on_mfma(CLS)) {
         L.run(K_DEC3, px2 * (2 * ncls * 9 * ncls * 2), [&] {
             return launch_dec3<CLS>(m, plan.dec3, conv_args(m->tt, wb + m->w.wcc_mfma, m->t3, nullptr, n), s);
@@ -645,16 +665,30 @@
         });
     } else {
         L.run(K_DEC3, px2 * (2 * ncls * 9 * ncls * 2) + px2 * (ncls * ncls * 4 * 2), [&] {
-            Dec3Args a{};
-            a.t = view(m->tt);
-            a.wc = wb + m->w.wcc;
-            a.bnc = wb + m->w.bncc;
-            a.wup = wb + m->w.wup2;
-            a.bnu = wb + m->w.bnu2;
-            a.e = view(m->ee);
-            a.N = n;
-            a.classes = ncls;
-            hipLaunchKernelGGL(dec3_kernel<CLS>, dim3(blocks_for((long long)n * H2 * W2)), dim3(256), 0, s, a);
+            if constexpr (l3c_side_sums(CLS)) {
+                Dec3CatArgs a{};
+                a.l3c = view(m->l3c);
+                a.o2c = view(m->o2c);
+                a.br = wb + m->w.cbr0;
+                a.wc = wb + m->w.wcc;
+                a.bnc = wb + m->w.bncc;
+                a.wup = wb + m->w.wup2;
+                a.bnu = wb + m->w.bnu2;
+                a.e = view(m->ee);
+                a.N = n;
+                hipLaunchKernelGGL(dec3_cat_kernel<CLS>, dim3(blocks_for((long long)n * H2 * W2 / DEC3_PX)), dim3(256), 0, s, a);
+            } else {
+                Dec3Args a{};
+                a.t = view(m->tt);
+                a.wc = wb + m->w.wcc;
+                a.bnc = wb + m->w.bncc;
+                a.wup = wb + m->w.wup2;
+                a.bnu = wb + m->w.bnu2;
+                a.e = view(m->ee);
+                a.N = n;
+                a.classes = ncls;
+                hipLaunchKernelGGL(dec3_kernel<CLS>, dim3(blocks_for((long long)n * H2 * W2)), dim3(256), 0, s, a);
+            }
             return GS_OK;
         });
     }
@@ -717,7 +751,7 @@
 static gs_status forward_any(Model *m, const ForwardReq &r)
 {
     Launcher L{m, r.s, GS_OK, r.n};
-    const ForwardPlan plan = plan_forward(r.n, r.H, r.W, m->p, m->q, m->cp, m->num_cus, no_vec(), m->encoder_only);
+    const ForwardPlan plan = plan_forward(r.n, r.H, r.W, m->p, m->q, m->cp, m->num_cus, no_vec(), m->encoder_only, r.logits != nullptr);
     const Encoded e = encode(m, L, plan, r);
     switch (m->cp) {
     case 5: return decode<5>(m, L, plan, r, e);
@@ -1063,7 +1097,9 @@
     GS_REQUIRE(h && stage && dims, "gs_espnet_read_stage: null argument");
     Model &m = h->m;
     auto it = m.stages.find(stage);
-    GS_REQUIRE(it != m.stages.end(), "stage '%s' was not produced by the last forward", stage);
+    GS_REQUIRE(it != m.stages.end(), "stage '%s' was not produced by the last forward%s", stage,
+               m.lean ? " (a lean forward -- mask-only, glomseg_lean.h -- materialises neither 'combine_t' nor the last 'level3.<i>', and no "
+                        "mask-only forward keeps 'conv': request logits to read them)" : "");
     GS_REQUIRE(image >= 0 && image < m.last_n, "image index %d out of range", image);
     const Act &a = it->second.first;
     const int C = it->second.second;
@@ -1125,7 +1161,7 @@
             r = kind == 1 ? launch_l3_reduce(&m, form::l3_reduce::C1S, false, rca, s) : launch_l3_c1(&m, rca, s);
             if (r != GS_OK) return r;
             r = kind == 1 ? launch_l3_down(&m, unfused_l3_down(dst.W, no_vec()), false, bca, s)
-                          : launch_l3_esp_last(&m, whole_row_l3_esp(dst.W, no_vec()), false, bca, s);
+                          : launch_l3_esp_last(&m, whole_row_l3_esp(dst.W, no_vec()), false, false, bca, s);
         }
         if (r != GS_OK) return r;
         hipLaunchKernelGGL(unpad_kernel, dim3(blocks_for((long long)nout)), dim3(256), 0, s, view(dst), 0, cout, tmp);
@@ -1166,6 +1202,17 @@
     if (st != GS_OK) return st;
     const ForwardPlan pl = plan_forward(n, height, width, p, q, padded_classes(classes), num_cus, no_vec(), encoder_only != 0);
     *flags = (pl.lazy_b2 ? GS_PLAN_LAZY_B2 : 0) | (pl.l3c_in_reduce ? GS_PLAN_L3C_IN_REDUCE : 0) | (pl.cls_in_l3 ? GS_PLAN_CLS_IN_L3 : 0);
+    return GS_OK;
+}
+
+gs_status gs_espnet_plan_lean(int n, int height, int width, int p, int q, int classes, int encoder_only, int num_cus, int want_logits,
+                              int *lean)
+{
+    GS_REQUIRE(lean, "gs_espnet_plan_lean: null argument");
+    int count = 0;
+    gs_status st = gs_espnet_plan_forward(n, height, width, p, q, classes, num_cus, nullptr, 0, &count);
+    if (st != GS_OK) return st;
+    *lean = plan_forward(n, height, width, p, q, padded_classes(classes), num_cus, no_vec(), encoder_only != 0, want_logits != 0).lean;
     return GS_OK;
 }
 
diff --git a/glomeruli_segmentation_amd/csrc/espnet_kernels.h b/glomeruli_segmentation_amd/csrc/espnet_kernels.h
--- a/glomeruli_segmentation_amd/csrc/espnet_kernels.h
+++ b/glomeruli_segmentation_amd/csrc/espnet_kernels.h
@@ -35,7 +35,11 @@
 #ifndef NT_DEC4_ST
 #define NT_DEC4_ST 1
 #endif
+#ifndef NT_DEC3_ST
+#define NT_DEC3_ST 1
+#endif
 typedef float f32x2_t __attribute__((ext_vector_type(2)));
+typedef float f32x4_t __attribute__((ext_vector_type(4)));
 template <bool NT>
 __device__ __forceinline__ float ld_stream(const float *p)
 {
@@ -245,26 +249,40 @@
     }
 }
 
+constexpr int POOL_PX = 2;
 __global__ void __launch_bounds__(256)
 pool_kernel(const ActV in, const ActV out, int N, int C, const float *bnp2, const ActV out2, int coff2, int C2)
 {
-    const long long idx = (long long)blockIdx.x * 256 + threadIdx.x;
-    if (idx >= (long long)N * C * out.H * out.W)
-        return;
-    const int x = (int)(idx % out.W);
-    const int y = (int)((idx / out.W) % out.H);
-    const int c = (int)((idx / ((long long)out.W * out.H)) % C);
-    const int n = (int)(idx / ((long long)out.W * out.H * C));
-    float s = 0.0f;
-#pragma unroll
-    for (int ky = 0; ky < 3; ++ky)
+    const int WP = out.W / POOL_PX;
+    const long long idx = (long long)blockIdx.x * 256 + threadIdx.x;
+    if (idx >= (long long)N * C * out.H * WP)
+        return;
+    const int x = (int)(idx % WP) * POOL_PX;
+    const int y = (int)((idx / WP) % out.H);
+    const int c = (int)((idx / ((long long)WP * out.H)) % C);
+    const int n = (int)(idx / ((long long)WP * out.H * C));
+    const float *row0 = at(in, n, c, 2 * y, 0);
+    float s[POOL_PX] = {0.0f, 0.0f};
+#pragma unroll
+    for (int ky = 0; ky < 3; ++ky) {
+        const bool rok = ky > 0 || y > 0;
+        const float *row = row0 + (rok ? ky - 1 : 0) * in.pitch;
+        const float4 q = *reinterpret_cast<const float4 *>(row + 2 * x);
+        const float l = row[x > 0 ? 2 * x - 1 : 0];
+        const float v[5] = {rok && x > 0 ? l : 0.0f, rok ? q.x : 0.0f, rok ? q.y : 0.0f, rok ? q.z : 0.0f, rok ? q.w : 0.0f};
 #pragma unroll
         for (int kx = 0; kx < 3; ++kx)
-            s += ldz(in, n, c, 2 * y - 1 + ky, 2 * x - 1 + kx);
-    s = s / 9.0f;
-    *at(out, n, c, y, x) = s;
+#pragma unroll
+            for (int p = 0; p < POOL_PX; ++p)
+                s[p] += v[2 * p + kx];
+    }
+#pragma unroll
+    for (int p = 0; p < POOL_PX; ++p)
+        s[p] = s[p] / 9.0f;
+    *reinterpret_cast<f32x2_t *>(at(out, n, c, y, x)) = f32x2_t{s[0], s[1]};
     if (bnp2)
-        *at(out2, n, coff2 + c, y, x) = bn_prelu(s, bnp2, C2, coff2 + c);
+        *reinterpret_cast<f32x2_t *>(at(out2, n, coff2 + c, y, x)) =
+            f32x2_t{bn_prelu(s[0], bnp2, C2, coff2 + c), bn_prelu(s[1], bnp2, C2, coff2 + c)};
 }
 
 __global__ void __launch_bounds__(256)
@@ -631,6 +649,100 @@
         for (int dy = 0; dy < 2; ++dy)
             if (o < ncls)
                 *reinterpret_cast<float2 *>(at(a.e, n, o, 2 * y + dy, 2 * x)) = make_float2(up[o][dy][0], up[o][dy][1]);
+}
+
+struct Dec3CatArgs {
+    ActV l3c;
+    ActV o2c;
+    const float *br;
+    const float *wc;
+    const float *bnc;
+    const float *wup;
+    const float *bnu;
+    ActV e;
+    int N;
+};
+constexpr int DEC3_PX = 4;
+
+__device__ __forceinline__ f32x2_t bn_prelu2(f32x2_t v, const float *bnp, int C, int c)
+{
+    const float alpha = bnp[2 * C + c], pin = alpha <= 1.0f ? __builtin_inff() : -__builtin_inff();
+    v = __builtin_elementwise_fma(v, (f32x2_t)(bnp[c]), (f32x2_t)(bnp[C + c]));
+    const f32x2_t av = v * alpha;
+    return f32x2_t{__builtin_amdgcn_fmed3f(v[0], av[0], pin), __builtin_amdgcn_fmed3f(v[1], av[1], pin)};
+}
+
+template <int CLS>
+__global__ void __launch_bounds__(256) dec3_cat_kernel(const Dec3CatArgs a)
+{
+    const int H2 = a.l3c.H, W2 = a.l3c.W, HB = H2 / 2, WB = W2 / 2;
+    const long long idx = (long long)blockIdx.x * 256 + threadIdx.x;
+    if (idx >= (long long)a.N * HB * WB)
+        return;
+    const int x = (int)(idx % WB) * 2;
+    const int y = (int)((idx / WB) % HB) * 2;
+    const int n = (int)(idx / ((long long)WB * HB));
+    const bool second = x & 2;
+    const int x4 = x & ~3, xe = second ? min(x + 2, W2 - 1) : max(x - 1, 0);
+    const bool cok[4] = {x > 0, true, true, x + 2 < W2}, rok[4] = {y > 0, true, true, y + 2 < H2};
+    const int ry[4] = {max(y - 1, 0), y, y + 1, min(y + 2, H2 - 1)};
+    f32x2_t s[2][CLS];
+#pragma unroll
+    for (int r = 0; r < 2; ++r)
+#pragma unroll
+        for (int k = 0; k < CLS; ++k)
+            s[r][k] = (f32x2_t)(0.0f);
+    for (int c = 0; c < 2 * CLS; ++c) {
+        const bool lo = c < CLS;
+        const float *plane = lo ? at(a.l3c, n, c, 0, 0) : at(a.o2c, n, c - CLS, 0, 0);
+        const int pitch = lo ? a.l3c.pitch : a.o2c.pitch;
+        f32x2_t w[4][2];
+#pragma unroll
+        for (int wr = 0; wr < 4; ++wr) {
+            const float *row = plane + ry[wr] * pitch;
+            const float4 q = *reinterpret_cast<const float4 *>(row + x4);
+            const float e = row[xe];
+            const f32x2_t t0 = bn_prelu2(f32x2_t{second ? q.y : e, second ? q.z : q.x}, a.br, 2 * CLS, c);
+            const f32x2_t t1 = bn_prelu2(f32x2_t{second ? q.w : q.y, second ? e : q.z}, a.br, 2 * CLS, c);
+            w[wr][0] = f32x2_t{rok[wr] && cok[0] ? t0[0] : 0.0f, rok[wr] ? t0[1] : 0.0f};
+            w[wr][1] = f32x2_t{rok[wr] ? t1[0] : 0.0f, rok[wr] && cok[3] ? t1[1] : 0.0f};
+        }
+#pragma unroll
+        for (int ky = 0; ky < 3; ++ky)
+#pragma unroll
+            for (int kx = 0; kx < 3; ++kx)
+#pragma unroll
+                for (int k = 0; k < CLS; ++k) {
+                    const f32x2_t wk = (f32x2_t)(a.wc[((k * 2 * CLS + c) * 3 + ky) * 3 + kx]);
+#pragma unroll
+                    for (int r = 0; r < 2; ++r) {
+                        const f32x2_t *wp = w[r + ky];
+                        const f32x2_t v = kx == 0 ? wp[0] : kx == 1 ? f32x2_t{wp[0][1], wp[1][0]} : wp[1];
+                        s[r][k] = __builtin_elementwise_fma(wk, v, s[r][k]);
+                    }
+                }
+    }
+#pragma unroll
+    for (int r = 0; r < 2; ++r) {
+#pragma unroll
+        for (int k = 0; k < CLS; ++k)
+            s[r][k] = bn_prelu2(s[r][k], a.bnc, CLS, k);
+#pragma unroll
+        for (int o = 0; o < CLS; ++o)
+#pragma unroll
+            for (int dy = 0; dy < 2; ++dy) {
+                f32x2_t up[2];
+#pragma unroll
+                for (int dx = 0; dx < 2; ++dx) {
+                    f32x2_t t = (f32x2_t)(0.0f);
+#pragma unroll
+                    for (int i = 0; i < CLS; ++i)
+                        t = __builtin_elementwise_fma(s[r][i], (f32x2_t)(a.wup[((i * CLS + o) * 2 + dy) * 2 + dx]), t);
+                    up[dx] = bn_prelu2(t, a.bnu, CLS, o);
+                }
+                st_stream<NT_DEC3_ST>(reinterpret_cast<f32x4_t *>(at(a.e, n, o, 2 * (y + r) + dy, 2 * x)), f32x4_t{up[0][0], up[1][0], up[0][1], up[1][1]});
+            }
+    }
 }
 
 template <int CLS>
diff --git a/glomeruli_segmentation_amd/csrc/forward_plan.h b/glomeruli_segmentation_amd/csrc/forward_plan.h
--- a/glomeruli_segmentation_amd/csrc/forward_plan.h
+++ b/glomeruli_segmentation_amd/csrc/forward_plan.h
@@ -102,6 +102,7 @@
     bool lazy_b2 = false;
     bool l3c_in_reduce = false;
     bool cls_in_l3 = false;
+    bool lean = false;
     void codes(int *out) const { GS_LAUNCH_CLASSES(GS_PLAN_CODE) }
 };
 #undef GS_FORM_ID
@@ -135,7 +136,8 @@
     return vec_fits(form::l3_esp_last::BR_VEC, W3, no_vec) ? form::l3_esp_last::BR_VEC : form::l3_esp_last::P2;
 }
 
-inline ForwardPlan plan_forward(int n, int H, int W, int p, int q, int cp, int num_cus, bool no_vec, bool encoder_only = false)
+inline ForwardPlan plan_forward(int n, int H, int W, int p, int q, int cp, int num_cus, bool no_vec, bool encoder_only = false,
+                                bool want_logits = true)
 {
     namespace f = form;
     const int W1 = W / 2, H2 = H / 4, W2 = W / 4, H3 = H / 8, W3 = W / 8;
@@ -144,6 +146,7 @@
     pl.lazy_b2 = b2_is_lazy(p);
     pl.l3c_in_reduce = !encoder_only && l3c_side_sums(cp);
     pl.cls_in_l3 = !encoder_only && cls_side_sums(cp, q);
+    pl.lean = !want_logits && pl.cls_in_l3 && pl.l3c_in_reduce;
 
     const bool small2 = CFG_SMALL2_WAVES > 0 && (long long)n * H2 * cdiv(W2, 64) * 2 <= cus * CFG_SMALL2_WAVES &&
                         vec_fits(f::l2_down::P2S_VEC, W2, no_vec);
diff --git a/glomeruli_segmentation_amd/engine.py b/glomeruli_segmentation_amd/engine.py
--- a/glomeruli_segmentation_amd/engine.py
+++ b/glomeruli_segmentation_amd/engine.py
@@ -286,6 +286,13 @@
     flags = ctypes.c_int()
     _lib.check(_lib.load().gs_espnet_plan_flags(n, height, width, p, q, classes, int(bool(encoder_only)), num_cus, ctypes.byref(flags)))
     return bool(flags.value & _lib.GS_PLAN_CLS_IN_L3)
+
+
+def plan_lean(n, height, width, p, q, classes, num_cus, encoder_only=False, want_logits=False):
+    lean = ctypes.c_int()
+    _lib.check(_lib.load().gs_espnet_plan_lean(n, height, width, p, q, classes, int(bool(encoder_only)), num_cus, int(bool(want_logits)),
+                                               ctypes.byref(lean)))
+    return bool(lean.value)
 
 
 def pack_weights(state_dict, classes=5, p=2, q=8, encoder_only=False):
diff --git a/include/glomseg_lean.h b/include/glomseg_lean.h
--- /dev/null
+++ b/include/glomseg_lean.h
@@ -0,0 +1,17 @@
+#ifndef GLOMSEG_LEAN_H
+#define GLOMSEG_LEAN_H
+
+#include "glomseg.h"
+
+#ifdef __cplusplus
+extern "C" {
+#endif
+
+gs_status gs_espnet_plan_lean(int n, int height, int width, int p, int q, int classes, int encoder_only, int num_cus, int want_logits,
+                              int *lean);
+
+#ifdef __cplusplus
+}
+#endif
+
+#endif
```

New measurement: 11940 patches/s (median of 6 runs). 1.1% higher.
